# asharakeh/bayes-od-rc

Hardware: AMD Instinct MI355X
Metric: images/sec at N=10 MC samples, 512x512; per-anchor covariance latency (higher is better)
Workload: dtype bf16; 1 GPU; ResNet-50 RetinaNet + covar head, N=10 MC-dropout, 512x512, full BayesOD pipeline (forward+posterior+soft-NMS+cluster-fuse); global_batch=512, mc_samples=10, anchors=49104, parallelism=one GPU (no exchange; N > 1: image-sharded, one RCCL gather/step), visible_gpus=1, gpu_max_hw_queues=4

## Files before the change

### bayes-od-rc_amd/build.py

```python
import os
import shutil
import subprocess
import sys

HERE = os.path.dirname(os.path.abspath(__file__))
CSRC = os.path.join(HERE, "csrc")
LIB_DIR = os.path.join(HERE, "lib")
LIB_PATH = os.path.join(LIB_DIR, "libbayesod_hip.so")

SOURCES = [
    ("conv_igemm.hip", []),
    ("conv_igemm_f32.hip", []),
    ("conv_pointwise.hip", []),
    ("aux_kernels.hip", []),
    ("post_kernels.hip", ["-ffp-contract=off"]),
    ("loss_kernels.hip", ["-ffp-contract=off"]),
    ("pdq_kernels.hip", ["-ffp-contract=off"]),
    ("score_kernels.hip", ["-ffp-contract=off"]),
    ("target_kernels.hip", ["-ffp-contract=off"]),
    ("stat_kernels.hip", ["-ffp-contract=off"]),
    ("train_kernels.hip", []),
    ("jpeg_kernels.hip", []),
    ("png_kernels.hip", []),
    ("corrupt_kernels.hip", ["-ffp-contract=off"]),
    ("engine.hip", []),
]
COMMON = ["--offload-arch=gfx950", "-O3", "-std=c++17", "-fPIC", "-Wall", "-Wno-unused-function",
          "-Wno-unused-result", "-Wno-unused-value", "-fno-slp-vectorize"]


def _hipcc():
    for cand in (os.environ.get("HIPCC"), shutil.which("hipcc"), "/opt/rocm/bin/hipcc"):
        if cand and os.path.exists(cand):
            return cand
    raise RuntimeError("hipcc not found (ROCm toolchain required to build libbayesod_hip.so)")


def _stale(target, deps):
    if not os.path.exists(target):
        return True
    t = os.path.getmtime(target)
    return any(os.path.getmtime(d) > t for d in deps)


HEADER = os.path.join(os.path.dirname(HERE), "include", "bayesod.h")
CDEF = os.path.join(os.path.dirname(HERE), "include", "bayesod_cdef.h")


def cdef_text():
    import re
    text = open(HEADER).read()
    text = re.sub(r"/\*.*?\*/", "", text, flags=re.S)
    out = []
    for line in text.splitlines():
        t = line.strip()
        if not t or t.startswith("#") or t == 'extern "C" {' or t == "}":
            continue
        out.append(line.rstrip())
    return ("/* GENERATED from include/bayesod.h by bayes_od_rc_amd.build.write_cdef(): the same declarations without\n"
            " * comments / preprocessor lines, for ffi.cdef(open('include/bayesod_cdef.h').read()).  Do not edit. */\n"
            + "\n".join(out) + "\n")


def write_cdef():
    text = cdef_text()
    if not os.path.exists(CDEF) or open(CDEF).read() != text:
        with open(CDEF, "w") as fp:
            fp.write(text)
    return CDEF


def _load_guard():
    import importlib.util
    spec = importlib.util.spec_from_file_location("bayesod_kernel_guard", os.path.join(HERE, "kernel_guard.py"))
    mod = importlib.util.module_from_spec(spec)
    spec.loader.exec_module(mod)
    return mod


def build(force=False, verbose=True):
    hipcc = _hipcc()
    try:
        write_cdef()
    except OSError as e:
        if verbose:
            print("include/bayesod_cdef.h not refreshed (%s)" % e, flush=True)
    os.makedirs(LIB_DIR, exist_ok=True)
    obj_dir = os.path.join(LIB_DIR, "obj")
    os.makedirs(obj_dir, exist_ok=True)
    headers = [os.path.join(CSRC, f) for f in os.listdir(CSRC) if f.endswith((".h", ".inc"))]
    headers.append(os.path.join(os.path.dirname(HERE), "include", "bayesod.h"))
    objs = []
    for src, extra in SOURCES:
        s = os.path.join(CSRC, src)
        o = os.path.join(obj_dir, src.replace(".hip", ".o"))
        if force or _stale(o, [s] + headers):
            cmd = [hipcc] + COMMON + extra + ["-c", s, "-o", o]
            if verbose:
                print(" ".join(cmd), flush=True)
            subprocess.check_call(cmd)
        objs.append(o)
    if force or _stale(LIB_PATH, objs):
        if os.environ.get("BOD_SKIP_KERNEL_GUARD") == "1":
            print("WARNING: BOD_SKIP_KERNEL_GUARD=1 -- linking libbayesod_hip.so WITHOUT the disassembly guards (spills, inline-asm MFMA "
                  "hazard windows and hand-counted LDS waits are UNCHECKED)", file=sys.stderr, flush=True)
        else:
            kernel_guard = _load_guard()
            regs = kernel_guard.verify(os.path.join(obj_dir, "conv_igemm.o"))
            regs.update(kernel_guard.verify_aux(os.path.join(obj_dir, "aux_kernels.o")))
            regs.update(kernel_guard.verify_pointwise(os.path.join(obj_dir, "conv_pointwise.o")))
            regs.update(kernel_guard.verify_pointwise_stage3(os.path.join(obj_dir, "conv_pointwise.o")))
            n_checked = sum(kernel_guard.check_no_packed_fp32(o) for o in objs)
            if verbose:
                print("no packed fp32 instruction in %d kernels" % n_checked, flush=True)
            if verbose:
                print("kernel guards ok: %d production kernels, no spills, inline-asm MFMA windows clean" % len(regs), flush=True)
        cmd = [hipcc, "--offload-arch=gfx950", "-shared", "-fPIC"] + objs + ["-o", LIB_PATH]
        if verbose:
            print(" ".join(cmd), flush=True)
        subprocess.check_call(cmd)
    return LIB_PATH


if __name__ == "__main__":
    build(force="--force" in sys.argv)
```

### bayes-od-rc_amd/csrc/conv_pointwise.hip

```cpp
#include "kernels.h"
#include <algorithm>

typedef __attribute__((ext_vector_type(8))) short pw_bf16x8;
typedef __attribute__((ext_vector_type(16))) float pw_f32x16;
typedef __attribute__((ext_vector_type(4))) float pw_f32x4;
typedef __attribute__((ext_vector_type(2))) uint32_t pw_u32x2;
typedef __attribute__((ext_vector_type(4))) uint32_t pw_u32x4;
typedef __attribute__((ext_vector_type(4))) int pw_i32x4;

#define PW_GLOBAL_PTR(p) ((const __attribute__((address_space(1))) void*)(p))
#define PW_LDS_PTR(p) ((__attribute__((address_space(3))) void*)(p))

__device__ uint4 pw_sink[64];

__device__ __forceinline__ uint32_t pw_pack(float lo, float hi) {
    uint32_t r;
    asm("v_cvt_pk_bf16_f32 %0, %1, %2" : "=v"(r) : "v"(lo), "v"(hi));
    return r;
}
__device__ __forceinline__ uint32_t pw_relu(uint32_t w) {
    uint32_t r;
    asm("v_pk_max_i16 %0, %1, 0" : "=v"(r) : "v"(w));
    return r;
}
__device__ __forceinline__ float pw_bf2f(uint32_t v) { return __uint_as_float(v << 16); }

template <int CPR> __device__ __forceinline__ int pw_swz(int px) { return CPR >= 16 ? (px & 15) : ((px >> 1) & 7); }

template <int N> __device__ __forceinline__ void pw_wait_vm() { asm volatile("s_waitcnt vmcnt(%0)" ::"n"(N) : "memory"); }
__device__ __forceinline__ void pw_lds_barrier() {
    asm volatile("s_waitcnt lgkmcnt(0)" ::: "memory");
    __builtin_amdgcn_s_barrier();
    asm volatile("" ::: "memory");
}

template <int K, int BP, bool RES, int WGS, int BC = 128, int NEXT = 0>
__global__ __launch_bounds__(BC * 2, WGS) void pw_conv_kernel(const ConvArgs a, int ptiles, int ctiles, int pstride) {
    constexpr int THREADS = BC * 2;
    constexpr int CPX = K * 2 / 16;
    constexpr int RCH = BC / 8;
    constexpr int XB = BP * K * 2;
    constexpr int RB = BP * BC * 2;
    constexpr int NXP = BP * CPX / THREADS;
    constexpr int NRP = BP * RCH / THREADS;
    constexpr int FP = BP / 32, KS = K / 16;
    constexpr int C2 = 64, KS2 = NEXT == 2 ? K / 16 : BC / 16;
    constexpr int K2 = NEXT == 2 ? K : BC;
    constexpr int NTP = NEXT ? BP * (C2 / 8) / THREADS : 0;
    static_assert(NXP >= 1 && NRP >= 1 && BP % 32 == 0 && (CPX & 7) == 0 && (!NEXT || (BC == 256 && BP == 64 && NTP == 1)), "tile shape");
    extern __shared__ __attribute__((aligned(16))) char pw_smem[];
    char* const xbuf = pw_smem;
    constexpr int NRB = RES ? 2 : 1;
    char* const rbuf = pw_smem + 2 * XB;
    int4* const meta = reinterpret_cast<int4*>(pw_smem + 2 * XB + NRB * RB);
    char* const tbuf = pw_smem + 2 * XB + NRB * RB + 3 * BP * 16;

    const int tid = threadIdx.x, lane = tid & 63;
    const int wave = __builtin_amdgcn_readfirstlane(tid >> 6);
    const int frow = lane & 31, fhalf = lane >> 5;
    const ConvGroup& G = a.g[0];
    const int xcd = blockIdx.x & 7, jb = blockIdx.x >> 3;
    const int ct = jb % ctiles, p0 = (jb / ctiles) * 8 + xcd;
    const int c0 = ct * BC;
    const int nt = p0 < ptiles ? (ptiles - p0 + pstride - 1) / pstride : 0;
    if (nt == 0) return;

    auto load_ent = [&](int t) {
        const int tt = t < nt ? t : nt - 1;
        int m = (p0 + tt * pstride) * BP + (tid % BP);
        const int valid = m < a.M;
        m = valid ? m : a.M - 1;
        const int4 e = *reinterpret_cast<const int4*>(&a.rows[m]);
        return make_int4(e.x, e.z, e.w, valid);
    };
    auto issue = [&](int t) {
        const int4* mt = meta + (t % 3) * BP;
        char* xb = xbuf + (t & 1) * XB;
#pragma unroll
        for (int i = 0; i < NXP; ++i) {
            const int q = i * THREADS + tid, row = q / CPX, cp = q % CPX;
            const int c = cp ^ pw_swz<CPX>(row);
            const char* src = reinterpret_cast<const char*>(G.in) + ((size_t)mt[row].x * a.in_cstride + G.in_coff + c * 8) * 2;
            __builtin_amdgcn_global_load_lds(PW_GLOBAL_PTR(src), PW_LDS_PTR(xb + (i * THREADS + wave * 64) * 16), 16, 0, 0);
        }
        if (RES) {
            char* rb = rbuf + (t & 1) * RB;
#pragma unroll
            for (int i = 0; i < NRP; ++i) {
                const int q = i * THREADS + tid, row = q / RCH, cp = q % RCH;
                const int c = cp ^ (row & 7);
                const char* src = reinterpret_cast<const char*>(G.res) + ((size_t)mt[row].z * a.res_cstride + c0 + c * 8) * 2;
                __builtin_amdgcn_global_load_lds(PW_GLOBAL_PTR(src), PW_LDS_PTR(rb + (i * THREADS + wave * 64) * 16), 16, 0, 0);
            }
        }
    };

    {
        const int4 e0 = load_ent(0), e1 = load_ent(1);
        if (tid < BP) { meta[tid] = e0; meta[BP + tid] = e1; }
    }
    __syncthreads();
    issue(0);
    asm volatile("" ::: "memory");
    pw_bf16x8 wf[KS];
    {
        const char* wrow = reinterpret_cast<const char*>(G.w) + ((size_t)(c0 + wave * 32 + frow) * K + fhalf * 8) * 2;
#pragma unroll
        for (int ks = 0; ks < KS; ++ks) wf[ks] = *reinterpret_cast<const pw_bf16x8*>(wrow + ks * 32);
    }
    float4 bv[4];
#pragma unroll
    for (int g = 0; g < 4; ++g) bv[g] = *reinterpret_cast<const float4*>(G.bias + c0 + wave * 32 + g * 8 + fhalf * 4);
    const bool relu = a.flags & CONV_RELU;
    pw_bf16x8 wf2[NEXT ? KS2 : 1];
    float4 bv2[4];
    if (NEXT) {
        const char* wrow = reinterpret_cast<const char*>(G.ch_w3) + ((size_t)((wave & 1) * 32 + frow) * K2 + fhalf * 8) * 2;
#pragma unroll
        for (int ks = 0; ks < KS2; ++ks) wf2[ks] = *reinterpret_cast<const pw_bf16x8*>(wrow + ks * 32);
#pragma unroll
        for (int g = 0; g < 4; ++g) bv2[g] = *reinterpret_cast<const float4*>(G.ch_b3 + (wave & 1) * 32 + g * 8 + fhalf * 4);
    }

    for (int t = 0; t < nt; ++t) {
        __syncthreads();
        const bool more = t + 1 < nt;
        if (more) issue(t + 1);
        asm volatile("" ::: "memory");
        const int4 ent = load_ent(t + 2);
        asm volatile("" ::: "memory");
        if (more) { if (t > 0) pw_wait_vm<1 + NRP + NTP + NXP + (RES ? NRP : 0) + 1>(); else pw_wait_vm<NXP + (RES ? NRP : 0) + 1>(); }
        else pw_wait_vm<1>();
        __syncthreads();

        const char* xb = xbuf + (t & 1) * XB;
        char* rb = rbuf + (RES ? (t & 1) : 0) * RB;
        pw_f32x16 acc[FP];
#pragma unroll
        for (int j = 0; j < FP; ++j)
#pragma unroll
            for (int r = 0; r < 16; ++r) acc[j][r] = 0.f;
#pragma unroll
        for (int ks = 0; ks < KS; ++ks)
#pragma unroll
            for (int j = 0; j < FP; ++j) {
                const int px = j * 32 + frow;
                const pw_bf16x8 b = *reinterpret_cast<const pw_bf16x8*>(xb + px * (K * 2) + (((ks * 2 + fhalf) ^ pw_swz<CPX>(px)) << 4));
                acc[j] = __builtin_amdgcn_mfma_f32_32x32x16_bf16(wf[ks], b, acc[j], 0, 0, 0);
            }
#pragma unroll
        for (int j = 0; j < FP; ++j) {
            const int px = j * 32 + frow;
#pragma unroll
            for (int g = 0; g < 4; ++g) {
                char* p = rb + px * (BC * 2) + (((wave * 4 + g) ^ (px & 7)) << 4) + fhalf * 8;
                float v0 = __builtin_fmaf(acc[j][g * 4 + 0], 1.0f, bv[g].x), v1 = __builtin_fmaf(acc[j][g * 4 + 1], 1.0f, bv[g].y);
                float v2 = __builtin_fmaf(acc[j][g * 4 + 2], 1.0f, bv[g].z), v3 = __builtin_fmaf(acc[j][g * 4 + 3], 1.0f, bv[g].w);
                if (RES) {
                    const uint2 r = *reinterpret_cast<const uint2*>(p);
                    v0 += pw_bf2f(r.x & 0xFFFFu) * 1.0f; v1 += pw_bf2f(r.x >> 16) * 1.0f;
                    v2 += pw_bf2f(r.y & 0xFFFFu) * 1.0f; v3 += pw_bf2f(r.y >> 16) * 1.0f;
                }
                uint2 o;
                o.x = pw_pack(v0, v1); o.y = pw_pack(v2, v3);
                if (relu) { o.x = pw_relu(o.x); o.y = pw_relu(o.y); }
                *reinterpret_cast<uint2*>(p) = o;
            }
        }
        __syncthreads();
        {
            const int4* mt = meta + (t % 3) * BP;
#pragma unroll
            for (int i = 0; i < NRP; ++i) {
                const int q = i * THREADS + tid, row = q / RCH, cp = q % RCH;
                const int c = cp ^ (row & 7);
                const uint4 v = *reinterpret_cast<const uint4*>(rb + q * 16);
                const int4 e = mt[row];
                uint4* dst = e.w ? reinterpret_cast<uint4*>(reinterpret_cast<uint16_t*>(G.out) + (size_t)e.y * a.out_cstride + c0 + c * 8) : &pw_sink[lane];
                *dst = v;
            }
        }
        if (NEXT) {
            if (wave < 4) {
                const int px = (wave >> 1) * 32 + frow;
                pw_f32x16 acc2;
#pragma unroll
                for (int r = 0; r < 16; ++r) acc2[r] = 0.f;
#pragma unroll
                for (int ks = 0; ks < KS2; ++ks) {
                    const pw_bf16x8 b = NEXT == 2 ? *reinterpret_cast<const pw_bf16x8*>(xb + px * (K * 2) + (((ks * 2 + fhalf) ^ pw_swz<CPX>(px)) << 4))
                                                  : *reinterpret_cast<const pw_bf16x8*>(rb + px * (BC * 2) + (((ks * 2 + fhalf) ^ (px & 7)) << 4));
                    acc2 = __builtin_amdgcn_mfma_f32_32x32x16_bf16(wf2[ks], b, acc2, 0, 0, 0);
                }
#pragma unroll
                for (int g = 0; g < 4; ++g) {
                    uint2 o;
                    o.x = pw_relu(pw_pack(__builtin_fmaf(acc2[g * 4 + 0], 1.0f, bv2[g].x), __builtin_fmaf(acc2[g * 4 + 1], 1.0f, bv2[g].y)));
                    o.y = pw_relu(pw_pack(__builtin_fmaf(acc2[g * 4 + 2], 1.0f, bv2[g].z), __builtin_fmaf(acc2[g * 4 + 3], 1.0f, bv2[g].w)));
                    *reinterpret_cast<uint2*>(tbuf + px * 128 + ((((wave & 1) * 4 + g) ^ (px & 7)) << 4) + fhalf * 8) = o;
                }
            }
            __syncthreads();
            {
                const int4* mt = meta + (t % 3) * BP;
                const int q = tid, row = q >> 3, cp = q & 7;
                const int c = cp ^ (row & 7);
                const uint4 v = *reinterpret_cast<const uint4*>(tbuf + q * 16);
                const int4 e = mt[row];
                uint4* dst = e.w ? reinterpret_cast<uint4*>(reinterpret_cast<uint16_t*>(G.ch_out3) + (size_t)e.y * C2 + c * 8) : &pw_sink[lane];
                *dst = v;
            }
        }
        asm volatile("" ::: "memory");
        if (tid < BP) meta[((t + 2) % 3) * BP + tid] = ent;
    }
}

template <int K, int BP, bool RES, int WGS, int BC = 128, int NEXT = 0>
static hipError_t pw_launch_cfg(const ConvArgs& a, hipStream_t s) {
    constexpr int LDS = 2 * BP * K * 2 + (RES ? 2 : 1) * BP * BC * 2 + 3 * BP * 16 + (NEXT ? BP * 128 : 0);
    static PerDeviceOnce once;
    bool& attr_set = *once.slot();
    auto kern = pw_conv_kernel<K, BP, RES, WGS, BC, NEXT>;
    if (!attr_set) {
        hipError_t e = hipFuncSetAttribute(reinterpret_cast<const void*>(kern), hipFuncAttributeMaxDynamicSharedMemorySize, LDS);
        if (e != hipSuccess) return e;
        attr_set = true;
    }
    const int ptiles = (a.M + BP - 1) / BP, ctiles = a.cout_pad / BC;
    const int slots = launch_cus(a) * WGS;
    int pstride = std::min(slots / ctiles, ptiles) / 8 * 8;
    if (pstride < 8) pstride = 8;
    hipLaunchKernelGGL(kern, dim3(pstride * ctiles), dim3(BC * 2), LDS, s, a, ptiles, ctiles, pstride);
    return hipGetLastError();
}

__global__ __launch_bounds__(512, 1) void pw_conv512_next_kernel(const ConvArgs a, int ptiles, int pstride) {
    constexpr int K = 128, BP = 32, BC = 512, C2 = 128, THREADS = 512;
    constexpr int CPX = K / 8, RCH = BC / 8, TCH = C2 / 8;
    constexpr int XB = BP * K * 2, RB = BP * BC * 2, TB = BP * C2 * 2;
    constexpr int NXP = BP * CPX / THREADS, NRP = BP * RCH / THREADS, NTP = BP * TCH / THREADS;
    constexpr int KS = K / 16, KSH = BC / 32;
    static_assert(NXP == 1 && NRP == 4 && NTP == 1, "tile shape");
    extern __shared__ __attribute__((aligned(16))) char pw_smem[];
    char* const xbuf = pw_smem;
    char* const rbuf = pw_smem + 2 * XB;
    pw_i32x4* const meta = reinterpret_cast<pw_i32x4*>(pw_smem + 2 * XB + 2 * RB);
    char* const tbuf = pw_smem + 2 * XB + 2 * RB + 3 * BP * 16;
    pw_f32x4* const relay = reinterpret_cast<pw_f32x4*>(pw_smem + 2 * XB + 2 * RB + 3 * BP * 16 + TB);
    float* const sbias = reinterpret_cast<float*>(pw_smem + 2 * XB + 2 * RB + 3 * BP * 16 + TB + 16384);

    const int tid = threadIdx.x, lane = tid & 63;
    const int wave = __builtin_amdgcn_readfirstlane(tid >> 6);
    const int frow = lane & 31, fhalf = lane >> 5;
    const int cb = wave & 3, kh = wave >> 2;
    const ConvGroup& G = a.g[0];
    const int p0 = blockIdx.x;
    const int nt = p0 < ptiles ? (ptiles - p0 + pstride - 1) / pstride : 0;
    if (nt == 0) return;

    auto load_ent = [&](int t) {
        const int tt = t < nt ? t : nt - 1;
        int m = (p0 + tt * pstride) * BP + (tid % BP);
        const int valid = m < a.M;
        m = valid ? m : a.M - 1;
        const int4 e = *reinterpret_cast<const int4*>(&a.rows[m]);
        return pw_i32x4{e.x, e.z, e.w, valid};
    };
    auto issue = [&](int t) {
        const int* mt = reinterpret_cast<const int*>(meta + (t % 3) * BP);
        const int in_off = mt[(tid / CPX) * 4];
        int res_off[NRP];
#pragma unroll
        for (int i = 0; i < NRP; ++i) res_off[i] = mt[((i * THREADS + tid) / RCH) * 4 + 2];
        {
            const int row = tid / CPX, cp = tid % CPX;
            const int c = cp ^ pw_swz<CPX>(row);
            const char* src = reinterpret_cast<const char*>(G.in) + ((size_t)in_off * a.in_cstride + G.in_coff + c * 8) * 2;
            __builtin_amdgcn_global_load_lds(PW_GLOBAL_PTR(src), PW_LDS_PTR(xbuf + (t & 1) * XB + (wave * 64) * 16), 16, 0, 0);
        }
        char* rb = rbuf + (t & 1) * RB;
#pragma unroll
        for (int i = 0; i < NRP; ++i) {
            const int q = i * THREADS + tid, row = q / RCH, cp = q % RCH;
            const int c = cp ^ pw_swz<RCH>(row);
            const char* src = reinterpret_cast<const char*>(G.res) + ((size_t)res_off[i] * a.res_cstride + c * 8) * 2;
            __builtin_amdgcn_global_load_lds(PW_GLOBAL_PTR(src), PW_LDS_PTR(rb + (i * THREADS + wave * 64) * 16), 16, 0, 0);
        }
    };

    {
        const pw_i32x4 e0 = load_ent(0), e1 = load_ent(1);
        if (tid < BP) { meta[tid] = e0; meta[BP + tid] = e1; }
        sbias[tid] = G.bias[tid];
        if (tid < C2) sbias[BC + tid] = G.ch_b3[tid];
    }
    __syncthreads();
    issue(0);
    asm volatile("" ::: "memory");
    pw_bf16x8 wf[2][KS], wf2[KSH];
#pragma unroll
    for (int b = 0; b < 2; ++b) {
        const char* wrow = reinterpret_cast<const char*>(G.w) + ((size_t)(wave * 64 + b * 32 + frow) * K + fhalf * 8) * 2;
#pragma unroll
        for (int ks = 0; ks < KS; ++ks) wf[b][ks] = *reinterpret_cast<const pw_bf16x8*>(wrow + ks * 32);
    }
    {
        const char* wrow = reinterpret_cast<const char*>(G.ch_w3) + ((size_t)(cb * 32 + frow) * BC + kh * (BC / 2) + fhalf * 8) * 2;
#pragma unroll
        for (int ks = 0; ks < KSH; ++ks) wf2[ks] = *reinterpret_cast<const pw_bf16x8*>(wrow + ks * 32);
    }
    const bool relu = a.flags & CONV_RELU;
    const int px = frow;

    for (int t = 0; t < nt; ++t) {
        pw_lds_barrier();
        const bool more = t + 1 < nt;
        if (more) issue(t + 1);
        asm volatile("" ::: "memory");
        const pw_i32x4 ent = load_ent(t + 2);
        asm volatile("" ::: "memory");
        if (more) { if (t > 0) pw_wait_vm<1 + NRP + NTP + NXP + NRP + 1>(); else pw_wait_vm<NXP + NRP + 1>(); }
        else pw_wait_vm<1>();
        pw_lds_barrier();

        const char* xb = xbuf + (t & 1) * XB;
        char* rb = rbuf + (t & 1) * RB;
        int sw = pw_swz<RCH>(px);
        asm volatile("" : "+v"(sw));
        pw_f32x16 acc[2];
#pragma unroll
        for (int b = 0; b < 2; ++b)
#pragma unroll
            for (int r = 0; r < 16; ++r) acc[b][r] = 0.f;
#pragma unroll
        for (int ks = 0; ks < KS; ++ks) {
            const pw_bf16x8 bf = *reinterpret_cast<const pw_bf16x8*>(xb + px * (K * 2) + (((ks * 2 + fhalf) ^ sw) << 4));
            acc[0] = __builtin_amdgcn_mfma_f32_32x32x16_bf16(wf[0][ks], bf, acc[0], 0, 0, 0);
            acc[1] = __builtin_amdgcn_mfma_f32_32x32x16_bf16(wf[1][ks], bf, acc[1], 0, 0, 0);
        }
#pragma unroll
        for (int b = 0; b < 2; ++b)
#pragma unroll
            for (int g = 0; g < 4; ++g) {
                char* p = rb + px * (BC * 2) + ((((wave * 2 + b) * 4 + g) ^ sw) << 4) + fhalf * 8;
                const pw_f32x4 bv = *reinterpret_cast<const pw_f32x4*>(sbias + (wave * 2 + b) * 32 + g * 8 + fhalf * 4);
                float v0 = __builtin_fmaf(acc[b][g * 4 + 0], 1.0f, bv.x), v1 = __builtin_fmaf(acc[b][g * 4 + 1], 1.0f, bv.y);
                float v2 = __builtin_fmaf(acc[b][g * 4 + 2], 1.0f, bv.z), v3 = __builtin_fmaf(acc[b][g * 4 + 3], 1.0f, bv.w);
                const pw_u32x2 r = *reinterpret_cast<const pw_u32x2*>(p);
                v0 += pw_bf2f(r.x & 0xFFFFu) * 1.0f; v1 += pw_bf2f(r.x >> 16) * 1.0f;
                v2 += pw_bf2f(r.y & 0xFFFFu) * 1.0f; v3 += pw_bf2f(r.y >> 16) * 1.0f;
                pw_u32x2 o;
                o.x = pw_pack(v0, v1); o.y = pw_pack(v2, v3);
                if (relu) { o.x = pw_relu(o.x); o.y = pw_relu(o.y); }
                *reinterpret_cast<pw_u32x2*>(p) = o;
            }
        pw_lds_barrier();
        const pw_i32x4* mt = meta + (t % 3) * BP;
#pragma unroll
        for (int i = 0; i < NRP; ++i) {
            const int q = i * THREADS + tid, row = q / RCH, cp = q % RCH;
            const int c = cp ^ pw_swz<RCH>(row);
            const pw_u32x4 v = *reinterpret_cast<const pw_u32x4*>(rb + q * 16);
            const pw_i32x4 e = mt[row];
            pw_u32x4* dst = e.w ? reinterpret_cast<pw_u32x4*>(reinterpret_cast<uint16_t*>(G.out) + (size_t)e.y * a.out_cstride + c * 8) : reinterpret_cast<pw_u32x4*>(&pw_sink[lane]);
            *dst = v;
        }
        pw_f32x16 acc2;
        if (kh == 0) {
#pragma unroll
            for (int r = 0; r < 16; ++r) acc2[r] = 0.f;
#pragma unroll
            for (int ks = 0; ks < KSH; ++ks) {
                const pw_bf16x8 bf = *reinterpret_cast<const pw_bf16x8*>(rb + px * (BC * 2) + (((ks * 2 + fhalf) ^ sw) << 4));
                acc2 = __builtin_amdgcn_mfma_f32_32x32x16_bf16(wf2[ks], bf, acc2, 0, 0, 0);
            }
#pragma unroll
            for (int g = 0; g < 4; ++g) relay[(cb * 4 + g) * 64 + lane] = pw_f32x4{acc2[g * 4 + 0], acc2[g * 4 + 1], acc2[g * 4 + 2], acc2[g * 4 + 3]};
        }
        pw_lds_barrier();
        if (kh == 1) {
#pragma unroll
            for (int g = 0; g < 4; ++g) {
                const pw_f32x4 v = relay[(cb * 4 + g) * 64 + lane];
                acc2[g * 4 + 0] = v.x; acc2[g * 4 + 1] = v.y; acc2[g * 4 + 2] = v.z; acc2[g * 4 + 3] = v.w;
            }
#pragma unroll
            for (int ks = 0; ks < KSH; ++ks) {
                const pw_bf16x8 bf = *reinterpret_cast<const pw_bf16x8*>(rb + px * (BC * 2) + (((KSH * 2 + ks * 2 + fhalf) ^ sw) << 4));
                acc2 = __builtin_amdgcn_mfma_f32_32x32x16_bf16(wf2[ks], bf, acc2, 0, 0, 0);
            }
#pragma unroll
            for (int g = 0; g < 4; ++g) {
                const pw_f32x4 bv = *reinterpret_cast<const pw_f32x4*>(sbias + BC + cb * 32 + g * 8 + fhalf * 4);
                pw_u32x2 o;
                o.x = pw_relu(pw_pack(__builtin_fmaf(acc2[g * 4 + 0], 1.0f, bv.x), __builtin_fmaf(acc2[g * 4 + 1], 1.0f, bv.y)));
                o.y = pw_relu(pw_pack(__builtin_fmaf(acc2[g * 4 + 2], 1.0f, bv.z), __builtin_fmaf(acc2[g * 4 + 3], 1.0f, bv.w)));
                *reinterpret_cast<pw_u32x2*>(tbuf + px * (C2 * 2) + (((cb * 4 + g) ^ sw) << 4) + fhalf * 8) = o;
            }
        }
        pw_lds_barrier();
        if (tid < BP) meta[((t + 2) % 3) * BP + tid] = ent;
        {
            const int row = tid / TCH, cp = tid % TCH;
            const int c = cp ^ pw_swz<TCH>(row);
            const pw_u32x4 v = *reinterpret_cast<const pw_u32x4*>(tbuf + tid * 16);
            const pw_i32x4 e = mt[row];
            pw_u32x4* dst = e.w ? reinterpret_cast<pw_u32x4*>(reinterpret_cast<uint16_t*>(G.ch_out3) + (size_t)e.y * C2 + c * 8) : reinterpret_cast<pw_u32x4*>(&pw_sink[lane]);
            *dst = v;
        }
    }
}

static hipError_t pw_launch_next512(const ConvArgs& a, hipStream_t s) {
    constexpr int BP = 32;
    constexpr int LDS = 2 * BP * 128 * 2 + 2 * BP * 512 * 2 + 3 * BP * 16 + BP * 128 * 2 + 16384 + (512 + 128) * 4;
    static PerDeviceOnce once;
    bool& attr_set = *once.slot();
    if (!attr_set) {
        hipError_t e = hipFuncSetAttribute(reinterpret_cast<const void*>(pw_conv512_next_kernel), hipFuncAttributeMaxDynamicSharedMemorySize, LDS);
        if (e != hipSuccess) return e;
        attr_set = true;
    }
    const int ptiles = (a.M + BP - 1) / BP;
    int pstride = std::min(launch_cus(a), ptiles) / 8 * 8;
    if (pstride < 8) pstride = 8;
    hipLaunchKernelGGL(pw_conv512_next_kernel, dim3(pstride), dim3(512), LDS, s, a, ptiles, pstride);
    return hipGetLastError();
}

bool conv_pointwise_eligible(const ConvArgs& a) {
    static const bool on = [] { const char* e = getenv("BOD_POINTWISE"); return !e || atoi(e) != 0; }();
    if (!on) return false;
    const ConvGroup& g = a.g[0];
    if (a.variant != 0 || a.split || a.xreuse || a.ksplit > 1 || a.groups != 1 || a.taps != 1 || a.fan_count > 1) return false;
    if (a.flags & (CONV_DROPOUT | CONV_OUT_F32 | CONV_ACCUM)) return false;
    if (g.w2 || g.ch_w2 || g.out_relu || g.agg_kind) return false;
    if (g.ch_w3 && !(g.ch_b3 && g.ch_out3 && ((a.cin == 64 && a.cout_pad == 256 && (g.res != nullptr) != (g.ch_dual != 0)) ||
                                              (a.cin == 128 && a.cout_pad == 512 && g.res && !g.ch_dual)))) return false;
    if (a.cin != 64 && a.cin != 128 && a.cin != 256 && !(a.cin == 512 && !g.res)) return false;
    if (a.cout_pad % 128 != 0 || a.cout_valid != a.cout_pad) return false;
    if ((a.in_cstride & 7) || (a.out_cstride & 7) || (g.in_coff & 7) || (g.res && (a.res_cstride & 7))) return false;
    static const int min_m = [] { const char* e = getenv("BOD_POINTWISE_MIN_M"); return e ? atoi(e) : -1; }();
    if (a.M < (min_m >= 0 ? min_m : 128 * launch_cus(a))) return false;
    return true;
}

hipError_t launch_conv_pointwise(const ConvArgs& a, hipStream_t s) {
    const bool res = a.g[0].res != nullptr;
    if (a.g[0].ch_w3 && a.g[0].ch_dual) return pw_launch_cfg<64, 64, false, 1, 256, 2>(a, s);
    if (a.g[0].ch_w3 && a.cin == 128) return pw_launch_next512(a, s);
    if (a.g[0].ch_w3) return pw_launch_cfg<64, 64, true, 1, 256, 1>(a, s);
    if (a.cin == 64) return res ? pw_launch_cfg<64, 64, true, 3>(a, s) : pw_launch_cfg<64, 64, false, 3>(a, s);
    if (a.cin == 128) return res ? pw_launch_cfg<128, 64, true, 2>(a, s) : pw_launch_cfg<128, 64, false, 2>(a, s);
    if (a.cin == 512) return pw_launch_cfg<512, 32, false, 2>(a, s);
    return res ? pw_launch_cfg<256, 32, true, 3>(a, s) : pw_launch_cfg<256, 32, false, 3>(a, s);
}


__global__ __launch_bounds__(256, 2) void slide3x3_c64_kernel(const ConvArgs a, int nstrips, int xsegs) {
    constexpr int SLOT = 66 * 128;
    constexpr int LEAD = 1;
    constexpr int RING = 4;
    constexpr int OB = 64 * 128;
    extern __shared__ __attribute__((aligned(16))) char sl_smem[];
    char* const ring = sl_smem;
    char* const obuf = sl_smem + RING * SLOT;
    const int tid = threadIdx.x, lane = tid & 63;
    const int wave = __builtin_amdgcn_readfirstlane(tid >> 6);
    const int frow = lane & 31, fhalf = lane >> 5;
    const int wc = wave & 1, wp = wave >> 1;
    const ConvGroup& G = a.g[0];
    const int H = a.plane_h, W = a.plane_w;

    pw_bf16x8 wf[36];
    {
        const char* wrow = reinterpret_cast<const char*>(G.w) + ((size_t)(wc * 32 + frow) * 576 + fhalf * 8) * 2;
#pragma unroll
        for (int k = 0; k < 36; ++k) wf[k] = *reinterpret_cast<const pw_bf16x8*>(wrow + k * 32);
    }
    float4 bv[4];
#pragma unroll
    for (int g = 0; g < 4; ++g) bv[g] = *reinterpret_cast<const float4*>(G.bias + wc * 32 + g * 8 + fhalf * 4);
    const bool relu = a.flags & CONV_RELU;

    for (int strip = blockIdx.x; strip < nstrips; strip += gridDim.x) {
        const int b = strip / xsegs, xs = strip - b * xsegs;
        const int x0 = xs * 64, nv = min(64, W - x0);
        const int m00 = (b * H) * W + x0;
        const int4 e0 = *reinterpret_cast<const int4*>(&a.rows[m00]);
        const int out_pitch = H > 1 ? a.rows[m00 + W].out_off - e0.z : 0;
        const long in0 = (long)e0.x;
        const int in_pitch = e0.y;
        auto issue_row = [&](int ir) {
            char* slot = ring + (ir % RING) * SLOT;
            auto piece = [&](int i) {
                const int q = i * 256 + tid;
                int px = q >> 3;
                const int cp = q & 7;
                const int c = cp ^ pw_swz<8>(px);
                px = px < nv + 2 ? px : 0;
                const char* src = reinterpret_cast<const char*>(G.in) + (((size_t)(in0 + (long)ir * in_pitch + px)) * a.in_cstride + G.in_coff + c * 8) * 2;
                __builtin_amdgcn_global_load_lds(PW_GLOBAL_PTR(src), PW_LDS_PTR(slot + (i * 256 + wave * 64) * 16), 16, 0, 0);
            };
            piece(0); piece(1);
            if (wave == 0 && lane < 16) piece(2);
        };
        __syncthreads();
        issue_row(0); issue_row(1); issue_row(2);
        for (int y = 0; y < H; ++y) {
            const bool pre = y + LEAD < H;
            if (pre) issue_row(y + 2 + LEAD);
            asm volatile("" ::: "memory");
            if (!pre) pw_wait_vm<0>();
            else if (wave == 0) { if (y == 0) pw_wait_vm<3>(); else pw_wait_vm<5>(); }
            else { if (y == 0) pw_wait_vm<2>(); else pw_wait_vm<4>(); }
            __syncthreads();
            pw_f32x16 acc;
#pragma unroll
            for (int r = 0; r < 16; ++r) acc[r] = 0.f;
#pragma unroll
            for (int ky = 0; ky < 3; ++ky) {
                const char* slot = ring + ((y + ky) % RING) * SLOT;
#pragma unroll
                for (int kx = 0; kx < 3; ++kx)
#pragma unroll
                    for (int ks = 0; ks < 4; ++ks) {
                        const int px = wp * 32 + frow + kx;
                        const pw_bf16x8 bf = *reinterpret_cast<const pw_bf16x8*>(slot + px * 128 + (((ks * 2 + fhalf) ^ pw_swz<8>(px)) << 4));
                        acc = __builtin_amdgcn_mfma_f32_32x32x16_bf16(wf[(ky * 3 + kx) * 4 + ks], bf, acc, 0, 0, 0);
                    }
            }
            char* ob = obuf + (y & 1) * OB;
            {
                const int px = wp * 32 + frow;
#pragma unroll
                for (int g = 0; g < 4; ++g) {
                    uint2 o;
                    o.x = pw_pack(__builtin_fmaf(acc[g * 4 + 0], 1.0f, bv[g].x), __builtin_fmaf(acc[g * 4 + 1], 1.0f, bv[g].y));
                    o.y = pw_pack(__builtin_fmaf(acc[g * 4 + 2], 1.0f, bv[g].z), __builtin_fmaf(acc[g * 4 + 3], 1.0f, bv[g].w));
                    if (relu) { o.x = pw_relu(o.x); o.y = pw_relu(o.y); }
                    *reinterpret_cast<uint2*>(ob + px * 128 + (((wc * 4 + g) ^ (px & 7)) << 4) + fhalf * 8) = o;
                }
            }
            __syncthreads();
#pragma unroll
            for (int i = 0; i < 2; ++i) {
                const int q = i * 256 + tid, px = q >> 3, cp = q & 7;
                const int c = cp ^ (px & 7);
                const uint4 v = *reinterpret_cast<const uint4*>(ob + q * 16);
                uint4* dst = px < nv ? reinterpret_cast<uint4*>(reinterpret_cast<uint16_t*>(G.out) + ((size_t)e0.z + (size_t)y * out_pitch + px) * a.out_cstride + c * 8)
                                     : &pw_sink[lane];
                *dst = v;
            }
            asm volatile("" ::: "memory");
        }
    }
}

__global__ __launch_bounds__(512, 1) void slide3x3_c128_kernel(const ConvArgs a, int nstrips, int xsegs) {
    constexpr int SLOT = 66 * 256;
    constexpr int RING = 4;
    constexpr int OB = 64 * 256;
    extern __shared__ __attribute__((aligned(16))) char sl_smem[];
    char* const ring = sl_smem;
    char* const obuf = sl_smem + RING * SLOT;
    float4* const xch = reinterpret_cast<float4*>(sl_smem + RING * SLOT + 2 * OB);
    float* const sbias = reinterpret_cast<float*>(sl_smem + RING * SLOT + 2 * OB + 8 * 4096);
    const int tid = threadIdx.x, lane = tid & 63;
    const int wave = __builtin_amdgcn_readfirstlane(tid >> 6);
    const int frow = lane & 31, fhalf = lane >> 5;
    const int cb = wave & 3, kh = wave >> 2;
    const ConvGroup& G = a.g[0];
    const int H = a.plane_h, W = a.plane_w;

    pw_bf16x8 wf[36];
    {
        const char* wrow = reinterpret_cast<const char*>(G.w) + ((size_t)(cb * 32 + frow) * 1152 + kh * 64 + fhalf * 8) * 2;
#pragma unroll
        for (int t = 0; t < 9; ++t)
#pragma unroll
            for (int ks = 0; ks < 4; ++ks) wf[t * 4 + ks] = *reinterpret_cast<const pw_bf16x8*>(wrow + (t * 128 + ks * 16) * 2);
    }
    if (tid < 128) sbias[tid] = G.bias[tid];
    const bool relu = a.flags & CONV_RELU;

    for (int strip = blockIdx.x; strip < nstrips; strip += gridDim.x) {
        const int b = strip / xsegs, xs = strip - b * xsegs;
        const int x0 = xs * 64, nv = min(64, W - x0);
        const int m00 = (b * H) * W + x0;
        const int4 e0 = *reinterpret_cast<const int4*>(&a.rows[m00]);
        const int out_pitch = H > 1 ? a.rows[m00 + W].out_off - e0.z : 0;
        const long in0 = (long)e0.x;
        const int in_pitch = e0.y;
        auto issue_row = [&](int ir) {
            char* slot = ring + (ir % RING) * SLOT;
            auto piece = [&](int i) {
                const int q = i * 512 + tid;
                int px = q >> 4;
                const int cp = q & 15;
                const int c = cp ^ (px & 7);
                px = px < nv + 2 ? px : 0;
                const char* src = reinterpret_cast<const char*>(G.in) + (((size_t)(in0 + (long)ir * in_pitch + px)) * a.in_cstride + G.in_coff + c * 8) * 2;
                __builtin_amdgcn_global_load_lds(PW_GLOBAL_PTR(src), PW_LDS_PTR(slot + (i * 512 + wave * 64) * 16), 16, 0, 0);
            };
            piece(0); piece(1);
            if (wave == 0 && lane < 32) piece(2);
        };
        __syncthreads();
        issue_row(0); issue_row(1); issue_row(2);
        for (int y = 0; y < H; ++y) {
            const bool pre = y + 1 < H;
            if (pre) issue_row(y + 3);
            asm volatile("" ::: "memory");
            if (!pre) pw_wait_vm<0>();
            else if (wave == 0) { if (y == 0) pw_wait_vm<3>(); else pw_wait_vm<5>(); }
            else { if (y == 0) pw_wait_vm<2>(); else pw_wait_vm<4>(); }
            __syncthreads();
            pw_f32x16 acc[2];
#pragma unroll
            for (int j = 0; j < 2; ++j)
#pragma unroll
                for (int r = 0; r < 16; ++r) acc[j][r] = 0.f;
#pragma unroll
            for (int ky = 0; ky < 3; ++ky) {
                const char* slot = ring + ((y + ky) % RING) * SLOT;
#pragma unroll
                for (int kx = 0; kx < 3; ++kx)
#pragma unroll
                    for (int ks = 0; ks < 4; ++ks)
#pragma unroll
                        for (int j = 0; j < 2; ++j) {
                            const int px = j * 32 + frow + kx;
                            const pw_bf16x8 bf = *reinterpret_cast<const pw_bf16x8*>(slot + px * 256 + (((kh * 8 + ks * 2 + fhalf) ^ (px & 7)) << 4));
                            acc[j] = __builtin_amdgcn_mfma_f32_32x32x16_bf16(wf[(ky * 3 + kx) * 4 + ks], bf, acc[j], 0, 0, 0);
                        }
            }
            {
                float4* mine = xch + wave * 256;
#pragma unroll
                for (int g = 0; g < 4; ++g) {
                    const pw_f32x16& v = acc[1 - kh];
                    mine[g * 64 + lane] = make_float4(v[g * 4 + 0], v[g * 4 + 1], v[g * 4 + 2], v[g * 4 + 3]);
                }
            }
            __syncthreads();
            char* ob = obuf + (y & 1) * OB;
            {
                const float4* theirs = xch + (wave ^ 4) * 256;
                const int px = kh * 32 + frow;
#pragma unroll
                for (int g = 0; g < 4; ++g) {
                    const float4 t = theirs[g * 64 + lane];
                    const pw_f32x16& v = acc[kh];
                    const float s0 = kh ? t.x + v[g * 4 + 0] : v[g * 4 + 0] + t.x, s1 = kh ? t.y + v[g * 4 + 1] : v[g * 4 + 1] + t.y;
                    const float s2 = kh ? t.z + v[g * 4 + 2] : v[g * 4 + 2] + t.z, s3 = kh ? t.w + v[g * 4 + 3] : v[g * 4 + 3] + t.w;
                    const float4 bvg = *reinterpret_cast<const float4*>(sbias + cb * 32 + g * 8 + fhalf * 4);
                    uint2 o;
                    o.x = pw_pack(__builtin_fmaf(s0, 1.0f, bvg.x), __builtin_fmaf(s1, 1.0f, bvg.y));
                    o.y = pw_pack(__builtin_fmaf(s2, 1.0f, bvg.z), __builtin_fmaf(s3, 1.0f, bvg.w));
                    if (relu) { o.x = pw_relu(o.x); o.y = pw_relu(o.y); }
                    *reinterpret_cast<uint2*>(ob + px * 256 + (((cb * 4 + g) ^ (px & 7)) << 4) + fhalf * 8) = o;
                }
            }
            __syncthreads();
#pragma unroll
            for (int i = 0; i < 2; ++i) {
                const int q = i * 512 + tid, px = q >> 4, cp = q & 15;
                const int c = cp ^ (px & 7);
                const uint4 v = *reinterpret_cast<const uint4*>(ob + q * 16);
                uint4* dst = px < nv ? reinterpret_cast<uint4*>(reinterpret_cast<uint16_t*>(G.out) + ((size_t)e0.z + (size_t)y * out_pitch + px) * a.out_cstride + c * 8)
                                     : &pw_sink[lane];
                *dst = v;
            }
            asm volatile("" ::: "memory");
        }
    }
}

bool conv_slide3x3_eligible(const ConvArgs& a) {
    static const bool on = [] { const char* e = getenv("BOD_SLIDE3X3"); return !e || atoi(e) != 0; }();
    if (!on) return false;
    const ConvGroup& g = a.g[0];
    if (a.variant != 0 || a.split || a.xreuse || a.ksplit > 1 || a.groups != 1 || a.taps != 9 || a.KW != 3 || a.fan_count > 1) return false;
    if (a.flags & (CONV_DROPOUT | CONV_OUT_F32 | CONV_ACCUM)) return false;
    if (g.w2 || g.ch_w2 || g.out_relu || g.agg_kind || g.res) return false;
    const bool c64 = a.cin == 64 && a.cout_pad == 64 && a.cout_valid == 64;
    static const bool c128_on = [] { const char* e = getenv("BOD_SLIDE3X3_C128"); return !e || atoi(e) != 0; }();
    const bool c128 = c128_on && a.cin == 128 && a.cout_pad == 128 && a.cout_valid == 128;
    if ((!c64 && !c128) || a.plane_h < 1 || a.plane_w < 1) return false;
    if ((a.in_cstride & 7) || (a.out_cstride & 7) || (g.in_coff & 7)) return false;
    if (a.M % (a.plane_h * a.plane_w) != 0) return false;
    static const int min_m = [] { const char* e = getenv("BOD_POINTWISE_MIN_M"); return e ? atoi(e) : -1; }();
    if (min_m >= 0) return a.M >= min_m;
    const long nstrips = (long)(a.M / (a.plane_h * a.plane_w)) * ((a.plane_w + 63) / 64);
    if (c128) return nstrips >= (long)launch_cus(a);
    return 2 * nstrips >= 3 * (long)launch_cus(a);
}

hipError_t launch_conv_slide3x3(const ConvArgs& a, hipStream_t s) {
    if (a.cin == 128) {
        constexpr int LDS128 = 4 * 66 * 256 + 2 * 64 * 256 + 8 * 4096 + 512;
        static PerDeviceOnce once128;
        bool& set128 = *once128.slot();
        if (!set128) {
            hipError_t e = hipFuncSetAttribute(reinterpret_cast<const void*>(slide3x3_c128_kernel), hipFuncAttributeMaxDynamicSharedMemorySize, LDS128);
            if (e != hipSuccess) return e;
            set128 = true;
        }
        const int xsegs = (a.plane_w + 63) / 64;
        const int nstrips = a.M / (a.plane_h * a.plane_w) * xsegs;
        hipLaunchKernelGGL(slide3x3_c128_kernel, dim3(std::min(nstrips, launch_cus(a))), dim3(512), LDS128, s, a, nstrips, xsegs);
        return hipGetLastError();
    }
    constexpr int LDS = 4 * 66 * 128 + 2 * 64 * 128;
    static PerDeviceOnce once;
    bool& attr_set = *once.slot();
    if (!attr_set) {
        hipError_t e = hipFuncSetAttribute(reinterpret_cast<const void*>(slide3x3_c64_kernel), hipFuncAttributeMaxDynamicSharedMemorySize, LDS);
        if (e != hipSuccess) return e;
        attr_set = true;
    }
    const int xsegs = (a.plane_w + 63) / 64;
    const int nstrips = a.M / (a.plane_h * a.plane_w) * xsegs;
    const int wgs = std::min(nstrips, 2 * launch_cus(a));
    hipLaunchKernelGGL(slide3x3_c64_kernel, dim3(wgs), dim3(256), LDS, s, a, nstrips, xsegs);
    return hipGetLastError();
}

bool conv_pointwise_can_fuse_next(const ConvArgs& a) {
    static const bool on = [] { const char* e = getenv("BOD_PW_FUSE_NEXT"); return !e || atoi(e) != 0; }();
    static const bool forced = [] { const char* e = getenv("BOD_FORCE_CONV_TILE"); return e && atoi(e) != 0; }();
    if (!on || forced) return false;
    return a.cin == 64 && a.cout_pad == 256 && a.g[0].res && conv_pointwise_eligible(a);
}

bool conv_pointwise_can_fuse_next3(const ConvArgs& a) {
    static const bool on = [] { const char* e = getenv("BOD_PW_FUSE_NEXT3"); return !e || atoi(e) != 0; }();
    static const bool forced = [] { const char* e = getenv("BOD_FORCE_CONV_TILE"); return e && atoi(e) != 0; }();
    if (!on || forced) return false;
    return a.cin == 128 && a.cout_pad == 512 && a.g[0].res && conv_pointwise_eligible(a);
}

bool conv_pointwise_can_fuse_dual(const ConvArgs& a) {
    static const bool on = [] { const char* e = getenv("BOD_PW_FUSE_DUAL"); return !e || atoi(e) != 0; }();
    static const bool forced = [] { const char* e = getenv("BOD_FORCE_CONV_TILE"); return e && atoi(e) != 0; }();
    if (!on || forced) return false;
    return a.cin == 64 && a.cout_pad == 256 && !a.g[0].res && !(a.flags & CONV_RELU) && conv_pointwise_eligible(a);
}
```

### bayes-od-rc_amd/csrc/engine.hip

```cpp
#include "../../include/bayesod.h"
#include "kernels.h"
#include "plane_tables.h"
#include "jpeg_entropy.h"
#include "png_inflate.h"

#include <algorithm>
#include <array>
#include <atomic>
#include <chrono>
#include <cmath>
#include <condition_variable>
#include <deque>
#include <functional>
#include <mutex>
#include <thread>
#include <tuple>
#include <type_traits>
#include <cstdarg>
#include <cstdio>
#include <cstring>
#include <map>
#include <memory>
#include <string>
#include <system_error>
// ... 3744 lines not shown
    }
    return pdq_call(device, [&](hipStream_t s, char* err, size_t cap) -> int {
        CorruptSlot slot;
        uint8_t* d_rgb = nullptr;
        uint8_t* d_out = nullptr;
        int st = corrupt_prepare(slot, who, spec, src_hw, s, err, cap);
        if (st == BOD_OK && hipMalloc(reinterpret_cast<void**>(&d_rgb), slot.frame_bytes) != hipSuccess) {
            d_rgb = nullptr; snprintf(err, cap, "%s: out of device memory for the frames", who); st = BOD_ERR_OOM;
        }
        if (st == BOD_OK && hipMemcpyAsync(d_rgb, rgb_packed_in, slot.frame_bytes, hipMemcpyHostToDevice, s) != hipSuccess) {
            snprintf(err, cap, "%s: copying the frames in failed", who); st = BOD_ERR_HIP;
        }
        if (st == BOD_OK) st = corrupt_enqueue(slot, who, spec, d_rgb, s, &d_out, err, cap);
        if (st == BOD_OK && (hipMemcpyAsync(rgb_packed_out, d_out, slot.frame_bytes, hipMemcpyDeviceToHost, s) != hipSuccess ||
                             hipStreamSynchronize(s) != hipSuccess)) {
            snprintf(err, cap, "%s: copying the frames back failed: %s", who, hipGetErrorString(hipGetLastError())); st = BOD_ERR_HIP;
        }
        hipStreamSynchronize(s);
        if (d_rgb) hipFree(d_rgb);
        slot.release();
        return st;
    });
}

bod_status bod_set_upload_corruption(bod_handle h, const bod_corrupt_op* ops, int32_t ops_per_frame, const uint32_t* frame_ids,
                                     const uint16_t* taps, int32_t n_taps, const uint8_t* luts, int32_t n_luts, const uint16_t* qtables,
                                     int32_t n_qtables, uint64_t seed) {
    if (!h) return BOD_ERR_INVALID_ARG;
    if (!ops) { h->corrupt_pending = CorruptSpec{}; return BOD_OK; }
    CorruptSpec spec;
    char err[512] = {0};
    const int st = corrupt_spec_make("bod_set_upload_corruption", h->cfg.batch, ops, ops_per_frame, frame_ids, taps, n_taps, luts, n_luts, qtables,
                                     n_qtables, seed, &spec, err, sizeof err);
    if (st != BOD_OK) return h->fail((bod_status)st, "%s", err);
    h->corrupt_pending = std::move(spec);
    return BOD_OK;
}

bod_status bod_jpeg_decode_rgb(int32_t device, int32_t n, const uint8_t* const* data, const int64_t* len, int32_t threads,
                               uint8_t* rgb_packed, int64_t rgb_capacity, int32_t* src_hw) {
    static const char* who = "bod_jpeg_decode_rgb";
    if (n < 1 || !data || !len || !rgb_packed || !src_hw) { g_create_error = std::string(who) + ": NULL argument or no frame"; return BOD_ERR_INVALID_ARG; }
    return pdq_call(device, [&](hipStream_t s, char* err, size_t cap) -> int {
        JpegSlot js;
        std::string e;
        uint8_t* d_rgb = nullptr;
        bod_status st = jpeg_host_decode(js, who, n, data, len, threads, src_hw, &e);
        if (st == BOD_OK && js.rgb_bytes > rgb_capacity) {
            e = std::string(who) + ": the frames take " + std::to_string(js.rgb_bytes) + " bytes, the buffer holds " + std::to_string(rgb_capacity);
            st = BOD_ERR_INVALID_ARG;
        }
        if (st == BOD_OK && hipMalloc(reinterpret_cast<void**>(&d_rgb), (size_t)js.rgb_bytes) != hipSuccess) {
            d_rgb = nullptr; e = std::string(who) + ": out of device memory for the frames"; st = BOD_ERR_OOM;
        }
        if (st == BOD_OK) st = jpeg_enqueue(js, who, d_rgb, s, &e);
        if (st == BOD_OK && (hipMemcpyAsync(rgb_packed, d_rgb, (size_t)js.rgb_bytes, hipMemcpyDeviceToHost, s) != hipSuccess ||
                             hipStreamSynchronize(s) != hipSuccess)) {
            e = std::string(who) + ": copying the frames back failed: " + hipGetErrorString(hipGetLastError()); st = BOD_ERR_HIP;
        }
        hipStreamSynchronize(s);
        if (d_rgb) hipFree(d_rgb);
        js.release();
        if (st != BOD_OK) snprintf(err, cap, "%s", e.c_str());
        return st;
    });
}

bod_status bod_png_decode_rgb(int32_t device, int32_t n, const uint8_t* const* data, const int64_t* len, int32_t threads,
                              uint8_t* rgb_packed, int64_t rgb_capacity, int32_t* src_hw) {
    static const char* who = "bod_png_decode_rgb";
    if (n < 1 || !data || !len || !rgb_packed || !src_hw) { g_create_error = std::string(who) + ": NULL argument or no frame"; return BOD_ERR_INVALID_ARG; }
    return pdq_call(device, [&](hipStream_t s, char* err, size_t cap) -> int {
        PngSlot ps;
        std::string e;
        uint8_t* d_rgb = nullptr;
        bod_status st = png_host_decode(ps, who, n, data, len, threads, src_hw, &e);
        if (st == BOD_OK && ps.rgb_bytes > rgb_capacity) {
            e = std::string(who) + ": the frames take " + std::to_string(ps.rgb_bytes) + " bytes, the buffer holds " + std::to_string(rgb_capacity);
            st = BOD_ERR_INVALID_ARG;
        }
        if (st == BOD_OK && hipMalloc(reinterpret_cast<void**>(&d_rgb), (size_t)ps.rgb_bytes) != hipSuccess) {
            d_rgb = nullptr; e = std::string(who) + ": out of device memory for the frames"; st = BOD_ERR_OOM;
        }
        if (st == BOD_OK) st = png_enqueue(ps, who, d_rgb, s, &e);
        if (st == BOD_OK && (hipMemcpyAsync(rgb_packed, d_rgb, (size_t)ps.rgb_bytes, hipMemcpyDeviceToHost, s) != hipSuccess ||
                             hipStreamSynchronize(s) != hipSuccess)) {
            e = std::string(who) + ": copying the frames back failed: " + hipGetErrorString(hipGetLastError()); st = BOD_ERR_HIP;
        }
        hipStreamSynchronize(s);
        if (d_rgb) hipFree(d_rgb);
        ps.release();
        if (st != BOD_OK) snprintf(err, cap, "%s", e.c_str());
        return st;
    });
}

bod_status bod_bench_png_decode(int32_t device, int32_t n, const uint8_t* const* data, const int64_t* len, int32_t threads, int32_t iters,
                                double* host_ms, double* kernel_ms) {
    static const char* who = "bod_bench_png_decode";
    if (n < 1 || iters < 1 || !data || !len || !host_ms || !kernel_ms) { g_create_error = std::string(who) + ": NULL argument, no frame or no iteration"; return BOD_ERR_INVALID_ARG; }
    return pdq_call(device, [&](hipStream_t s, char* err, size_t cap) -> int {
        PngSlot ps;
        std::string e;
        uint8_t* d_rgb = nullptr;
        hipEvent_t ev[2] = {nullptr, nullptr};
        std::vector<int32_t> hw((size_t)n * 2);
        bod_status st = BOD_OK;
        for (int i = 0; i < iters && st == BOD_OK; ++i) {
            const auto t0 = std::chrono::steady_clock::now();
            st = png_host_decode(ps, who, n, data, len, threads, hw.data(), &e);
            host_ms[i] = std::chrono::duration<double, std::milli>(std::chrono::steady_clock::now() - t0).count();
        }
        if (st == BOD_OK && hipMalloc(reinterpret_cast<void**>(&d_rgb), (size_t)ps.rgb_bytes) != hipSuccess) {
            d_rgb = nullptr; e = std::string(who) + ": out of device memory for the frames"; st = BOD_ERR_OOM;
        }
        if (st == BOD_OK) st = png_enqueue(ps, who, d_rgb, s, &e);
        if (st == BOD_OK && (hipEventCreate(&ev[0]) != hipSuccess || hipEventCreate(&ev[1]) != hipSuccess)) { e = std::string(who) + ": hipEventCreate failed"; st = BOD_ERR_HIP; }
        for (int i = 0; i < iters && st == BOD_OK; ++i) {
            float ms = 0.f;
            hipError_t he = hipEventRecord(ev[0], s);
            if (he == hipSuccess) he = launch_png_unfilter(png_args(ps, d_rgb), s);
            if (he == hipSuccess) he = hipEventRecord(ev[1], s);
            if (he == hipSuccess) he = hipEventSynchronize(ev[1]);
            if (he == hipSuccess) he = hipEventElapsedTime(&ms, ev[0], ev[1]);
            if (he != hipSuccess) { e = std::string(who) + ": timing the kernel failed: " + hipGetErrorString(he); st = BOD_ERR_HIP; }
            kernel_ms[i] = ms;
        }
        hipStreamSynchronize(s);
        for (hipEvent_t v : ev) if (v) hipEventDestroy(v);
        if (d_rgb) hipFree(d_rgb);
        ps.release();
        if (st != BOD_OK) snprintf(err, cap, "%s", e.c_str());
        return st;
    });
}

bod_status bod_bench_head_conv(bod_handle h, int32_t layer, int32_t variant, int32_t iters, double* mean_ms, double* flops) {
    if (!h || !mean_ms || iters < 1 || layer < 0 || layer > 7) return BOD_ERR_INVALID_ARG;
    BODCHK(join_overlap(h));
    if (!h->weights_ready) return h->fail(BOD_ERR_NOT_READY, "weights not finalized");
    HIPCHK(h, hipSetDevice(h->cfg.device));
    int seen = 0; Op* op = nullptr;
    for (Op& o : h->ops) if (o.is_head3x3 && o.flavour != FLAVOUR_RAW && seen++ == layer) { op = &o; break; }
    if (!op) return h->fail(BOD_ERR_INVALID_ARG, "no head launch %d", layer);
    ConvArgs a = op->conv;
    a.variant = variant;
    hipEvent_t e0, e1;
    HIPCHK(h, hipEventCreate(&e0)); HIPCHK(h, hipEventCreate(&e1));
    HIPCHK(h, launch_conv_igemm(a, h->stream));
    HIPCHK(h, hipEventRecord(e0, h->stream));
    for (int i = 0; i < iters; ++i) HIPCHK(h, launch_conv_igemm(a, h->stream));
    HIPCHK(h, hipEventRecord(e1, h->stream));
    HIPCHK(h, hipStreamSynchronize(h->stream));
    float ms = 0; HIPCHK(h, hipEventElapsedTime(&ms, e0, e1));
    hipEventDestroy(e0); hipEventDestroy(e1);
    if ((variant == 90 || variant == 91) && a.mx == 1) {
        unsigned long long c[16];
        conv_igemm_phase_cycles(c, true);
        const double tiles = (double)c[15];
        fprintf(stderr, "# f16mx phase clock, wave 0, cycles per tile (%.0f tiles): whole tile %.0f = set-up %.0f + loop %.0f (of which: waiting for the next K-tile's pieces + barrier %.0f, "
                        "K-tile bodies %.0f; 72 K-tiles) + epilogue %.0f; of the wait: vmcnt / lgkmcnt %.0f, s_barrier %.0f\n", tiles, (double)c[9] / tiles, ((double)c[8] - (double)c[6] - (double)c[7]) / tiles,
                ((double)c[6] + (double)c[7]) / tiles, (double)c[6] / tiles, (double)c[7] / tiles, ((double)c[9] - (double)c[8]) / tiles,
                (double)c[13] / tiles, ((double)c[6] - (double)c[13]) / tiles);
        fprintf(stderr, "# f16mx phase clock by K-tile flavour, cycles per K-tile: wave 0: H %.0f  X %.0f | wave 4: H %.0f  X %.0f, wait + barrier per K-tile %.0f (wave 0: %.0f)"
                        " | MFMA issue of a SIMD's two waves: H 2048, X 1024\n",
                (double)c[0] / tiles / 36.0, (double)c[1] / tiles / 36.0, (double)c[2] / tiles / 36.0, (double)c[3] / tiles / 36.0, (double)c[4] / tiles / 72.0, (double)c[6] / tiles / 72.0);
    } else if (variant == 90) {
        unsigned long long c[16];
        conv_igemm_phase_cycles(c, true);
        const double tiles = (double)c[15];
        static const char* names[6] = {"set-up", "main loop", "barrier+bias/relu/pack", "philox+lds writes", "barrier", "store loop"};
        fprintf(stderr, "# phase clock, wave 0, cycles per tile (%.0f tiles):", tiles);
        for (int k = 0; k < 6; ++k) fprintf(stderr, "  %s %.0f", names[k], (double)c[k] / tiles);
        if (c[10] + c[11] + c[12] > 0)
            fprintf(stderr, "  fused 1x1 MFMAs %.0f  barriers+fp32 tile %.0f  MC reduction+stores %.0f", (double)c[10] / tiles, (double)c[11] / tiles, (double)c[12] / tiles);
        double cyc = 0; for (int k = 0; k < 6; ++k) cyc += (double)c[k];
        cyc += (double)c[10] + (double)c[11] + (double)c[12];
        fprintf(stderr, "  | shader clock during the tiles %.3f GHz (cycles / 100 MHz real-time ticks); tiles account for %.3f ms of the %.3f ms launch per CU\n",
                cyc / (double)c[14] * 0.1, (double)c[14] / tiles * 1e-5 * (tiles / (iters + 1)) / 256.0, ms / iters);
    }
    *mean_ms = ms / iters;
    if (flops) *flops = op->flops;
    return BOD_OK;
}

bod_status bod_profile_begin(bod_handle h) {
    if (!h) return BOD_ERR_INVALID_ARG;
    for (auto& e : h->ev_head) { hipEventDestroy(e.first); hipEventDestroy(e.second); }
    for (auto& e : h->ev_post) { hipEventDestroy(e.first); hipEventDestroy(e.second); }
    h->ev_head.clear(); h->ev_post.clear(); h->prof_flops = 0; h->profiling = true;
    return BOD_OK;
}

extern "C++" {
namespace {
struct Rccl {
    typedef int (*gather_fn)(const void*, void*, size_t, int, int, void*, hipStream_t);
    typedef const char* (*errstr_fn)(int);
    gather_fn gather = nullptr; errstr_fn errstr = nullptr; bool tried = false;
    bool load() {
        if (tried) return gather != nullptr;
        tried = true;
        void* lib = dlopen("librccl.so", RTLD_NOW | RTLD_GLOBAL);
        if (!lib) lib = dlopen("librccl.so.1", RTLD_NOW | RTLD_GLOBAL);
        if (!lib) return false;
        gather = reinterpret_cast<gather_fn>(dlsym(lib, "ncclGather"));
        errstr = reinterpret_cast<errstr_fn>(dlsym(lib, "ncclGetErrorString"));
        return gather != nullptr;
    }
};
Rccl& rccl() { static Rccl r; return r; }
}
}

int32_t bod_record_width(bod_handle h) { return h ? 21 + 2 * h->cfg.num_classes + (h->parts ? 48 : 0) + (h->class_parts ? 4 : 0) : 0; }

bod_status bod_gather_detections(bod_handle h, int32_t slot, void* nccl_comm, int32_t world, int32_t rank, int32_t root,
                                 float* gathered_host, float** gathered_device) {
    MarkerRange mr_api("bod:gather_detections");
    if (!h) return BOD_ERR_INVALID_ARG;
    if (world < 1 || rank < 0 || rank >= world || root < 0 || root >= world)
        return h->fail(BOD_ERR_INVALID_ARG, "bod_gather_detections: world %d, rank %d, root %d", world, rank, root);
    if (!nccl_comm && world != 1) return h->fail(BOD_ERR_INVALID_ARG, "bod_gather_detections: %d ranks need an ncclComm_t", world);
    if (rank != root && (gathered_host || gathered_device)) return h->fail(BOD_ERR_INVALID_ARG, "bod_gather_detections: only the root receives");
    HIPCHK(h, hipSetDevice(h->cfg.device));
    const int B = h->cfg.batch, K = h->cfg.nms_max_output_size, C = h->cfg.num_classes, W = bod_record_width(h);
    const size_t block = (size_t)B * K * W;
    int sidx = slot;
    static const bool side_on = [] { const char* e = getenv("BOD_SIDE_STREAM"); return e && atoi(e) != 0; }();
    hipStream_t st = (slot >= 0 && slot <= 1 && !side_on && h->done_stream[slot]) ? h->done_stream[slot] : h->side;
    if (slot < 0) {
        if (!h->cluster_done) return h->fail(BOD_ERR_NOT_READY, "bod_gather_detections: bod_cluster_fuse has not run");
        BODCHK(join_overlap(h));
        sidx = h->slot;
        st = h->stream;
    } else if (slot > 1 || !h->side_pending[slot]) {
        return h->fail(BOD_ERR_NOT_READY, "bod_gather_detections: slot %d has no pending batch", slot);
    }
    for (int img = 0; h->parts && img < B; ++img)
        if (!h->det_parts_ok[sidx][img]) return h->fail(BOD_ERR_NOT_READY, "bod_gather_detections: image %d was fused without its posterior's parts (bod_set_posterior_parts)", img);
    for (int img = 0; h->cparts && img < B; ++img)
        if (!h->det_cparts_ok[sidx][img]) return h->fail(BOD_ERR_NOT_READY, "bod_gather_detections: image %d was fused without its posterior's class parts (bod_set_posterior_class_parts)", img);
    if (!h->rec_send && hipMalloc(reinterpret_cast<void**>(&h->rec_send), block * 4) != hipSuccess)
        return h->fail(BOD_ERR_OOM, "bod_gather_detections: %zu bytes", block * 4);
    if (h->ev_gather && h->gather_stream && h->gather_stream != st) HIPCHK(h, hipStreamWaitEvent(st, h->ev_gather, 0));
    if (slot >= 0) HIPCHK(h, hipStreamWaitEvent(st, h->ev_done[slot], 0));
    if (h->cparts)
        HIPCHK(h, launch_pack_records_class(h->nms_nsel_s[sidx], h->out_scores_s[sidx], h->out_means_s[sidx], h->out_covs_s[sidx],
                                            h->out_counts_s[sidx], h->out_parts_s[sidx], h->out_cparts_s[sidx], h->rec_send, B, K, C, st));
    else if (h->parts)
        HIPCHK(h, launch_pack_records_parts(h->nms_nsel_s[sidx], h->out_scores_s[sidx], h->out_means_s[sidx], h->out_covs_s[sidx],
                                            h->out_counts_s[sidx], h->out_parts_s[sidx], h->rec_send, B, K, C, st));
    else
        HIPCHK(h, launch_pack_records(h->nms_nsel_s[sidx], h->out_scores_s[sidx], h->out_means_s[sidx], h->out_covs_s[sidx],
                                      h->out_counts_s[sidx], h->rec_send, B, K, C, st));
    float* recv = nullptr;
    if (rank == root) {
        if (world == 1 && !nccl_comm) recv = h->rec_send;
        else {
            if (h->rec_recv_elems < block * world) {
                if (h->rec_recv && h->rec_recv != h->rec_send) hipFree(h->rec_recv);
                h->rec_recv = nullptr; h->rec_recv_elems = 0;
                if (hipMalloc(reinterpret_cast<void**>(&h->rec_recv), block * world * 4) != hipSuccess)
                    return h->fail(BOD_ERR_OOM, "bod_gather_detections: %zu bytes", block * world * 4);
                h->rec_recv_elems = block * world;
            }
            recv = h->rec_recv;
        }
    }
    if (nccl_comm) {
        if (!rccl().load()) return h->fail(BOD_ERR_NOT_READY, "bod_gather_detections: librccl.so (ncclGather) could not be opened");
        const int rc = rccl().gather(h->rec_send, recv, block,  7, root, nccl_comm, st);
        if (rc != 0) return h->fail(BOD_ERR_HIP, "ncclGather: %s", rccl().errstr ? rccl().errstr(rc) : "error");
    }
    if (!h->ev_gather) HIPCHK(h, hipEventCreateWithFlags(&h->ev_gather, hipEventDisableTiming));
    if (rank == root && gathered_host) {
        HIPCHK(h, hipMemcpyAsync(gathered_host, recv, block * world * 4, hipMemcpyDeviceToHost, st));
        HIPCHK(h, hipEventRecord(h->ev_gather, st)); h->gather_stream = st;
        HIPCHK(h, hipEventSynchronize(h->ev_gather));
    } else {
        HIPCHK(h, hipEventRecord(h->ev_gather, st)); h->gather_stream = st;
    }
    if (!(rank == root && gathered_host) && slot >= 0) {
        HIPCHK(h, hipEventRecord(h->ev_done[slot], st));
    }
    if (gathered_device) *gathered_device = recv;
    return BOD_OK;
}

bod_status bod_plan_info(bod_handle h, int32_t* info8) {
    if (!h || !info8) return BOD_ERR_INVALID_ARG;
    if (!h->weights_ready) return h->fail(BOD_ERR_NOT_READY, "bod_plan_info: the plan is built by bod_finalize_weights");
    for (int i = 0; i < 8; ++i) info8[i] = 0;
    info8[0] = h->agg_plan; info8[1] = h->plan_fused_out; info8[2] = h->plan_xreuse; info8[3] = h->plan_xreuse0;
    info8[4] = (int32_t)h->ops.size();
    for (const Op& o : h->ops) if (o.kind == Op::CONV && !o.is_head3x3 && o.conv.xreuse) ++info8[5];
    info8[6] = h->plan_mx;
    info8[7] = h->plan_sparse;
    return BOD_OK;
}

bod_status bod_plan_info_n(bod_handle h, int32_t* info, int32_t n) {
    if (!h || !info || n < 0) return BOD_ERR_INVALID_ARG;
    int32_t all[11];
    BODCHK(bod_plan_info(h, all));
    all[8] = h->plan_halo;
    all[9] = h->plan_tail_rows;
    all[10] = h->plan_stage_end;
    for (int i = 0; i < n && i < 11; ++i) info[i] = all[i];
    return BOD_OK;
}

static bod_status stat_handle(bod_handle h, const char* who) {
    if (!h->cfg.mc_statistics) return h->fail(BOD_ERR_INVALID_ARG, "%s: the handle was not created with mc_statistics = 1", who);
    BODCHK(join_overlap(h));
    HIPCHK(h, hipSetDevice(h->cfg.device));
    return ensure_stat(h);
}

static bod_status stat_view_ready(bod_handle h, const char* who, int32_t view) {
    if (view != BOD_VIEW_IDENTITY && view != BOD_VIEW_HFLIP)
        return h->fail(BOD_ERR_INVALID_ARG, "%s: view must be BOD_VIEW_IDENTITY (0) or BOD_VIEW_HFLIP (1), got %d", who, view);
    if (view == BOD_VIEW_IDENTITY) return BOD_OK;
    if (!h->anchors_ready) return h->fail(BOD_ERR_NOT_READY, "%s: bod_set_anchors has not been called (a mirrored view maps every anchor to its partner)", who);
    const bod_config& c = h->cfg;
    const int K = c.anchors_per_location;
    if (h->mirror_sym < 0) {
        std::vector<float> an((size_t)h->A * 4);
        HIPCHK(h, hipMemcpyAsync(an.data(), h->d_anchors, an.size() * 4, hipMemcpyDeviceToHost, h->stream));
        HIPCHK(h, hipStreamSynchronize(h->stream));
        const float fw = (float)c.image_w;
        int bad = -1;
        for (int l = 0; l < h->nlev && bad < 0; ++l) {
            const size_t off = (size_t)h->lvl_p0[l] * K;
            const int W = h->lw[l];
            for (int y = 0; y < h->lh[l] && bad < 0; ++y)
                for (int x = 0; x < W && bad < 0; ++x)
                    for (int k = 0; k < K; ++k) {
                        const float* s = &an[(off + ((size_t)y * W + x) * K + k) * 4];
                        const float* p = &an[(off + ((size_t)y * W + (W - 1 - x)) * K + k) * 4];
                        const float want[4] = {s[0], fw - s[1], s[2], s[3]};
                        if (memcmp(p, want, 16) != 0) { bad = l; break; }
                    }
        }
        h->mirror_sym = bad < 0; h->mirror_bad_level = bad < 0 ? 0 : c.min_level + bad;
    }
    if (!h->mirror_sym)
        return h->fail(BOD_ERR_INVALID_ARG, "%s: the anchors of pyramid level %d are not mirror-symmetric about image_w / 2 for a %dx%d image "
                       "(BOD_VIEW_HFLIP needs image_w to be a multiple of 2^max_level = %d)", who, h->mirror_bad_level, c.image_h, c.image_w,
                       1 << c.max_level);
    return BOD_OK;
}

static bod_status stat_fold(bod_handle h, const char* who, const float* cls, const float* box, const float* cov, int kb, int32_t view = BOD_VIEW_IDENTITY) {
    if (kb < 1) return h->fail(BOD_ERR_INVALID_ARG, "%s: a record of %d samples", who, kb);
    if (h->stat_k > (1 << 24) - kb) return h->fail(BOD_ERR_INVALID_ARG, "%s: more than 2^24 samples in one accumulator", who);
    if (h->class_parts && h->stat_ent_k != h->stat_k)
        return h->fail(BOD_ERR_NOT_READY, "%s: ent_sum holds %d of the record's %d samples (bod_stat_merge_entropy / bod_stat_set_entropy has not followed)", who, h->stat_ent_k, h->stat_k);
    StatMergeArgs m{};
    m.BA = (int64_t)h->cfg.batch * h->A; m.C = h->cfg.num_classes; m.ka = h->stat_k; m.kb = kb;
    m.acc_cls = h->stat_acc[0]; m.acc_box = h->stat_acc[1]; m.acc_cov = h->stat_acc[2];
    m.src_cls = cls; m.src_box = box; m.src_cov = h->cfg.has_covar_head ? cov : nullptr;
    if (!cls || !box || (h->cfg.has_covar_head && !cov)) return h->fail(BOD_ERR_INVALID_ARG, "%s: NULL statistics array", who);
    if (cls == m.acc_cls || box == m.acc_box) return h->fail(BOD_ERR_INVALID_ARG, "%s: the source is the accumulator itself", who);
    if (((uintptr_t)cls | (uintptr_t)box | (uintptr_t)m.src_cov) & 15u) return h->fail(BOD_ERR_INVALID_ARG, "%s: statistics arrays must be 16-byte aligned", who);
    if (view == BOD_VIEW_HFLIP) {
        StatMirrorArgs mm{};
        mm.m = m; mm.A = h->A; mm.K = h->cfg.anchors_per_location; mm.nlev = h->nlev;
        for (int l = 0; l < h->nlev; ++l) { mm.lvl_off[l] = (int32_t)h->lvl_p0[l] * mm.K; mm.lvl_w[l] = h->lw[l]; }
        mm.lvl_off[h->nlev] = h->A;
        mm.u_flip = (float)(h->cfg.image_w - 1);
        HIPCHK(h, launch_stat_merge_mirror(mm, h->stream));
    } else {
        HIPCHK(h, launch_stat_merge(m, h->stream));
    }
    h->stat_k += kb;
    return BOD_OK;
}

static bod_status stat_fold_entropy(bod_handle h, const char* who, const float* ent, int32_t view = BOD_VIEW_IDENTITY) {
    if (!ent) return h->fail(BOD_ERR_INVALID_ARG, "%s: ent_sum is NULL", who);
    if (ent == h->stat_ent) return h->fail(BOD_ERR_INVALID_ARG, "%s: the source is the accumulator itself", who);
    if ((uintptr_t)ent & 15u) return h->fail(BOD_ERR_INVALID_ARG, "%s: ent_sum must be 16-byte aligned", who);
    if (h->stat_ent_k >= h->stat_k) return h->fail(BOD_ERR_NOT_READY, "%s: ent_sum already holds the record's %d samples (fold the three arrays first)", who, h->stat_k);
    const int64_t BA = (int64_t)h->cfg.batch * h->A;
    if (view == BOD_VIEW_HFLIP) {
        StatMirrorArgs mm{};
        mm.A = h->A; mm.K = h->cfg.anchors_per_location; mm.nlev = h->nlev;
        for (int l = 0; l < h->nlev; ++l) { mm.lvl_off[l] = (int32_t)h->lvl_p0[l] * mm.K; mm.lvl_w[l] = h->lw[l]; }
        mm.lvl_off[h->nlev] = h->A;
        HIPCHK(h, launch_stat_merge_entropy(h->stat_ent, ent, BA, h->stat_ent_k == 0, &mm, h->stream));
    } else {
        HIPCHK(h, launch_stat_merge_entropy(h->stat_ent, ent, BA, h->stat_ent_k == 0, nullptr, h->stream));
    }
    h->stat_ent_k = h->stat_k;
    return BOD_OK;
}

bod_status bod_stat_reset(bod_handle h) {
    if (!h) return BOD_ERR_INVALID_ARG;
    BODCHK(stat_handle(h, "bod_stat_reset"));
    h->stat_k = 0; h->stat_ent_k = 0;
    return BOD_OK;
}

static bod_status stat_forward_view(bod_handle h, const char* who, const float* images, int32_t on_device, uint64_t seed, uint32_t first_image_id,
                                    int32_t sample_base, int32_t view) {
    MarkerRange mr_api("bod:stat_forward");
    if (!h) return BOD_ERR_INVALID_ARG;
    BODCHK(stat_handle(h, who));
    if (!h->weights_ready) return h->fail(BOD_ERR_NOT_READY, "weights not finalized");
    if (!h->anchors_ready) return h->fail(BOD_ERR_NOT_READY, "bod_set_anchors has not been called (the box statistics are those of the decoded boxes)");
    const bod_config& c = h->cfg;
    const int n = c.mc_samples;
    if (sample_base < 0 || sample_base + n > 65535 || (c.mc_ensemble_size > 0 && sample_base + n > c.mc_ensemble_size))
        return h->fail(BOD_ERR_INVALID_ARG, "%s: sample_base=%d / mc_samples=%d / mc_ensemble_size=%d inconsistent", who, sample_base, n,
                       c.mc_ensemble_size);
    if (h->stat_k > (1 << 24) - n) return h->fail(BOD_ERR_INVALID_ARG, "%s: more than 2^24 samples in one accumulator", who);
    BODCHK(stat_view_ready(h, who, view));
    if (view == BOD_VIEW_HFLIP && !h->d_mirror) BODCHK(h->dalloc(&h->d_mirror, (size_t)c.batch * c.image_h * c.image_w * 3, false));
    const float* dev = nullptr;
    BODCHK(stage_images(h, images, on_device, &dev));
    if (view == BOD_VIEW_HFLIP) {
        HIPCHK(h, launch_mirror_images(dev, h->d_mirror, c.batch, c.image_h, c.image_w, h->stream));
        dev = h->d_mirror;
    }
    h->cur_images = dev;
    const int flavour = h->agg_plan ? FLAVOUR_AGG : FLAVOUR_RAW;
    const int32_t base = c.mc_sample_base;
    h->cfg.mc_sample_base = sample_base;
    const bod_status st = run_forward(h, dev, seed, first_image_id, flavour);
    h->cfg.mc_sample_base = base;
    BODCHK(st);
    if (flavour == FLAVOUR_RAW) {
        StatRawArgs r{};
        r.B = c.batch; r.N = n; r.A = h->A; r.C = c.num_classes;
        r.cls = h->raw[0]; r.box = h->raw[1]; r.cov = c.has_covar_head ? h->raw[2] : nullptr; r.anchors = h->d_anchors;
        r.cls_sum = h->agg[0]; r.box_moments = h->agg[1]; r.cov_sum = c.has_covar_head ? h->agg[2] : nullptr;
        r.ent_sum = h->ent;
        HIPCHK(h, launch_stat_from_raw(r, h->stream));
    }
    BODCHK(stat_fold(h, who, h->agg[0], h->agg[1], h->agg[2], n, view));
    if (h->class_parts) BODCHK(stat_fold_entropy(h, who, h->ent, view));
    return BOD_OK;
}

bod_status bod_stat_forward(bod_handle h, const float* images, int32_t on_device, uint64_t seed, uint32_t first_image_id, int32_t sample_base) {
    return stat_forward_view(h, "bod_stat_forward", images, on_device, seed, first_image_id, sample_base, BOD_VIEW_IDENTITY);
}

bod_status bod_stat_forward_view(bod_handle h, const float* images, int32_t on_device, uint64_t seed, uint32_t first_image_id, int32_t sample_base,
                                 int32_t view) {
    return stat_forward_view(h, "bod_stat_forward_view", images, on_device, seed, first_image_id, sample_base, view);
}

bod_status bod_stat_merge_from(bod_handle dst, bod_handle src) {
    if (!dst) return BOD_ERR_INVALID_ARG;
    if (!src) return dst->fail(BOD_ERR_INVALID_ARG, "bod_stat_merge_from: src is NULL");
    if (src == dst) return dst->fail(BOD_ERR_INVALID_ARG, "bod_stat_merge_from: src and dst are the same handle");
    if (!src->cfg.mc_statistics) return dst->fail(BOD_ERR_INVALID_ARG, "bod_stat_merge_from: src was not created with mc_statistics = 1");
    const bod_config& a = dst->cfg; const bod_config& b = src->cfg;
    const char* field = a.device != b.device ? "device" : a.batch != b.batch ? "batch" : dst->A != src->A ? "num_anchors" :
                        a.num_classes != b.num_classes ? "num_classes" : a.has_covar_head != b.has_covar_head ? "has_covar_head" : nullptr;
    if (field) return dst->fail(BOD_ERR_INVALID_ARG, "bod_stat_merge_from: the handles differ in %s", field);
    if (dst->class_parts && !src->class_parts)
        return dst->fail(BOD_ERR_INVALID_ARG, "bod_stat_merge_from: src carries no ent_sum (it was created without BOD_PARTS_CLASS in covariance_parts, dst with it)");
    BODCHK(stat_handle(dst, "bod_stat_merge_from"));
    if (src->stat_k == 0) return BOD_OK;
    if (stat_handle(src, "bod_stat_merge_from") != BOD_OK) return dst->fail(BOD_ERR_HIP, "bod_stat_merge_from: src: %s", src->err.c_str());
    if (dst->class_parts && (src->stat_ent_k != src->stat_k || dst->stat_ent_k != dst->stat_k))
        return dst->fail(BOD_ERR_NOT_READY, "bod_stat_merge_from: ent_sum is behind its record (src %d of %d samples, dst %d of %d)", src->stat_ent_k, src->stat_k,
                         dst->stat_ent_k, dst->stat_k);
    HIPCHK(dst, hipEventRecord(src->ev_stat, src->stream));
    HIPCHK(dst, hipStreamWaitEvent(dst->stream, src->ev_stat, 0));
    BODCHK(stat_fold(dst, "bod_stat_merge_from", src->stat_acc[0], src->stat_acc[1], src->stat_acc[2], src->stat_k));
    if (dst->class_parts) BODCHK(stat_fold_entropy(dst, "bod_stat_merge_from", src->stat_ent));
    HIPCHK(dst, hipEventRecord(dst->ev_stat, dst->stream));
    HIPCHK(dst, hipStreamWaitEvent(src->stream, dst->ev_stat, 0));
    return BOD_OK;
}

bod_status bod_stat_merge(bod_handle h, const void* const* ptrs3, int32_t samples) {
    if (!h) return BOD_ERR_INVALID_ARG;
    BODCHK(stat_handle(h, "bod_stat_merge"));
    if (!ptrs3) return h->fail(BOD_ERR_INVALID_ARG, "bod_stat_merge: ptrs3 is NULL");
    return stat_fold(h, "bod_stat_merge", static_cast<const float*>(ptrs3[0]), static_cast<const float*>(ptrs3[1]),
                     static_cast<const float*>(ptrs3[2]), samples);
}

bod_status bod_stat_merge_view(bod_handle h, const void* const* ptrs3, int32_t samples, int32_t view) {
    if (!h) return BOD_ERR_INVALID_ARG;
    BODCHK(stat_handle(h, "bod_stat_merge_view"));
    if (!ptrs3) return h->fail(BOD_ERR_INVALID_ARG, "bod_stat_merge_view: ptrs3 is NULL");
    BODCHK(stat_view_ready(h, "bod_stat_merge_view", view));
    return stat_fold(h, "bod_stat_merge_view", static_cast<const float*>(ptrs3[0]), static_cast<const float*>(ptrs3[1]),
                     static_cast<const float*>(ptrs3[2]), samples, view);
}

bod_status bod_stat_device(bod_handle h, void** ptrs3, int32_t* samples) {
    if (!h) return BOD_ERR_INVALID_ARG;
    BODCHK(stat_handle(h, "bod_stat_device"));
    if (ptrs3) { ptrs3[0] = h->stat_acc[0]; ptrs3[1] = h->stat_acc[1]; ptrs3[2] = h->cfg.has_covar_head ? h->stat_acc[2] : nullptr; }
    if (samples) *samples = h->stat_k;
    return BOD_OK;
}

bod_status bod_stat_get(bod_handle h, float* cls_sum, float* box_moments, float* cov_sum, int32_t* samples) {
    if (!h) return BOD_ERR_INVALID_ARG;
    BODCHK(stat_handle(h, "bod_stat_get"));
    if (cov_sum && !h->cfg.has_covar_head) return h->fail(BOD_ERR_INVALID_ARG, "model has no covariance head");
    const size_t BA = (size_t)h->cfg.batch * h->A;
    BODCHK(d2h(h, cls_sum, h->stat_acc[0], BA * h->cfg.num_classes));
    BODCHK(d2h(h, box_moments, h->stat_acc[1], BA * 16));
    BODCHK(d2h(h, cov_sum, h->stat_acc[2], BA * 10));
    HIPCHK(h, hipStreamSynchronize(h->stream));
    if (samples) *samples = h->stat_k;
    return BOD_OK;
}

bod_status bod_stat_set(bod_handle h, const float* cls_sum, const float* box_moments, const float* cov_sum, int32_t samples) {
    if (!h) return BOD_ERR_INVALID_ARG;
    BODCHK(stat_handle(h, "bod_stat_set"));
    if (samples < 0 || samples > (1 << 24)) return h->fail(BOD_ERR_INVALID_ARG, "bod_stat_set: samples = %d", samples);
    if (cov_sum && !h->cfg.has_covar_head) return h->fail(BOD_ERR_INVALID_ARG, "model has no covariance head");
    const size_t BA = (size_t)h->cfg.batch * h->A;
    if (cls_sum) HIPCHK(h, hipMemcpyAsync(h->stat_acc[0], cls_sum, BA * h->cfg.num_classes * 4, hipMemcpyHostToDevice, h->stream));
    if (box_moments) HIPCHK(h, hipMemcpyAsync(h->stat_acc[1], box_moments, BA * 64, hipMemcpyHostToDevice, h->stream));
    if (cov_sum) HIPCHK(h, hipMemcpyAsync(h->stat_acc[2], cov_sum, BA * 40, hipMemcpyHostToDevice, h->stream));
    HIPCHK(h, hipStreamSynchronize(h->stream));
    h->stat_k = samples;
    h->stat_ent_k = 0;
    return BOD_OK;
}

bod_status bod_stat_merge_entropy(bod_handle h, const void* ent_sum, int32_t view) {
    BODCHK(class_parts_handle(h, "bod_stat_merge_entropy"));
    BODCHK(stat_handle(h, "bod_stat_merge_entropy"));
    BODCHK(stat_view_ready(h, "bod_stat_merge_entropy", view));
    return stat_fold_entropy(h, "bod_stat_merge_entropy", static_cast<const float*>(ent_sum), view);
}

bod_status bod_stat_device_entropy(bod_handle h, void** ptr) {
    BODCHK(class_parts_handle(h, "bod_stat_device_entropy"));
    BODCHK(stat_handle(h, "bod_stat_device_entropy"));
    if (!ptr) return h->fail(BOD_ERR_INVALID_ARG, "bod_stat_device_entropy: ptr is NULL");
    *ptr = h->stat_ent;
    return BOD_OK;
}

bod_status bod_stat_get_entropy(bod_handle h, float* ent_sum) {
    BODCHK(class_parts_handle(h, "bod_stat_get_entropy"));
    BODCHK(stat_handle(h, "bod_stat_get_entropy"));
    if (h->stat_ent_k != h->stat_k)
        return h->fail(BOD_ERR_NOT_READY, "bod_stat_get_entropy: ent_sum holds %d of the record's %d samples", h->stat_ent_k, h->stat_k);
    BODCHK(d2h(h, ent_sum, h->stat_ent, (size_t)h->cfg.batch * h->A));
    HIPCHK(h, hipStreamSynchronize(h->stream));
    return BOD_OK;
}

bod_status bod_stat_set_entropy(bod_handle h, const float* ent_sum) {
    BODCHK(class_parts_handle(h, "bod_stat_set_entropy"));
    BODCHK(stat_handle(h, "bod_stat_set_entropy"));
    if (!ent_sum) return h->fail(BOD_ERR_INVALID_ARG, "bod_stat_set_entropy: ent_sum is NULL");
    HIPCHK(h, hipMemcpyAsync(h->stat_ent, ent_sum, (size_t)h->cfg.batch * h->A * 4, hipMemcpyHostToDevice, h->stream));
    HIPCHK(h, hipStreamSynchronize(h->stream));
    h->stat_ent_k = h->stat_k;
    return BOD_OK;
}

bod_status bod_stat_posterior(bod_handle h, uint64_t seed, uint32_t first_image_id) {
    if (!h) return BOD_ERR_INVALID_ARG;
    BODCHK(stat_handle(h, "bod_stat_posterior"));
    if (h->stat_k < 2) return h->fail(BOD_ERR_NOT_READY, "bod_stat_posterior: the accumulator holds %d samples; bayes_od needs >= 2 (sample covariance divides by N-1)", h->stat_k);
    if (h->class_parts && h->stat_ent_k != h->stat_k)
        return h->fail(BOD_ERR_NOT_READY, "bod_stat_posterior: ent_sum holds %d of the record's %d samples (bod_stat_merge_entropy / bod_stat_set_entropy has not followed)", h->stat_ent_k, h->stat_k);
    if (!h->anchors_ready) return h->fail(BOD_ERR_NOT_READY, "bod_set_anchors has not been called");
    for (int sidx = 0; sidx < 2; ++sidx)
        if (h->side_pending[sidx]) HIPCHK(h, hipStreamWaitEvent(h->stream, h->ev_done[sidx], 0));
    MarkerRange mr("bod:posterior");
    PostCfg pc = post_cfg(h, seed, first_image_id);
    pc.N = h->stat_k;
    pc.aggregated = 1;
    PostBuffers pb = h->pb;
    pb.cls = nullptr; pb.box = nullptr; pb.cov = nullptr; pb.anchors = h->d_anchors;
    pb.agg_cls = h->stat_acc[0]; pb.agg_box = h->stat_acc[1]; pb.agg_cov = h->stat_acc[2];
    h->keep_ready = false;
    HIPCHK(h, launch_posterior(pc, pb, h->stream));
    if (h->parts) { HIPCHK(h, launch_posterior_parts(pc, pb, h->parts, h->stream)); std::fill(h->parts_ok.begin(), h->parts_ok.end(), 1); }
    if (h->cparts) { HIPCHK(h, launch_posterior_class_parts(pc, pb, h->stat_ent, h->cparts, h->stream)); std::fill(h->cparts_ok.begin(), h->cparts_ok.end(), 1); }
    if (h->cfg.ranking_method == BOD_RANK_JOINT_ENTROPY && h->cfg.gaussian_isotropic && h->cfg.dirichlet_non_informative)
        HIPCHK(h, launch_joint_entropy_rank(pc, pb, h->stream));
    h->posterior_done = true; h->nms_done = h->cluster_done = false; h->affinity_img = -1;
    return BOD_OK;
}

bod_status bod_profile_select(bod_handle h, int32_t which) {
    if (!h) return BOD_ERR_INVALID_ARG;
    if (which < 0 || which > 2) return h->fail(BOD_ERR_INVALID_ARG, "bod_profile_select: %d", which);
    h->prof_which = which;
    return BOD_OK;
}

bod_status bod_profile_end(bod_handle h, double* head_ms, int64_t* head_launches, double* head_flops, double* post_ms, int64_t* post_launches) {
    if (!h) return BOD_ERR_INVALID_ARG;
    BODCHK(join_overlap(h));
    HIPCHK(h, hipStreamSynchronize(h->stream));
    double hm = 0, pm = 0;
    for (auto& e : h->ev_head) { float ms = 0; HIPCHK(h, hipEventElapsedTime(&ms, e.first, e.second)); hm += ms; }
    for (auto& e : h->ev_post) { float ms = 0; HIPCHK(h, hipEventElapsedTime(&ms, e.first, e.second)); pm += ms; }
    if (head_ms) *head_ms = hm;
    if (head_launches) *head_launches = (int64_t)h->ev_head.size();
    if (head_flops) *head_flops = h->prof_flops;
// ... 11 lines not shown
```

### bayes-od-rc_amd/csrc/kernels.h

```cpp
#pragma once
#include <hip/hip_runtime.h>
#include <stdint.h>
#include <vector>
#include "../../include/bayesod.h"
#include "plan_tables.h"
#include "sparse_tables.h"


struct ConvGroup {
    const void* in;
    const void* w;
    const float* bias;
    void* out;
    const void* res;
    void* out_relu;
    int32_t in_coff;
    int32_t layer_id;
    const void* w2;
    const float* bias2;
    float* out2;
    int32_t cout2;
    int32_t out2_cstride;
    int32_t agg_kind;
    int32_t agg_n;
// ... 60 lines not shown
bool conv_igemm_uses_full_cout_tile(const ConvArgs& a);
bool conv_igemm_uses_big_tile(const ConvArgs& a);
void conv_igemm_phase_cycles(unsigned long long* out16, bool reset);
hipError_t launch_conv_igemm_f32(const ConvArgs& a, hipStream_t s);
hipError_t launch_pairs_to_hx(const void* in, void* out, long npix, int C, hipStream_t s, int fmt = 1);

hipError_t launch_stem_conv(const float* img, const float* w, const float* bias, void* out, int out_f32,
                            int B, int H, int W, int oh, int ow, hipStream_t s);
enum StemConvForm { STEM_CONV_F32 = 0, STEM_CONV_SEG64 = 1, STEM_CONV_ROW = 2 };
bool stem_conv_row_fits(const float* img, int W);
StemConvForm stem_conv_form(const float* img, int out_f32, int W);
hipError_t launch_stem_conv_form(StemConvForm form, const float* img, const float* w, const float* bias, void* out,
                                 int B, int H, int W, int oh, int ow, hipStream_t s);
bool stem_pool_fused_applies(const float* img, int B, int W, int ow, int n_cu);
hipError_t launch_stem_pool_fused(const float* img, const float* w, const float* bias, void* pooled, int split, int B, int H, int W, int oh,
                                  int ow, int ph, int pw, int pool_pitch, int pool_plane, hipStream_t s);
enum StemFusedForm { STEM_FUSED_8 = 0, STEM_FUSED_4 = 1, STEM_FUSED_SPLIT = 2 };
bool stem_pool_fused_fits(const float* img, int W, int ow);
StemFusedForm stem_pool_fused_form(int split);
hipError_t launch_stem_pool_fused_form(StemFusedForm form, const float* img, const float* w, const float* bias, void* pooled, int B, int H,
                                       int W, int oh, int ow, int ph, int pw, int pool_pitch, int pool_plane, hipStream_t s);
hipError_t launch_stem_pool(const void* in, void* out, int mode, int B, int ih, int iw, int oh, int ow,
                            int out_pitch, int out_plane, hipStream_t s);

struct PostCfg {
    int32_t B, N, A, C, draws;
    int32_t use_full_covar, has_covar, dirichlet, gaussian_iso, ranking_method;
    float iso_var;
    float kitti_sh, kitti_sw;
    const float* kitti_frame;
    uint32_t seed_lo, seed_hi, image_base;
    int32_t aggregated;
};

struct PostBuffers {
    const float* cls;
    const float* box;
    const float* cov;
    const float* anchors;
    const float* agg_cls;
    const float* agg_box;
    const float* agg_cov;
    uint8_t* keep;
    float* d_counts;
    int32_t* block_counts;
    int32_t* num_kept;
    float* counts;
    float* score;
    float* means;
    float* covs;
    float* ranking;
    float* corners;
    int32_t* anchor_index;
};

hipError_t launch_posterior(const PostCfg& c, const PostBuffers& b, hipStream_t s);
hipError_t launch_posterior_keep(const PostCfg& c, const PostBuffers& b, hipStream_t s);
hipError_t launch_posterior_fuse(const PostCfg& c, const PostBuffers& b, hipStream_t s);

struct SparseTailArgs {
    const uint8_t* keep;
    const RowEnt* pix;
    RowEnt* rows;
    int2* ext;
    RowEnt* halo_rows;
    int2* halo_ext;
    int32_t* tile_count;
    int2* runs;
    StQuad* chunks;
    StQuad* tiles;
    int32_t B, N, P, apl, cap_tiles;
    int32_t tail_rows;
    int64_t Ppad;
    SparseLevels lv;
};
hipError_t launch_sparse_tail_rows(const SparseTailArgs& a, hipStream_t s);
hipError_t launch_joint_entropy_rank(const PostCfg& c, const PostBuffers& b, hipStream_t s);
hipError_t launch_validation_post(const PostCfg& c, const PostBuffers& b, hipStream_t s);

struct NmsArgs {
    int32_t B, A;
    const int32_t* num_kept;
    const float* corners;
    const float* ranking;
    float* work_scores;
    int32_t* work_begin;
    int32_t* selected;
    int32_t* num_selected;
    int32_t max_out;
    float iou_thr, sigma;
    int32_t variant;
};
hipError_t launch_nms(const NmsArgs& a, hipStream_t s);

struct ValGatherArgs {
    int32_t B, A, C, max_out;
    const int32_t* num_kept;
    const int32_t* selected;
    const int32_t* num_selected;
    const float* score;
    const float* corners;
    float* out_scores;
    float* out_corners;
    int32_t* out_num;
};
hipError_t launch_validation_gather(const ValGatherArgs& a, hipStream_t s);

struct ClusterArgs {
    int32_t B, A, C, max_out;
    const int32_t* num_kept;
    const int32_t* selected;
    const int32_t* num_selected;
    const float* corners;
    const float* counts;
    const float* means;
    const float* covs;
    float thr;
    const float* affinity; int32_t affinity_img;
    float* out_scores; float* out_means; float* out_covs; float* out_counts;
};
hipError_t launch_cluster_fuse(const ClusterArgs& a, hipStream_t s);
hipError_t launch_iou_matrix(const float* corners, int M, float* out, hipStream_t s);
#define BOD_PARTS_TRI 30
hipError_t launch_posterior_parts(const PostCfg& c, const PostBuffers& b, float* parts, hipStream_t s);
hipError_t launch_cluster_parts(const ClusterArgs& a, const float* parts, float* out_parts, hipStream_t s);
#define BOD_LOG_SDEN(x) (__builtin_amdgcn_logf(x) * 0.693147180559945f)
hipError_t launch_posterior_class_parts(const PostCfg& c, const PostBuffers& b, const float* ent_sum, float* cparts, hipStream_t s);
hipError_t launch_cluster_class_parts(const ClusterArgs& a, const float* cparts, float* out_cparts, hipStream_t s);
hipError_t launch_pack_records(const int32_t* num, const float* scores, const float* means, const float* covs, const float* counts,
                               float* rec, int B, int K, int C, hipStream_t s);
hipError_t launch_pack_records_parts(const int32_t* num, const float* scores, const float* means, const float* covs, const float* counts,
                                     const float* parts, float* rec, int B, int K, int C, hipStream_t s);
hipError_t launch_pack_records_class(const int32_t* num, const float* scores, const float* means, const float* covs, const float* counts,
                                     const float* parts, const float* cparts, float* rec, int B, int K, int C, hipStream_t s);

struct PreprocArgs {
    const uint8_t* src;
    float* dst;
    int32_t B, sh, sw;
    int32_t rh, rw;
    int32_t H, W;
    int32_t crop_y, crop_x, pad_y, pad_x, vis_h, vis_w;
    int32_t resize;
    float scale_y, scale_x;
    float mean[3];
};
hipError_t launch_preprocess(const PreprocArgs& a, hipStream_t s);

struct PreprocFrame {
    int64_t offset;
    int32_t sh, sw, rh, rw;
    float scale_y, scale_x;
    int32_t crop_y, crop_x, pad_y, pad_x, vis_h, vis_w;
};
struct PreprocRaggedArgs {
    const uint8_t* src;
    float* dst;
    const PreprocFrame* frames;
    int32_t B, H, W;
    int32_t resize;
    float mean[3];
};
hipError_t launch_preprocess_ragged(const PreprocRaggedArgs& a, hipStream_t s);

struct PreprocAugFrame {
    PreprocFrame g;
    int32_t flip;
    int32_t resize;
    float gain, bias;
};
struct PreprocAugArgs {
    const uint8_t* src;
    float* dst;
    const PreprocAugFrame* frames;
    int32_t B, H, W;
    float mean[3];
};
hipError_t launch_preprocess_augment(const PreprocAugArgs& a, hipStream_t s);

struct JpegFrame {
    int64_t coef_off[3];
    int64_t plane_off[3];
    int64_t rgb_off;
    int32_t bw[3], bh[3];
    int32_t components;
    int32_t h_samp, v_samp;
    int32_t width, height;
    int32_t pad[7];
    uint16_t quant[3][64];
};
static_assert(sizeof(JpegFrame) == 512 && offsetof(JpegFrame, quant) == 128, "JpegFrame layout (16-byte loads of the quantisation rows)");
struct JpegArgs {
    const JpegFrame* frames;
    const int16_t* coefs;
    uint8_t* planes;
    uint8_t* rgb;
    int32_t n;
    int32_t idct_wgs_per_frame;
    int32_t color_wgs_per_frame;
};
hipError_t launch_jpeg_idct(const JpegArgs& a, hipStream_t s);
hipError_t launch_jpeg_color(const JpegArgs& a, hipStream_t s);

struct PngFrame {
    int64_t raw_off;
    int64_t rgb_off;
    int32_t height, width;
    int32_t channels;
    int32_t pad;
};
static_assert(sizeof(PngFrame) == 32, "PngFrame layout");
struct PngArgs {
    const PngFrame* frames;
    const uint8_t* raw;
    uint8_t* rgb;
    int32_t n;
    int32_t rows_per_band;
};
constexpr int PNG_MAX_BAND_ROWS = 1024;
hipError_t launch_png_unfilter(const PngArgs& a, hipStream_t s);

struct LossArgs {
    int32_t B, A, C;
    int32_t do_cls;
    int32_t reg_kind;
    float label_smoothing;
    const float* cls; const float* cls_t;
    const float* box; const float* box_t;
    const float* cov;
    const float* anchors;
    const uint8_t* pos; const uint8_t* neg;
    const float* row_term;
};
hipError_t launch_loss(const LossArgs& a, float* partial, int nblocks, hipStream_t s);
hipError_t launch_loss_reduce(const float* partial, int nblocks, float* sums4, hipStream_t s);
hipError_t launch_loss_frames(const LossArgs& a, float* partial, hipStream_t s);
hipError_t launch_loss_frames_reduce(const float* partial, int frames, int nblocks, double* sums, hipStream_t s);
hipError_t launch_loss_backward(const LossArgs& a, const float* sums4, float w_cls, float w_reg, float* dcls, float* dbox, float* dcov,
                                hipStream_t s);
#define BOD_ENERGY_MIN_SAMPLES 2
#define BOD_ENERGY_MAX_SAMPLES 1024
#define BOD_ENERGY_DEFAULT_SAMPLES 64
struct EnergyArgs {
    int32_t B, A, M;
    const float* box; const float* box_t;
    const float* cov;
    const float* anchors;
    const uint32_t* dyn;
    uint32_t seed_lo, seed_hi, first_image_id;
    int32_t id_stride;
    const int32_t* list;
    float* row_term;
};
hipError_t launch_loss_compact(const uint8_t* pos, long long n, int32_t* list, hipStream_t s);
hipError_t launch_energy_forward(const EnergyArgs& a, hipStream_t s);
hipError_t launch_energy_backward(const EnergyArgs& a, const float* sums4, float w_reg, float* dbox, float* dcov, hipStream_t s);
hipError_t launch_head_bias_grad(const float* g, long long rows, int nch, float* out, hipStream_t s);

struct TargetArgs {
    int32_t A, B, C;
    float min_positive_iou, max_negative_iou;
    const float* anchors;
    const int32_t* gt_off;
    const float* gt_boxes;
    const float* gt_classes;
    float* cls_t; float* box_t;
    uint8_t* pos; uint8_t* neg;
    int32_t* best_gt; float* best_iou;
};
hipError_t launch_anchor_targets(const TargetArgs& a, hipStream_t s);

struct StatRawArgs {
    int32_t B, N, A, C;
    const float* cls; const float* box; const float* cov;
    const float* anchors;
    float* cls_sum; float* box_moments; float* cov_sum;
    float* ent_sum;
};
hipError_t launch_stat_from_raw(const StatRawArgs& a, hipStream_t s);
struct StatMergeArgs {
    int64_t BA;
    int32_t C;
    int32_t ka, kb;
    float* acc_cls; float* acc_box; float* acc_cov;
    const float* src_cls; const float* src_box; const float* src_cov;
};
hipError_t launch_stat_merge(const StatMergeArgs& a, hipStream_t s);
struct StatMirrorArgs {
    StatMergeArgs m;
    int32_t A, K, nlev;
    int32_t lvl_off[9];
    int32_t lvl_w[8];
    float u_flip;
};
hipError_t launch_stat_merge_mirror(const StatMirrorArgs& a, hipStream_t s);
hipError_t launch_stat_merge_entropy(float* acc, const float* src, int64_t BA, int copy, const StatMirrorArgs* mirror, hipStream_t s);
hipError_t launch_mirror_images(const float* in, float* out, int B, int H, int W, hipStream_t s);

bool conv_pointwise_eligible(const ConvArgs& a);
bool conv_pointwise_can_fuse_next(const ConvArgs& a);
bool conv_pointwise_can_fuse_next3(const ConvArgs& a);
bool conv_pointwise_can_fuse_dual(const ConvArgs& a);
hipError_t launch_conv_pointwise(const ConvArgs& a, hipStream_t s);
bool conv_slide3x3_eligible(const ConvArgs& a);
hipError_t launch_conv_slide3x3(const ConvArgs& a, hipStream_t s);

hipError_t launch_gather_transpose(const void* in, const RowEnt* rows, void* out, int M, int Kpad, int C, int cstride,
                                   int taps, int KW, bool append_ones_row, hipStream_t s, bool f32 = false);
hipError_t launch_fill_row_bf16(void* row, int n_set, int n_total, float value, hipStream_t s);

struct FoldArgs {
    const float* kernel;
    const float* bias;
    const float *gamma, *beta, *mean, *var;
    float eps;
    int32_t taps, cin, cout, cout_pad;
    uint16_t* w_fwd;
    float* w_fwd32;
    uint16_t* w_bwd;
    uint16_t* w_flip;
    float* b_fwd;
    int32_t f32;
};
struct ActBwdArgs {
    const float* dout;
    const uint16_t* out_bf16;
    const RowEnt* rows;
    float* dres;
    uint16_t* dz;
    uint16_t* dzp;
    uint16_t* dzt;
    int32_t M, cout, cout_pad, out_cstride, res_cstride, Kpad;
    float scale;
    int32_t f32;
};
struct UnfoldArgs {
    const float* dwp;
    const float* kernel; const float* bias;
    const float *gamma, *mean, *var;
    float eps;
    int32_t taps, cin, cout;
    float *d_kernel, *d_bias, *d_gamma, *d_beta;
    float* dot;
    float l2;
    float* l2_loss;
};
hipError_t launch_fold_pack(const FoldArgs& a, hipStream_t s);
hipError_t launch_fold_pack_all(const FoldArgs* device_array, int count, long max_elems, hipStream_t s);
hipError_t launch_act_backward_gather(const ActBwdArgs& a, hipStream_t s, bool* wrote_transpose = nullptr);
hipError_t launch_relu_merge(const float* dout_relu, const void* out, float* dout, long n, hipStream_t s, bool f32 = false);
hipError_t launch_col2im(const float* dxcol, const RowEnt* rows, float* din, int M, int taps, int KW, int cin, int in_cstride, hipStream_t s);
hipError_t launch_stem_pool_backward(const void* stem_out, const float* dpool, void* dz, int B, int ih, int iw, int oh, int ow, int pool_pitch,
                                     int pool_plane, hipStream_t s, bool f32 = false);
hipError_t launch_unfold_grad(const UnfoldArgs& a, hipStream_t s);
hipError_t launch_l2_grad(const float* w, float* g, long n, float rate, float* loss_acc, hipStream_t s);
hipError_t launch_sumsq(const float* g, long n, float* acc, float* partial1024, hipStream_t s);
hipError_t launch_adam(float* w, const float* g, float* m, float* v, long n, const float* sumsq, float clip, const float* lr_t, float beta1, float beta2,
                       float eps, hipStream_t s);
hipError_t launch_f32_to_bf16(const float* in, void* out, long n, hipStream_t s);
hipError_t launch_make_dgrad_rows(const RowEnt* fwd, RowEnt* out, int M, hipStream_t s);

int pdq_corner_heatmaps_run(int H, int W, int n, const double* means_yx, const double* covs_yx, int32_t* rois, float* heatmaps,
                            hipStream_t s, char* errbuf, size_t errcap);
int pdq_frames_run(int H, int W, int F, const int32_t* num_gt, const int32_t* gt_boxes, const int32_t* num_det, const int32_t* det_boxes,
                   const double* det_corner_covs, double* fg_loss, double* bg_loss, double* det_bg_loss, float* heatmaps, hipStream_t s,
                   char* errbuf, size_t errcap);
int score_pairs_run(long long n, const double* means, const double* covs, const double* targets, int num_samples, unsigned long long seed,
                    unsigned long long first_row_id, double* out, int32_t* status, hipStream_t s, char* errbuf, size_t errcap);

struct CorruptSpec {
    int32_t n = 0, ops_per_frame = 0;
    std::vector<bod_corrupt_op> ops;
    std::vector<uint32_t> frame_ids;
    std::vector<uint16_t> taps;
    std::vector<uint8_t> luts;
    std::vector<uint16_t> qtables;
    uint64_t seed = 0;
};
int corrupt_spec_make(const char* who, int32_t n, const bod_corrupt_op* ops, int32_t ops_per_frame, const uint32_t* frame_ids,
                      const uint16_t* taps, int32_t n_taps, const uint8_t* luts, int32_t n_luts, const uint16_t* qtables,
                      int32_t n_qtables, uint64_t seed, CorruptSpec* out, char* errbuf, size_t errcap);
struct CorruptSlot {
    std::vector<char> host;
    char* dev = nullptr; size_t dev_cap = 0;
    uint8_t* scratch = nullptr; size_t scratch_cap = 0;
    hipEvent_t copied = nullptr;
    size_t sums_off = 0, sums_bytes = 0, taps_off = 0, luts_off = 0, q_off = 0, frame_bytes = 0;
    int32_t wgs[4][4] = {};
    uint32_t kinds[4] = {};
    void release();
};
int corrupt_prepare(CorruptSlot& slot, const char* who, const CorruptSpec& spec, const int32_t* src_hw, hipStream_t stream,
                    char* errbuf, size_t errcap);
int corrupt_enqueue(CorruptSlot& slot, const char* who, const CorruptSpec& spec, uint8_t* buf, hipStream_t stream, uint8_t** result,
                    char* errbuf, size_t errcap);
```

### bayes-od-rc_amd/engine.py

```python
import ctypes as C

import numpy as np

from . import _lib
from ._lib import BodConfig, BodSizes, as_f32, fptr, iptr

_KINDS = {"kernel": 0, "bias": 1, "gamma": 2, "beta": 3, "mean": 4, "var": 5}
PRECISIONS = {"bf16": 0, "fp32": 1, "bf16x3": 2, "f16mx": 3, "f16mx4": 4}
VIEWS = {"identity": _lib.BOD_VIEW_IDENTITY, "hflip": _lib.BOD_VIEW_HFLIP}


def make_config(image_hw, batch=1, mc_samples=10, num_classes=8, anchors_per_location=9, device=0,
                dropout_rate=0.3, use_full_covar=True, bayes_od_config=None, nms_config=None,
                has_covar_head=True, dataset_name='bdd', orig_size=None, nms_variant='A',
                num_categorical_draws=30, layers=(3, 4, 5, 6, 7), precision='bf16', mc_sample_base=0,
                mc_ensemble_size=0, training=False, backbone_depth=50, pipeline_overlap=False, mc_statistics=False,
                covariance_parts=False, class_parts=False):
    bo = bayes_od_config or {'ranking_method': 'score', 'dirichlet_prior': {'type': 'non_informative'},
                             'gaussian_prior': {'type': 'isotropic', 'isotropic_variance': 100000.0}}
    nms = nms_config or {'max_output_size': 100, 'iou_threshold': 0.5, 'soft_nms_sigma': 0.5}
    cfg = BodConfig()
    cfg.device = int(device)
    cfg.image_h, cfg.image_w = int(image_hw[0]), int(image_hw[1])
    cfg.batch, cfg.mc_samples = int(batch), int(mc_samples)
# ... 396 lines not shown
        if loss_options is not None:
            self.set_loss_options(**loss_options)
        ng, boxes, classes = _pack_gt(gt_boxes, gt_classes, self.B, self.Ccls)
        sums = np.empty((self.B, 4), np.float64)
        self._chk_val(self.lib.bod_validation_losses_boxes(self.h, iptr(ng), fptr(boxes), fptr(classes), float(min_positive_iou),
                                                           float(max_negative_iou), int(bool(do_classification)), int(reg_kind),
                                                           float(label_smoothing), _lib.dptr(sums)))
        return sums

    def _val_records(self, num, scores, corners):
        return [(scores[b, :num[b]].copy(), corners[b, :num[b]].copy()) for b in range(self.B)]

    def validation_detections_batch(self):
        num = np.empty(self.B, np.int32)
        scores, corners = np.empty((self.B, self.K, self.Ccls), np.float32), np.empty((self.B, self.K, 4), np.float32)
        self._chk_val(self.lib.bod_get_validation_detections_batch(self.h, iptr(num), fptr(scores), fptr(corners)))
        return self._val_records(num, scores, corners)

    def validate_boxes(self, images, gt_boxes, gt_classes, min_positive_iou=0.5, max_negative_iou=0.4, do_classification=True,
                       reg_kind=3, label_smoothing=0.001, loss_options=None):
        if loss_options is not None:
            self.set_loss_options(**loss_options)
        ng, boxes, classes = _pack_gt(gt_boxes, gt_classes, self.B, self.Ccls)
        if images is None:
            ptr, on_dev = self.lib.bod_device_images(self.h), 1
        else:
            img = self._img(images)
            ptr, on_dev = img.ctypes.data, 0
        sums, num = np.empty((self.B, 4), np.float64), np.empty(self.B, np.int32)
        scores, corners = np.empty((self.B, self.K, self.Ccls), np.float32), np.empty((self.B, self.K, 4), np.float32)
        self._chk_val(self.lib.bod_validate_boxes(self.h, ptr, on_dev, iptr(ng), fptr(boxes), fptr(classes), float(min_positive_iou),
                                                  float(max_negative_iou), int(bool(do_classification)), int(reg_kind),
                                                  float(label_smoothing), _lib.dptr(sums), iptr(num), fptr(scores), fptr(corners)))
        return sums, self._val_records(num, scores, corners)

    def num_kept(self):
        out = np.zeros(self.B, np.int32)
        self._chk(self.lib.bod_get_num_kept(self.h, iptr(out)))
        return out

    def get_posterior(self, image_index=0):
        m = int(self.num_kept()[image_index])
        counts = np.empty((m, self.Ccls), np.float32)
        score = np.empty((m, self.Ccls), np.float32)
        means = np.empty((m, 4), np.float32)
        covs = np.empty((m, 4, 4), np.float32)
        ranking = np.empty((m,), np.float32)
        aidx = np.empty((m,), np.int32)
        self._chk(self.lib.bod_get_posterior(self.h, image_index, fptr(counts), fptr(score), fptr(means),
                                             fptr(covs), fptr(ranking), iptr(aidx)))
        return {"counts": counts, "score": score, "means": means, "covs": covs, "ranking": ranking,
                "anchor_index": aidx}

    def set_posterior(self, image_index, counts, means, covs, ranking):
        counts, means, covs, ranking = as_f32(counts), as_f32(means).reshape(-1, 4), as_f32(covs), as_f32(ranking)
        m = means.shape[0]
        self._chk(self.lib.bod_set_posterior(self.h, image_index, m, fptr(counts), fptr(means), fptr(covs),
                                             fptr(ranking)))

    def get_posterior_parts(self, image_index=0):
        m = int(self.num_kept()[image_index])
        parts = np.empty((m, 3, 4, 4), np.float32)
        self._chk(self.lib.bod_get_posterior_parts(self.h, image_index, fptr(parts)))
        return parts

    def set_posterior_parts(self, image_index, parts):
        parts = as_f32(parts).reshape(-1, 3, 4, 4)
        self._chk(self.lib.bod_set_posterior_parts(self.h, image_index, parts.shape[0], fptr(parts)))

    def get_detection_parts(self, image_index=0):
        parts = np.empty((self.K, 3, 4, 4), np.float32)
        n = C.c_int32(0)
        self._chk(self.lib.bod_get_detection_parts(self.h, image_index, fptr(parts)))
        self._chk(self.lib.bod_get_detections(self.h, image_index, C.byref(n), None, None, None, None))
        return parts[:n.value].copy()

    def get_detection_parts_batch(self):
        parts = np.empty((self.B, self.K, 3, 4, 4), np.float32)
        self._chk(self.lib.bod_get_detection_parts_batch(self.h, fptr(parts)))
        return parts

    def device_detection_parts_pointer(self, slot=0):
        p = C.c_void_p(0)
        self._chk(self.lib.bod_device_detection_parts(self.h, slot, C.byref(p)))
        return int(p.value or 0), (self.B, self.K, 3, 16)

    @property
    def has_cov_parts(self):
        return bool(self.cfg.covariance_parts & _lib.BOD_PARTS_COVARIANCE)

    @property
    def has_class_parts(self):
        return bool(self.cfg.covariance_parts & _lib.BOD_PARTS_CLASS)

    def get_posterior_class_parts(self, image_index=0):
        m = int(self.num_kept()[image_index])
        rows = np.empty((m, 3), np.float32)
        self._chk(self.lib.bod_get_posterior_class_parts(self.h, image_index, fptr(rows)))
        return rows

    def get_posterior_mean_probs(self, image_index=0):
        m = int(self.num_kept()[image_index])
        p = np.empty((m, self.Ccls), np.float32)
        self._chk(self.lib.bod_get_posterior_mean_probs(self.h, image_index, fptr(p)))
        return p

    def set_posterior_class_parts(self, image_index, mean_probs, rows):
        mean_probs = as_f32(mean_probs).reshape(-1, self.Ccls)
        rows = as_f32(rows).reshape(-1, 3)
        if rows.shape[0] != mean_probs.shape[0]:
            raise ValueError("mean_probs has %d rows, rows has %d" % (mean_probs.shape[0], rows.shape[0]))
        self._chk(self.lib.bod_set_posterior_class_parts(self.h, image_index, rows.shape[0], fptr(mean_probs), fptr(rows)))

    def get_detection_class_parts(self, image_index=0):
        rows = np.empty((self.K, 4), np.float32)
        n = C.c_int32(0)
        self._chk(self.lib.bod_get_detection_class_parts(self.h, image_index, fptr(rows)))
        self._chk(self.lib.bod_get_detections(self.h, image_index, C.byref(n), None, None, None, None))
        return rows[:n.value].copy()

    def get_detection_class_parts_batch(self):
        rows = np.empty((self.B, self.K, 4), np.float32)
        self._chk(self.lib.bod_get_detection_class_parts_batch(self.h, fptr(rows)))
        return rows

    def device_detection_class_parts_pointer(self, slot=0):
        p = C.c_void_p(0)
        self._chk(self.lib.bod_device_detection_class_parts(self.h, slot, C.byref(p)))
        return int(p.value or 0), (self.B, self.K, 4)

    def nms(self):
        self._chk(self.lib.bod_nms(self.h))

    def get_nms(self, image_index=0):
        idx = np.zeros(self.K, np.int32)
        n = C.c_int32(0)
        self._chk(self.lib.bod_get_nms(self.h, image_index, iptr(idx), C.byref(n)))
        return idx[:n.value].copy()

    def _set_centres(self, image_index, centres):
        c = np.ascontiguousarray(centres, dtype=np.int32)
        self._chk(self.lib.bod_set_nms(self.h, image_index, iptr(c), c.shape[0]))

    def set_affinity(self, image_index, centre_columns):
        c = as_f32(centre_columns)
        self._chk(self.lib.bod_set_affinity(self.h, image_index, fptr(c), c.shape[0], c.shape[1]))

    def get_iou_matrix(self, image_index=0):
        m = int(self.num_kept()[image_index])
        out = np.empty((m, m), np.float32)
        if m:
            self._chk(self.lib.bod_get_iou_matrix(self.h, image_index, fptr(out)))
        return out

    def cluster_fuse(self):
        self._chk(self.lib.bod_cluster_fuse(self.h))

    def get_detections(self, image_index=0):
        k = self.K
        scores = np.empty((k, self.Ccls), np.float32)
        means = np.empty((k, 4), np.float32)
        covs = np.empty((k, 4, 4), np.float32)
        counts = np.empty((k, self.Ccls), np.float32)
        n = C.c_int32(0)
        self._chk(self.lib.bod_get_detections(self.h, image_index, C.byref(n), fptr(scores), fptr(means),
                                              fptr(covs), fptr(counts)))
        n = n.value
        return scores[:n].copy(), means[:n].copy(), covs[:n].copy(), counts[:n].copy()

    def get_detections_batch(self, out=None):
        b, k, c = self.B, self.K, self.Ccls
        if out is None:
            out = {"num": np.empty(b, np.int32), "scores": np.empty((b, k, c), np.float32),
                   "means": np.empty((b, k, 4), np.float32), "covs": np.empty((b, k, 4, 4), np.float32),
                   "counts": np.empty((b, k, c), np.float32)}
        self._chk(self.lib.bod_get_detections_batch(self.h, iptr(out["num"]), fptr(out["scores"]),
                                                    fptr(out["means"]), fptr(out["covs"]), fptr(out["counts"])))
        return out

    def wait_slot(self, slot):
        self._chk(self.lib.bod_collect(self.h, slot, None, None, None, None, None))

    def device_raw_pointers(self, mark_ready=False):
        ptrs = (C.c_void_p * 3)()
        self._chk(self.lib.bod_device_raw(self.h, ptrs, int(mark_ready)))
        return [ptrs[i] for i in range(3)]

    def device_detection_pointers(self, slot=0):
        ptrs = (C.c_void_p * 5)()
        self._chk(self.lib.bod_device_detections(self.h, slot, ptrs))
        b, k, c = self.B, self.K, self.Ccls
        shapes = [(b,), (b, k, c), (b, k, 4), (b, k, 16), (b, k, c)]
        names = ["num", "scores", "means", "covs", "counts"]
        return {n: (int(p), s) for n, p, s in zip(names, ptrs, shapes)}

    def stat_reset(self):
        self._chk(self.lib.bod_stat_reset(self.h))

    @staticmethod
    def _view(view):
        if isinstance(view, str):
            if view not in VIEWS:
                raise ValueError("view must be one of %s or 0 / 1, got %r" % (sorted(VIEWS), view))
            return VIEWS[view]
        return int(view)

    def stat_forward(self, images=None, seed=0, first_image_id=0, sample_base=0, image_buffer=None, device_images=None, view=0):
        v = self._view(view)
        if images is None:
            ptr, on_device = (self._device_images(image_buffer) if device_images is None else int(device_images)), 1
        else:
            a = self._img(images)
            ptr, on_device = a.ctypes.data, 0
        if v == _lib.BOD_VIEW_IDENTITY:
            self._chk(self.lib.bod_stat_forward(self.h, ptr, on_device, seed, first_image_id, int(sample_base)))
        else:
            self._chk(self.lib.bod_stat_forward_view(self.h, ptr, on_device, seed, first_image_id, int(sample_base), v))

    def stat_merge_from(self, other):
        self._chk(self.lib.bod_stat_merge_from(self.h, other.h))

    def stat_merge(self, ptrs, samples, view=0):
        ptrs = list(ptrs)
        p = (C.c_void_p * 3)(*[int(x) if x else None for x in (ptrs + [None])[:3]])
        v = self._view(view)
        if v == _lib.BOD_VIEW_IDENTITY:
            self._chk(self.lib.bod_stat_merge(self.h, p, int(samples)))
        else:
            self._chk(self.lib.bod_stat_merge_view(self.h, p, int(samples), v))
        if len(ptrs) > 3 and ptrs[3]:
            self.stat_merge_entropy(ptrs[3], view=v)

    def stat_merge_entropy(self, ptr, view=0):
        self._chk(self.lib.bod_stat_merge_entropy(self.h, C.c_void_p(int(ptr)), self._view(view)))

    def stat_device_entropy_pointer(self):
        p = C.c_void_p(0)
        self._chk(self.lib.bod_stat_device_entropy(self.h, C.byref(p)))
        return int(p.value or 0)

    def get_entropy(self):
        ent = np.empty((self.B, self.A), np.float32)
        self._chk(self.lib.bod_stat_get_entropy(self.h, fptr(ent)))
        return ent

    def set_entropy(self, ent_sum):
        ent = as_f32(ent_sum)
        if ent.shape != (self.B, self.A):
            raise ValueError("ent_sum of shape %s, expected %s" % (ent.shape, (self.B, self.A)))
        self._chk(self.lib.bod_stat_set_entropy(self.h, fptr(ent)))

    def stat_device_pointers(self):
        ptrs = (C.c_void_p * 3)()
        self._chk(self.lib.bod_stat_device(self.h, ptrs, None))
        return [ptrs[i] for i in range(3)]

    @property
    def stat_samples(self):
        k = C.c_int32(0)
        self._chk(self.lib.bod_stat_device(self.h, None, C.byref(k)))
        return int(k.value)

    def get_statistics(self):
        n = (self.B, self.A)
        cls = np.empty(n + (self.Ccls,), np.float32)
        box = np.empty(n + (16,), np.float32)
        cov = np.empty(n + (10,), np.float32) if self.cfg.has_covar_head else None
        k = C.c_int32(0)
        self._chk(self.lib.bod_stat_get(self.h, fptr(cls), fptr(box), fptr(cov), C.byref(k)))
        return cls, box, cov, int(k.value)

    def set_statistics(self, cls_sum, box_moments, cov_sum=None, samples=0):
        n = (self.B, self.A)
        arrs = []
        for a, w in ((cls_sum, self.Ccls), (box_moments, 16), (cov_sum, 10)):
            a = as_f32(a) if a is not None else None
            if a is not None and a.shape != n + (w,):
                raise ValueError("statistics array of shape %s, expected %s" % (a.shape, n + (w,)))
            arrs.append(a)
        self._chk(self.lib.bod_stat_set(self.h, fptr(arrs[0]), fptr(arrs[1]), fptr(arrs[2]), int(samples)))

    def stat_posterior(self, seed=0, first_image_id=0):
        self._chk(self.lib.bod_stat_posterior(self.h, seed, first_image_id))

    def bench_head_conv(self, layer=1, variant=0, iters=10):
        ms, fl = C.c_double(0), C.c_double(0)
        self._chk(self.lib.bod_bench_head_conv(self.h, layer, variant, iters, C.byref(ms), C.byref(fl)))
        return ms.value, fl.value

    def gather_detections(self, slot=-1, comm=None, world=1, rank=0, root=0, want_host=True):
        w = int(self.lib.bod_record_width(self.h))
        out = None
        dev = C.c_void_p(0)
        if rank == root and want_host:
            out = np.empty((world, self.B, self.K, w), np.float32)
        self._chk(self.lib.bod_gather_detections(self.h, int(slot), C.c_void_p(int(comm) if comm else 0), int(world), int(rank), int(root),
                                                 out.ctypes.data if out is not None else None,
                                                 C.byref(dev) if rank == root else None))
        if rank == root and not want_host:
            return int(dev.value or 0), (world, self.B, self.K, w)
        return out

    def plan_info(self):
        info = (C.c_int32 * 11)()
        self._chk(self.lib.bod_plan_info_n(self.h, info, 11))
        return {"aggregating": bool(info[0]), "fused_head_outputs": bool(info[1]), "row_reuse": bool(info[2]),
                "fan_out_row_reuse": bool(info[3]), "ops": int(info[4]), "plane_row_reuse_layers": int(info[5]), "tower_mx": bool(info[6]), "tower_mx_format": int(info[6]),
                "sparse_tail": bool(info[7]), "sparse_halo": bool(info[8]), "sparse_tail_rows": int(info[9]),
                "stage_end_pixels": int(info[10])}

    @property
    def aggregating(self):
        return self.plan_info()["aggregating"]

    def profile_begin(self, which=None):
        if which is not None:
            self._chk(self.lib.bod_profile_select(self.h, int(which)))
        self._chk(self.lib.bod_profile_begin(self.h))

    def profile_end(self):
        hm, pm, fl = C.c_double(0), C.c_double(0), C.c_double(0)
        hl, pl = C.c_int64(0), C.c_int64(0)
        self._chk(self.lib.bod_profile_end(self.h, C.byref(hm), C.byref(hl), C.byref(fl), C.byref(pm), C.byref(pl)))
        return {"head_conv_ms": hm.value, "head_conv_launches": hl.value, "head_conv_flops": fl.value,
                "posterior_ms": pm.value, "posterior_launches": pl.value}


def pack_ragged(frames, batch=None):
    frames = list(frames)
    if batch is not None and len(frames) != int(batch):
        raise ValueError("expected %d frames, got %d" % (int(batch), len(frames)))
    if not frames:
        raise ValueError("no frames to pack")
    for i, f in enumerate(frames):
        if not isinstance(f, np.ndarray) or f.dtype != np.uint8 or f.ndim != 3 or f.shape[2] != 3 or f.shape[0] < 1 or f.shape[1] < 1:
            raise ValueError("frame %d: expected a uint8 array of shape (h, w, 3), got %s %s" %
                             (i, getattr(f, "dtype", type(f).__name__), getattr(f, "shape", "")))
    sizes = np.asarray([f.shape[:2] for f in frames], np.int32)
    buf = np.empty(3 * int(np.sum(sizes[:, 0].astype(np.int64) * sizes[:, 1])), np.uint8)
    off = 0
    for f in frames:
        buf[off:off + f.size] = f.reshape(-1)
        off += f.size
    return buf, sizes


AUGMENT_DTYPE = np.dtype([("flip", "<i4"), ("scale", "<f4"), ("off_y", "<f4"), ("off_x", "<f4"), ("gain", "<f4"), ("bias", "<f4")])
AUGMENT_IDENTITY = {"flip": 0, "scale": 1.0, "off_y": 0.5, "off_x": 0.5, "gain": 1.0, "bias": 0.0}
AUGMENT_DEFAULTS = {"flip_probability": 0.5, "scale_range": [0.8, 1.25], "random_placement": True, "gain_range": [0.8, 1.2],
                    "bias_range": [-20.0, 20.0], "min_visible": 0.25}


def augment_records(aug, batch=None):
    if isinstance(aug, np.ndarray):
        if aug.dtype != AUGMENT_DTYPE:
            raise ValueError("augmentation records must have dtype AUGMENT_DTYPE, got %s" % (aug.dtype,))
        rec = np.ascontiguousarray(aug).reshape(-1)
    else:
        rec = np.empty(len(aug), AUGMENT_DTYPE)
        for i, d in enumerate(aug):
            unknown = set(d) - set(AUGMENT_IDENTITY)
            if unknown:
                raise ValueError("frame %d: unknown augmentation field(s) %s" % (i, sorted(unknown)))
            rec[i] = tuple(d.get(k, v) for k, v in AUGMENT_IDENTITY.items())
    if batch is not None and rec.shape[0] != int(batch):
        raise ValueError("expected %d augmentation records, got %d" % (int(batch), rec.shape[0]))
    return rec


def augment_config(cfg=None):
    out = dict(AUGMENT_DEFAULTS)
    unknown = set(cfg or {}) - set(out)
    if unknown:
        raise ValueError("unknown augmentation setting(s) %s (known: %s)" % (sorted(unknown), sorted(out)))
    out.update(cfg or {})
    return out


def _f32_in(x, lo, hi):
    v = np.float32(x)
    if float(v) > hi:
        v = np.nextafter(v, np.float32(-np.inf))
    elif float(v) < lo:
        v = np.nextafter(v, np.float32(np.inf))
    return v


def draw_augmentation(cfg, seed, image_ids):
    cfg = augment_config(cfg)
    ids = [int(i) for i in np.asarray(image_ids).reshape(-1)]
    rec = np.empty(len(ids), AUGMENT_DTYPE)
    (s_lo, s_hi), (g_lo, g_hi), (b_lo, b_hi) = cfg["scale_range"], cfg["gain_range"], cfg["bias_range"]
    if not (0.0 < s_lo <= s_hi) or g_lo > g_hi or b_lo > b_hi or not (0.0 <= cfg["flip_probability"] <= 1.0):
        raise ValueError("bad augmentation ranges: %r" % (cfg,))
    for k, image_id in enumerate(ids):
        u = np.random.Generator(np.random.Philox(key=[int(seed), image_id])).random(6)
        placed = bool(cfg["random_placement"])
        rec[k] = (int(u[0] < cfg["flip_probability"]),
                  _f32_in(np.exp(np.log(s_lo) + u[1] * (np.log(s_hi) - np.log(s_lo))), s_lo, s_hi),
                  np.float32(u[2]) if placed else 0.5, np.float32(u[3]) if placed else 0.5,
                  _f32_in(g_lo + u[4] * (g_hi - g_lo), g_lo, g_hi), _f32_in(b_lo + u[5] * (b_hi - b_lo), b_lo, b_hi))
    return rec


def augment_boxes(src_hw, net_hw, aug, gt_boxes, gt_classes, aspect_resize=True, min_visible=0.25):
    lib = _lib.load()
    sizes = np.ascontiguousarray(src_hw, dtype=np.int32).reshape(-1, 2)
    b = sizes.shape[0]
    rec = augment_records(aug, b)
    if len(gt_boxes) != b or len(gt_classes) != b:
        raise ValueError("expected ground truth for %d frames, got %d box and %d class arrays" % (b, len(gt_boxes), len(gt_classes)))
    boxes = [as_f32(x).reshape(-1, 4) for x in gt_boxes]
    classes = [as_f32(c) for c in gt_classes]
    width = max([c.shape[-1] for c in classes if c.ndim == 2] + [c.size // x.shape[0] for x, c in zip(boxes, classes) if x.shape[0]])
    for i, (x, c) in enumerate(zip(boxes, classes)):
        if c.size != x.shape[0] * width:
            raise ValueError("frame %d: class rows of shape %s do not match %d boxes x %d classes" % (i, c.shape, x.shape[0], width))
    ng = np.asarray([x.shape[0] for x in boxes], np.int32)
    allb = as_f32(np.concatenate(boxes + [np.zeros((1, 4), np.float32)], axis=0))
    allc = as_f32(np.concatenate([c.reshape(-1, width) for c in classes] + [np.zeros((1, width), np.float32)], axis=0))
    rows = int(np.maximum(ng, 1).sum())
    num_out, bo, co = np.empty(b, np.int32), np.empty((rows, 4), np.float32), np.empty((rows, width), np.float32)
    st = lib.bod_augment_boxes(b, iptr(sizes), int(net_hw[0]), int(net_hw[1]), int(bool(aspect_resize)),
                               rec.ctypes.data_as(C.POINTER(_lib.BodAugment)), iptr(ng), fptr(allb), fptr(allc), width,
                               float(min_visible), iptr(num_out), fptr(bo), fptr(co))
    _lib.check(lib, None, st)
    ends = np.cumsum(num_out)
    return ([bo[e - n:e].copy() for n, e in zip(num_out, ends)], [co[e - n:e].copy() for n, e in zip(num_out, ends)])


def _pack_gt(gt_boxes, gt_classes, batch, num_classes=None):
    if len(gt_boxes) != batch or len(gt_classes) != batch:
        raise ValueError("expected ground truth for %d frames, got %d box and %d class arrays" % (batch, len(gt_boxes), len(gt_classes)))
    boxes = [as_f32(b).reshape(-1, 4) for b in gt_boxes]
    classes = [as_f32(c) for c in gt_classes]
    classes = [c.reshape(b.shape[0], -1) if c.ndim != 2 else c for b, c in zip(boxes, classes)]
    width = classes[0].shape[1] if num_classes is None else num_classes
    for b, c in zip(boxes, classes):
        if c.shape != (b.shape[0], width):
            raise ValueError("class rows of shape %s do not match %d boxes x %d classes" % (c.shape, b.shape[0], width))
    ng = np.asarray([b.shape[0] for b in boxes], np.int32)
    return ng, as_f32(np.concatenate(boxes, axis=0)), as_f32(np.concatenate(classes, axis=0))


def anchor_targets(anchors, gt_boxes, gt_classes, min_positive_iou=0.5, max_negative_iou=0.4, device=0, return_best=False):
    lib = _lib.load()
    anchors = as_f32(anchors).reshape(-1, 4)
    b, a = len(gt_boxes), anchors.shape[0]
    ng, boxes, classes = _pack_gt(gt_boxes, gt_classes, b)
    c = classes.shape[1]
    ct, bt = np.empty((b, a, c), np.float32), np.empty((b, a, 4), np.float32)
    pm, nm = np.empty((b, a), np.uint8), np.empty((b, a), np.uint8)
    bg = np.empty((b, a), np.int32) if return_best else None
    bi = np.empty((b, a), np.float32) if return_best else None
    u8 = C.POINTER(C.c_uint8)
    st = lib.bod_anchor_targets(device, a, fptr(anchors), b, iptr(ng), fptr(boxes), fptr(classes), c, float(min_positive_iou),
                                float(max_negative_iou), fptr(ct), fptr(bt), pm.ctypes.data_as(u8), nm.ctypes.data_as(u8),
                                iptr(bg), fptr(bi))
    _lib.check(lib, None, st)
    out = (ct, bt, pm.astype(bool), nm.astype(bool))
    return out + (bg, bi) if return_best else out


def stage_conv(x, w, bias=None, stride=1, padding="same", relu=False, residual=None, dropout_rate=0.0,
               seed=0, layer_id=0, image_id=0, round_output_bf16=False, device=0, precision='bf16'):
    lib = _lib.load()
    x, w = as_f32(x), as_f32(w)
    b, h, wd, cin = x.shape
    kh, kw, cin2, cout = w.shape
    if cin2 != cin:
        raise ValueError("kernel Cin %d != input Cin %d" % (cin2, cin))
    if padding == "same":
        oh, ow = -(-h // stride), -(-wd // stride)
    else:
        oh, ow = (h - kh) // stride + 1, (wd - kw) // stride + 1
    out = np.empty((b, oh, ow, cout), np.float32)
    bias = as_f32(bias) if bias is not None else None
    residual = as_f32(residual) if residual is not None else None
    st = lib.bod_stage_conv(device, fptr(x), b, h, wd, cin, fptr(w), fptr(bias), kh, kw, cout, stride,
                            int(padding == "same"), int(relu), fptr(residual), float(dropout_rate), seed,
                            layer_id, image_id, int(round_output_bf16), PRECISIONS[precision], fptr(out))
    _lib.check(lib, None, st)
    return out


def stage_conv_wgrad(x, dy, kernel_hw, stride=1, padding="same", ksplit=0, device=0):
    lib = _lib.load()
    x, dy = as_f32(x), as_f32(dy)
    b, h, wd, cin = x.shape
    kh, kw = int(kernel_hw[0]), int(kernel_hw[1])
    cout = dy.shape[-1]
    dw = np.empty((kh, kw, cin, cout), np.float32)
    db = np.empty((cout,), np.float32)
    st = lib.bod_stage_conv_wgrad(device, fptr(x), b, h, wd, cin, fptr(dy), kh, kw, cout, stride,
                                  int(padding == "same"), int(ksplit), fptr(dw), fptr(db))
    _lib.check(lib, None, st)
    return dw, db


def stage_conv_dgrad(dy, w, padding="same", device=0):
    w = as_f32(w)
    if padding != "same" or w.shape[0] % 2 == 0 or w.shape[1] % 2 == 0:
        raise ValueError("stage_conv_dgrad covers stride-1 SAME convolutions with odd kernels")
    wt = np.ascontiguousarray(np.transpose(w[::-1, ::-1], (0, 1, 3, 2)))
    return stage_conv(dy, wt, None, stride=1, padding="same", device=device)


def stage_act_backward(dout, out_off, cout, cout_pad, out_cstride, kpad, out_act=None, dout_relu=None, scale=1.0, res_off=None,
                       res_cstride=0, dres=None, dzp=None, dzt=None, precision="bf16", device=0):
    lib = _lib.load()
    dout = as_f32(dout).reshape(-1)
    out_off = np.ascontiguousarray(out_off, dtype=np.int32).reshape(-1)
    m = int(out_off.size)
    flat = lambda a: None if a is None else as_f32(a).reshape(-1).copy()
    out_act, dout_relu, dres, dzp, dzt = flat(out_act), flat(dout_relu), flat(dres), flat(dzp), flat(dzt)
    for name, a in (("out_act", out_act), ("dout_relu", dout_relu), ("dzp", dzp)):
        if a is not None and a.size != dout.size:
            raise ValueError("%s must have dout's %d elements" % (name, dout.size))
    if dzt is not None and dzt.size != int(cout_pad) * int(kpad):
        raise ValueError("dzt must have cout_pad * kpad elements")
    if res_off is not None:
        res_off = np.ascontiguousarray(res_off, dtype=np.int32).reshape(-1)
        if res_off.size != m:
            raise ValueError("res_off must have one entry per row")
    dz = np.empty((m, int(cout_pad)), np.float32)
    wrote = C.c_int32(-1)
    st = lib.bod_stage_act_backward(device, PRECISIONS[precision], fptr(dout), fptr(out_act), fptr(dout_relu), dout.size, iptr(out_off),
                                    iptr(res_off), m, int(cout), int(cout_pad), int(out_cstride), int(res_cstride), float(scale),
                                    int(kpad), fptr(dres), 0 if dres is None else dres.size, fptr(dz), fptr(dzp), fptr(dzt),
                                    C.byref(wrote))
    _lib.check(lib, None, st)
    return {"dz": dz, "dzp": dzp, "dzt": None if dzt is None else dzt.reshape(int(cout_pad), int(kpad)), "dres": dres,
            "wrote_transpose": bool(wrote.value)}


DGRAD_ROUTES = {"flip": _lib.BOD_DGRAD_FLIP, "rows": _lib.BOD_DGRAD_ROWS, "col2im": _lib.BOD_DGRAD_COL2IM}


def stage_conv_dgrad_route(dz, w, in_hw, din, route, stride=1, padding="same", ksplit=0, device=0):
    lib = _lib.load()
    dz, w, din = as_f32(dz), as_f32(w), as_f32(din).copy()
    grouped = w.ndim == 5
    g = w.shape[0] if grouped else 1
    kh, kw, cin, cout = w.shape[-4:]
    h, wd = int(in_hw[0]), int(in_hw[1])
    b = dz.shape[-4]
    if padding == "same":
        oh, ow = -(-h // stride), -(-wd // stride)
    else:
        oh, ow = (h - kh) // stride + 1, (wd - kw) // stride + 1
    lead = (g,) if grouped else ()
    if dz.shape != lead + (b, oh, ow, cout) or din.shape != lead + (b, h + 2, wd + 2, cin):
        raise ValueError("dz %s / din %s do not fit %d group(s) of a %dx%d input" % (dz.shape, din.shape, g, h, wd))
    info = np.zeros(2, np.int32)
    st = lib.bod_stage_conv_dgrad(device, DGRAD_ROUTES[route], fptr(dz), fptr(w), b, h, wd, cin, cout, kh, kw, int(stride),
                                  int(padding == "same"), int(ksplit), g, fptr(din), iptr(info))
    _lib.check(lib, None, st)
    return din, int(info[0]), bool(info[1])


def stage_stem_pool_backward(stem_out, dpool, precision="bf16", device=0):
    lib = _lib.load()
    stem_out, dpool = as_f32(stem_out), as_f32(dpool)
    b, ih, iw, c = stem_out.shape
    if c != 64:
        raise ValueError("the stem has 64 channels")
    dz = np.empty_like(stem_out)
    st = lib.bod_stage_stem_pool_backward(device, PRECISIONS[precision], fptr(stem_out), fptr(dpool), dpool.size, b, ih, iw, fptr(dz))
    _lib.check(lib, None, st)
    return dz


STEM_FORMS = {"auto": _lib.BOD_STEM_AUTO, "f32+pool_f32": _lib.BOD_STEM_F32_POOL_F32, "f32+pool_split": _lib.BOD_STEM_F32_POOL_SPLIT,
              "seg64+pool": _lib.BOD_STEM_SEG64_POOL, "row+pool": _lib.BOD_STEM_ROW_POOL, "fused8": _lib.BOD_STEM_FUSED_8,
              "fused4": _lib.BOD_STEM_FUSED_4, "fused_split": _lib.BOD_STEM_FUSED_SPLIT}
STEM_FORM_PRECISION = {"f32+pool_f32": "fp32", "f32+pool_split": "bf16x3", "seg64+pool": "bf16", "row+pool": "bf16", "fused8": "bf16",
                       "fused4": "bf16", "fused_split": "bf16x3"}
STEM_SENTINEL = -65536.0


def stem_geometry(h, w):
    oh, ow = (h - 7) // 2 + 1, (w - 7) // 2 + 1
    return oh, ow, (oh - 1) // 2 + 1, (ow + 1) // 2 + 1


def stage_stem(images, w, bias, form="auto", precision=None, misalign=False, n_cu=0, sentinel=STEM_SENTINEL, device=0):
    lib = _lib.load()
    images, w, bias = as_f32(images), as_f32(w), as_f32(bias)
    if images.ndim != 4 or images.shape[3] != 3 or w.shape != (7, 7, 3, 64) or bias.shape != (64,):
        raise ValueError("stage_stem: images [B,H,W,3], w [7,7,3,64], bias [64]")
    if precision is None:
        precision = STEM_FORM_PRECISION[form]
    b, h, wd, _ = images.shape
    oh, ow, ph, pw = stem_geometry(h, wd)
    if min(oh, ow) < 1:
        raise ValueError("stage_stem: H and W must be at least 7")
    stem = np.full((b, oh, ow, 64), np.nan, np.float32)
    pooled = np.full((b, ph + 2, pw + 2, 128 if precision == "bf16x3" else 64), np.nan, np.float32)
    ran = C.c_int32(-1)
    st = lib.bod_stage_stem(device, STEM_FORMS[form], PRECISIONS[precision], fptr(images), b, h, wd, fptr(w), fptr(bias), int(bool(misalign)),
                            int(n_cu), float(sentinel), fptr(stem), fptr(pooled), C.byref(ran))
    _lib.check(lib, None, st)
    name = {v: k for k, v in STEM_FORMS.items()}[ran.value]
    return {"form": name, "stem": None if name.startswith("fused") else stem, "pooled": pooled}


def stage_stem_pool(stem, mode, sentinel=STEM_SENTINEL, device=0):
    lib = _lib.load()
    stem = as_f32(stem)
    if stem.ndim != 4 or stem.shape[3] != 64:
        raise ValueError("stage_stem_pool: stem [B,ih,iw,64]")
    b, ih, iw, _ = stem.shape
# ... 253 lines not shown
```

### bayes-od-rc_amd/kernel_guard.py

```python
import os
import re
import subprocess
import tempfile

import shutil


def _llvm_bin_candidates():
    import glob
    roots = []
    for hipcc in (os.environ.get("HIPCC"), shutil.which("hipcc")):
        if hipcc:
            roots.append(os.path.dirname(os.path.dirname(os.path.realpath(hipcc))))
    roots += [os.environ.get("ROCM_PATH"), os.environ.get("ROCM_HOME"), "/opt/rocm"] + sorted(glob.glob("/opt/rocm-*"), reverse=True)
    out = []
    for r in roots:
        if r:
            for sub in ("lib/llvm/bin", "llvm/bin", "bin"):
                d = os.path.join(r, sub)
                if d not in out:
                    out.append(d)
    return out

PRODUCTION = [
    "conv_igemm_kernelILi256ELi256ELi2ELi4ELi0ELb1ELb0EE",
    "conv_igemm_kernelILi256ELi256ELi2ELi4ELi5ELb1ELb0EE",
    "conv_igemm_kernelILi256ELi256ELi2ELi4ELi6ELb1ELb0EE",
    "conv_igemm_kernelILi256ELi256ELi2ELi4ELi0ELb0ELb0EE",
    "conv_igemm_kernelILi128ELi128ELi2ELi2ELi0ELb0ELb0EE",
    "conv_igemm_kernelILi64ELi128ELi1ELi4ELi0ELb0ELb0EE",
    "conv_igemm_kernelILi64ELi128ELi1ELi4ELi10ELb0ELb0EE",
    "conv_igemm_kernelILi128ELi128ELi2ELi2ELi10ELb0ELb0EE",
    "conv_igemm_kernelILi256ELi256ELi2ELi4ELi0ELb0ELb1EE",
    "conv_igemm_kernelILi128ELi128ELi2ELi2ELi0ELb0ELb1EE",
    "conv_igemm_kernelILi64ELi128ELi1ELi4ELi0ELb0ELb1EE",
    "conv_igemm_kernelILi256ELi256ELi2ELi4ELi0ELb1ELb1EE",
    "conv_igemm_kernelILi256ELi256ELi2ELi4ELi9ELb1ELb0EE",
    "conv_igemm_mx_kernelILi1EE",
    "conv_igemm_mx_kernelILi2EE",
    "conv_igemm_mx_kernelILi3EE",
    "conv_igemm_kernelILi256ELi192ELi2ELi4ELi0ELb1ELb0EE",
]
MX_ASM_MFMA = ["conv_igemm_mx_kernelILi1EE", "conv_igemm_mx_kernelILi3EE"]
MX_MFMA_RE = r"(?:v_mfma_scale_f32_32x32x64_f8f6f4|v_mfma_f32_32x32x16_f16)"
def _select(*markers):
    out = [k for k in PRODUCTION if any(m in k for m in markers)]
    assert len(out) == len(markers), (markers, out)
    return out


INLINE_ASM_MFMA = _select("ELi256ELi2ELi4ELi0ELb1ELb0E", "ELi5ELb1ELb0E", "ELi6ELb1ELb0E", "ELi9ELb1ELb0E", "ELi192ELi2ELi4ELi0ELb1ELb0E")
INLINE_ASM_LDS = _select("ELi256ELi2ELi4ELi0ELb1ELb0E", "ELi5ELb1ELb0E", "ELi6ELb1ELb0E", "ELi192ELi2ELi4ELi0ELb1ELb0E")
MIN_LOOP_MFMA = {k: (144 if "ILi256ELi192E" in k else 192) for k in INLINE_ASM_MFMA}
TOLERATED_SCRATCH = {}


class GuardError(RuntimeError):
    pass


def _tool(name):
    for d in _llvm_bin_candidates():
        p = os.path.join(d, name)
        if os.path.exists(p):
            return p
    p = shutil.which(name)
    if p:
        return p
    raise GuardError("%s not found (looked in %s and PATH): the ROCm llvm tools are needed for the kernel guards; "
                     "BOD_SKIP_KERNEL_GUARD=1 builds without them, unchecked" % (name, ", ".join(_llvm_bin_candidates())))


def extract_device_object(host_obj, workdir):
    fat = os.path.join(workdir, "fat.bin")
    co = os.path.join(workdir, "dev.co")
    subprocess.check_call([_tool("llvm-objcopy"), "--dump-section=.hip_fatbin=" + fat, host_obj, os.path.join(workdir, "stripped.o")])
    subprocess.check_call([_tool("clang-offload-bundler"), "--unbundle", "--type=o", "--input=" + fat,
                           "--targets=hipv4-amdgcn-amd-amdhsa--gfx950", "--output=" + co])
    return co


def kernel_metadata(code_object):
    text = subprocess.run([_tool("llvm-readelf"), "--notes", code_object], capture_output=True, text=True, check=True).stdout
    out = {}
    for block in re.split(r"\n  - ", text)[1:]:
        name = re.search(r"\.name:\s+(\S+)", block)
        if not name or ".symbol:" not in block:
            continue
        fields = {}
        for key in ("vgpr_count", "agpr_count", "sgpr_count", "vgpr_spill_count", "sgpr_spill_count", "private_segment_fixed_size",
                    "group_segment_fixed_size"):
            m = re.search(r"\.%s:\s+(\d+)" % key, block)
            if m:
                fields[key] = int(m.group(1))
        out[name.group(1)] = fields
    return out


def check_no_spills(meta, wanted=PRODUCTION, tolerated=()):
    for want in wanted:
        hits = [(n, f) for n, f in meta.items() if want in n]
        if not hits:
            raise GuardError("kernel %s not found in the code object" % want)
        for n, f in hits:
            if want in tolerated and f.get("private_segment_fixed_size", 0) <= TOLERATED_SCRATCH.get(want, 0):
                continue
            if f.get("vgpr_spill_count", 0) or f.get("private_segment_fixed_size", 0):
                raise GuardError("%s spills %d VGPRs (%d B scratch/lane)" % (n, f.get("vgpr_spill_count", 0), f.get("private_segment_fixed_size", 0)))


def check_no_scratch_in_loop(body, want, mfma_re):
    mf = [i for i, l in enumerate(body) if re.match(mfma_re, l)]
    if not mf:
        raise GuardError("%s: no MFMA of the main loop found" % want)
    bad = [l for l in body[mf[0]:mf[-1] + 1] if l.startswith("scratch_")]
    if bad:
        raise GuardError("%s: %d scratch access(es) inside the main loop, e.g. `%s`" % (want, len(bad), bad[0]))
    return len([l for l in body if l.startswith("scratch_")])


def disassemble(code_object, with_addr=False):
    text = subprocess.run([_tool("llvm-objdump"), "-d", "--no-show-raw-insn", code_object], capture_output=True, text=True, check=True).stdout
    funcs, cur = {}, None
    for line in text.split("\n"):
        m = re.match(r"^[0-9a-f]+ <([^>]+)>:$", line)
        if m:
            cur = funcs.setdefault(m.group(1), [])
            continue
        if cur is None:
            continue
        parts = line.split("//")
        ins = parts[0].strip()
        if ins:
            if with_addr:
                am = re.match(r"\s*([0-9A-Fa-f]+):", parts[1]) if len(parts) > 1 else None
                cur.append((int(am.group(1), 16) if am else -1, ins))
            else:
                cur.append(ins)
    return funcs


def _regs(tok):
    m = re.match(r"v\[(\d+):(\d+)\]$", tok)
    if m:
        return set(range(int(m.group(1)), int(m.group(2)) + 1))
    m = re.match(r"v(\d+)$", tok)
    return {int(m.group(1))} if m else set()


MFMA = "v_mfma_f32_16x16x32_bf16"


def check_inline_asm_mfma(body, want, window=16, min_mfma=None, mfma_re=None):
    if min_mfma is None:
        min_mfma = MIN_LOOP_MFMA.get(want, 192)
    MFMA = mfma_re or globals()["MFMA"]
    is_mfma = (lambda l: re.match(MFMA, l) is not None) if mfma_re else (lambda l: l.startswith(MFMA))
    mf = [i for i, l in enumerate(body) if is_mfma(l)]
    if len(mf) < min_mfma:
        raise GuardError("%s: only %d %s found (the loop changed shape: re-derive the guard)" % (want, len(mf), MFMA))
    for i in mf:
        srcs = set()
        for tok in re.findall(r"v\[\d+:\d+\]", body[i]):
            srcs |= _regs(tok)
        slots, k = 0, i - 1
        while k >= 0 and slots < 2:
            l = body[k]
            mm = re.match(r"s_nop (\d+)", l)
            if mm:
                slots += int(mm.group(1)) + 1
            else:
                if l.startswith("v_") and not l.startswith("v_mfma") and not l.startswith("v_cmp"):
                    toks = re.findall(r"v\[\d+:\d+\]|\bv\d+\b", l)
                    if toks and (_regs(toks[0]) & srcs):
                        raise GuardError("%s: `%s` writes a source of `%s` %d slot(s) before it" % (want, l, body[i], slots))
                slots += 1
            k -= 1
        dst = _regs(re.match((MFMA if mfma_re else re.escape(MFMA)) + r" (v\[\d+:\d+\])", body[i]).group(1))
        slots, k = 0, i + 1
        while k < len(body) and slots < window:
            l = body[k]
            mm = re.match(r"s_nop (\d+)", l)
            slots += int(mm.group(1)) + 1 if mm else 1
            if not is_mfma(l) and re.match(r"(v_|ds_|buffer_|global_|flat_)", l):
                toks = re.findall(r"v\[\d+:\d+\]|\bv\d+\b", l)
                touched = set().union(*[_regs(t) for t in toks]) if toks else set()
                if touched & dst:
                    raise GuardError("%s: `%s` touches the destination of `%s` %d slots behind it" % (want, l, body[i], slots))
            if l.startswith("s_cbranch") or l.startswith("s_branch") or l.startswith("s_endpgm"):
                break
            k += 1
    return len(mf)


def check_asm_lds_reads(body, want, min_reads=60):
    addr_index = {a: i for i, (a, _) in enumerate(body)}
    mf = [i for i, (_, l) in enumerate(body) if l.startswith(MFMA)]
    if not mf:
        raise GuardError("%s: no %s" % (want, MFMA))
    start = mf[0]
    while start > 0 and not body[start - 1][1].startswith("s_barrier"):
        start -= 1
    queue, checked, i, steps = [], 0, start, 0
    end = mf[-1] + 1
    seen_back_edge = False
    while i < len(body) and steps < 200000:
        steps += 1
        a, l = body[i]
        op = l.split()[0]
        if op == "ds_read_b128":
            dst = _regs(re.match(r"ds_read_b128 (v\[\d+:\d+\])", l).group(1))
            addr_regs = set().union(*[_regs(t) for t in re.findall(r"\bv\d+\b", l)]) if re.findall(r"\bv\d+\b", l) else set()
            busy = set().union(*[q for q in queue if q]) if queue else set()
            if (dst | addr_regs) & busy:
                raise GuardError("%s: `%s` touches a fragment register still in flight" % (want, l))
            queue.append(dst)
            checked += 1
        elif op.startswith("ds_"):
            queue.append(set())
        elif op.startswith("s_load") or op.startswith("s_buffer_load"):
            pass
        elif op == "s_waitcnt":
            m = re.search(r"lgkmcnt\((\d+)\)", l)
            if m:
                n = int(m.group(1))
                while len(queue) > n:
                    queue.pop(0)
        elif op.startswith("s_cbranch") or op == "s_branch":
            off = int(l.split()[1])
            if off >= 32768:
                off -= 65536
            target = a + 4 + 4 * off
            if off < 0:
                if seen_back_edge:
                    i += 1
                    continue
                seen_back_edge = True
                if target not in addr_index:
                    raise GuardError("%s: branch target %x not found" % (want, target))
                i = addr_index[target]
                continue
            if target not in addr_index:
                raise GuardError("%s: branch target %x not found" % (want, target))
            skipped = [sk for _, sk in body[i + 1:addr_index[target]]]

            def backward(sk):
                return (sk.startswith("s_cbranch") or sk.startswith("s_branch ")) and int(sk.split()[1]) >= 32768
            if not seen_back_edge and any(backward(sk) for sk in skipped):
                i += 1
                continue
            if any(sk.startswith(MFMA) or sk.startswith("ds_read_b128") for sk in skipped):
                i += 1
                continue
            i = addr_index[target]
            continue
        else:
            busy = set().union(*[q for q in queue if q]) if queue else set()
            if busy:
                toks = re.findall(r"v\[\d+:\d+\]|\bv\d+\b", l)
                touched = set().union(*[_regs(t) for t in toks]) if toks else set()
                if touched & busy:
                    raise GuardError("%s: `%s` touches a fragment register whose ds_read may still be in flight (%d reads outstanding)"
                                     % (want, l, len([q for q in queue if q])))
        if i >= end and seen_back_edge and not queue:
            break
        i += 1
    if checked < min_reads:
        raise GuardError("%s: only %d fragment reads walked" % (want, checked))
    return checked


AUX_PRODUCTION = ["stem_conv_bf16_row_kernel", "stem_pool_fused_kernel", "stem_pool_fused_split_kernel"]


def verify_aux(host_obj, wanted=AUX_PRODUCTION):
    with tempfile.TemporaryDirectory() as wd:
        co = extract_device_object(host_obj, wd)
        meta = kernel_metadata(co)
        check_no_spills(meta, wanted)
        return {n: f.get("vgpr_count", -1) for n, f in meta.items() if any(w in n for w in wanted)}


POINTWISE_PRODUCTION = ["pw_conv_kernelILi64ELi64E", "pw_conv_kernelILi128ELi64E", "pw_conv_kernelILi256ELi32E", "pw_conv_kernelILi512ELi32E",
                        "slide3x3_c64_kernel", "slide3x3_c128_kernel"]
POINTWISE_STAGE3 = ["pw_conv512_next_kernel"]


def verify_pointwise(host_obj):
    regs = verify_aux(host_obj, POINTWISE_PRODUCTION)
    for n, v in regs.items():
        m = re.search(r"pw_conv_kernelILi\d+ELi\d+ELb[01]ELi(\d+)ELi(\d+)ELi[012]E", n)
        if m:
            waves_per_simd = int(m.group(1)) * (int(m.group(2)) // 32) / 4.0
            cap = min(512, int(512 / waves_per_simd) // 8 * 8)
        else:
            cap = 256
        if v > cap:
            raise GuardError("%s uses %d registers: more than the %d that keep its workgroups co-resident" % (n, v, cap))
    return regs


def verify_pointwise_stage3(host_obj):
    regs = verify_aux(host_obj, POINTWISE_STAGE3)
    for n, v in regs.items():
        if v > 256:
            raise GuardError("%s uses %d registers: more than the 256 of two waves per SIMD" % (n, v))
    return regs


PACKED_FP32_RE =r"v_pk_(?:mul|add|fma)_f32\b"


def check_no_packed_fp32(host_obj):
    sections = subprocess.run([_tool("llvm-readelf"), "-S", host_obj], capture_output=True, text=True, check=True).stdout
    if ".hip_fatbin" not in sections:
        return 0
    with tempfile.TemporaryDirectory() as d:
        funcs = disassemble(extract_device_object(host_obj, d))
    for name, body in funcs.items():
        hits = [l for l in body if re.match(PACKED_FP32_RE, l)]
        if hits:
            raise GuardError("%s: %d packed fp32 instruction(s) in %s, e.g. `%s` (build with -fno-slp-vectorize: DESIGN.md 8.4)"
                             % (os.path.basename(host_obj), len(hits), name, hits[0]))
    return len(funcs)


def verify(host_obj, wanted=PRODUCTION, asm_kernels=INLINE_ASM_MFMA):
    with tempfile.TemporaryDirectory() as wd:
        co = extract_device_object(host_obj, wd)
        meta = kernel_metadata(co)
        check_no_spills(meta, wanted, tolerated=[w for w in MX_ASM_MFMA if w in wanted])
        funcs = disassemble(co)
        for want in asm_kernels:
            names = [n for n in funcs if want in n]
            if not names:
                raise GuardError("kernel %s not found in the disassembly" % want)
            for n in names:
                check_inline_asm_mfma(funcs[n], want)
        for want in MX_ASM_MFMA:
            if want in wanted:
                for n in [n for n in funcs if want in n]:
                    check_inline_asm_mfma(funcs[n], want, min_mfma=144, mfma_re=MX_MFMA_RE)
                    check_no_scratch_in_loop(funcs[n], want, MX_MFMA_RE)
        if any(w in INLINE_ASM_LDS for w in asm_kernels):
            funcs_a = disassemble(co, with_addr=True)
            for want in INLINE_ASM_LDS:
                for n in [n for n in funcs_a if want in n]:
                    check_asm_lds_reads(funcs_a[n], want)
        return {n: f.get("vgpr_count", -1) + f.get("agpr_count", 0) for n, f in meta.items() if any(w in n for w in wanted)}
```

Before: 2421 images/sec.

## Use LDS-only barriers in pointwise/slide convs and route stage-5 residual 512 to pointwise

Adds an LB template variant of the pointwise and 3x3 slide conv kernels. It replaces __syncthreads with a barrier that waits only on lgkmcnt, so in-flight global DMA loads and stores are not drained at each barrier. It uses LDS-typed vector types, and it preloads the row offsets before issuing the loads so the compiler does not insert vmcnt(0) waits. It also enables the pointwise path for cin=512 with a residual (stage-5 conv) using a new 256-channel config. A disassembly guard checks where vmcnt(0) appears, because correctness now depends on hand-counted waits.

After: 2442 images/sec, median of 6. No clear change (+0.9%).

```diff
diff --git a/bayes-od-rc_amd/build.py b/bayes-od-rc_amd/build.py
--- a/bayes-od-rc_amd/build.py
+++ b/bayes-od-rc_amd/build.py
@@ -110,6 +110,7 @@
             regs.update(kernel_guard.verify_aux(os.path.join(obj_dir, "aux_kernels.o")))
             regs.update(kernel_guard.verify_pointwise(os.path.join(obj_dir, "conv_pointwise.o")))
             regs.update(kernel_guard.verify_pointwise_stage3(os.path.join(obj_dir, "conv_pointwise.o")))
+            regs.update(kernel_guard.verify_pointwise_stream_barrier(os.path.join(obj_dir, "conv_pointwise.o")))
             n_checked = sum(kernel_guard.check_no_packed_fp32(o) for o in objs)
             if verbose:
                 print("no packed fp32 instruction in %d kernels" % n_checked, flush=True)
diff --git a/bayes-od-rc_amd/csrc/conv_pointwise.hip b/bayes-od-rc_amd/csrc/conv_pointwise.hip
--- a/bayes-od-rc_amd/csrc/conv_pointwise.hip
+++ b/bayes-od-rc_amd/csrc/conv_pointwise.hip
@@ -33,8 +33,28 @@
     __builtin_amdgcn_s_barrier();
     asm volatile("" ::: "memory");
 }
-
-template <int K, int BP, bool RES, int WGS, int BC = 128, int NEXT = 0>
+template <bool LB> struct pw_lds_t { typedef float4 f4; typedef uint2 u2; typedef uint4 u4; typedef int4 i4; };
+template <> struct pw_lds_t<true> { typedef pw_f32x4 f4; typedef pw_u32x2 u2; typedef pw_u32x4 u4; typedef pw_i32x4 i4; };
+template <bool LB> __device__ __forceinline__ void pw_barrier() { if (LB) pw_lds_barrier(); else __syncthreads(); }
+
+enum : int { PW_LB_SLIDE128 = 1,
+             PW_LB_SLIDE64 = 2,
+             PW_LB_DUAL = 4,
+             PW_LB_K512 = 8,
+             PW_LB_NEXT = 16 };
+constexpr bool PW_STAGE5_2C_DEFAULT = true;
+constexpr int PW_LB_DEFAULT = PW_LB_SLIDE128 | PW_LB_DUAL | PW_LB_NEXT;
+int conv_stream_barrier_mask() {
+    static const int mask = [] {
+        const char* e = getenv("BOD_STREAM_BARRIER");
+        if (e && atoi(e) == 0) return 0;
+        const char* k = getenv("BOD_STREAM_BARRIER_KERNELS");
+        return k ? (atoi(k) & 31) : PW_LB_DEFAULT;
+    }();
+    return mask;
+}
+
+template <int K, int BP, bool RES, int WGS, int BC = 128, int NEXT = 0, bool LB = false>
 __global__ __launch_bounds__(BC * 2, WGS) void pw_conv_kernel(const ConvArgs a, int ptiles, int ctiles, int pstride) {
     constexpr int THREADS = BC * 2;
     constexpr int CPX = K * 2 / 16;
@@ -48,11 +68,12 @@
     constexpr int K2 = NEXT == 2 ? K : BC;
     constexpr int NTP = NEXT ? BP * (C2 / 8) / THREADS : 0;
     static_assert(NXP >= 1 && NRP >= 1 && BP % 32 == 0 && (CPX & 7) == 0 && (!NEXT || (BC == 256 && BP == 64 && NTP == 1)), "tile shape");
+    typedef typename pw_lds_t<LB>::f4 F4; typedef typename pw_lds_t<LB>::u2 U2; typedef typename pw_lds_t<LB>::u4 U4; typedef typename pw_lds_t<LB>::i4 I4;
     extern __shared__ __attribute__((aligned(16))) char pw_smem[];
     char* const xbuf = pw_smem;
     constexpr int NRB = RES ? 2 : 1;
     char* const rbuf = pw_smem + 2 * XB;
-    int4* const meta = reinterpret_cast<int4*>(pw_smem + 2 * XB + NRB * RB);
+    I4* const meta = reinterpret_cast<I4*>(pw_smem + 2 * XB + NRB * RB);
     char* const tbuf = pw_smem + 2 * XB + NRB * RB + 3 * BP * 16;
 
     const int tid = threadIdx.x, lane = tid & 63;
@@ -71,16 +92,27 @@
         const int valid = m < a.M;
         m = valid ? m : a.M - 1;
         const int4 e = *reinterpret_cast<const int4*>(&a.rows[m]);
-        return make_int4(e.x, e.z, e.w, valid);
+        return I4{e.x, e.z, e.w, valid};
     };
     auto issue = [&](int t) {
-        const int4* mt = meta + (t % 3) * BP;
+        const I4* mt = meta + (t % 3) * BP;
         char* xb = xbuf + (t & 1) * XB;
+        const int* mi = reinterpret_cast<const int*>(mt);
+        int in_off[NXP], res_off[NRP];
+        if (LB) {
+#pragma unroll
+            for (int i = 0; i < NXP; ++i) in_off[i] = mi[((i * THREADS + tid) / CPX) * 4];
+            if (RES) {
+#pragma unroll
+                for (int i = 0; i < NRP; ++i) res_off[i] = mi[((i * THREADS + tid) / RCH) * 4 + 2];
+            }
+            asm volatile("" ::: "memory");
+        }
 #pragma unroll
         for (int i = 0; i < NXP; ++i) {
             const int q = i * THREADS + tid, row = q / CPX, cp = q % CPX;
             const int c = cp ^ pw_swz<CPX>(row);
-            const char* src = reinterpret_cast<const char*>(G.in) + ((size_t)mt[row].x * a.in_cstride + G.in_coff + c * 8) * 2;
+            const char* src = reinterpret_cast<const char*>(G.in) + ((size_t)(LB ? in_off[i] : mt[row].x) * a.in_cstride + G.in_coff + c * 8) * 2;
             __builtin_amdgcn_global_load_lds(PW_GLOBAL_PTR(src), PW_LDS_PTR(xb + (i * THREADS + wave * 64) * 16), 16, 0, 0);
         }
         if (RES) {
@@ -89,14 +121,14 @@
             for (int i = 0; i < NRP; ++i) {
                 const int q = i * THREADS + tid, row = q / RCH, cp = q % RCH;
                 const int c = cp ^ (row & 7);
-                const char* src = reinterpret_cast<const char*>(G.res) + ((size_t)mt[row].z * a.res_cstride + c0 + c * 8) * 2;
+                const char* src = reinterpret_cast<const char*>(G.res) + ((size_t)(LB ? res_off[i] : mt[row].z) * a.res_cstride + c0 + c * 8) * 2;
                 __builtin_amdgcn_global_load_lds(PW_GLOBAL_PTR(src), PW_LDS_PTR(rb + (i * THREADS + wave * 64) * 16), 16, 0, 0);
             }
         }
     };
 
     {
-        const int4 e0 = load_ent(0), e1 = load_ent(1);
+        const I4 e0 = load_ent(0), e1 = load_ent(1);
         if (tid < BP) { meta[tid] = e0; meta[BP + tid] = e1; }
     }
     __syncthreads();
@@ -123,15 +155,15 @@
     }
 
     for (int t = 0; t < nt; ++t) {
-        __syncthreads();
+        pw_barrier<LB>();
         const bool more = t + 1 < nt;
         if (more) issue(t + 1);
         asm volatile("" ::: "memory");
-        const int4 ent = load_ent(t + 2);
+        const I4 ent = load_ent(t + 2);
         asm volatile("" ::: "memory");
         if (more) { if (t > 0) pw_wait_vm<1 + NRP + NTP + NXP + (RES ? NRP : 0) + 1>(); else pw_wait_vm<NXP + (RES ? NRP : 0) + 1>(); }
         else pw_wait_vm<1>();
-        __syncthreads();
+        pw_barrier<LB>();
 
         const char* xb = xbuf + (t & 1) * XB;
         char* rb = rbuf + (RES ? (t & 1) : 0) * RB;
@@ -157,26 +189,26 @@
                 float v0 = __builtin_fmaf(acc[j][g * 4 + 0], 1.0f, bv[g].x), v1 = __builtin_fmaf(acc[j][g * 4 + 1], 1.0f, bv[g].y);
                 float v2 = __builtin_fmaf(acc[j][g * 4 + 2], 1.0f, bv[g].z), v3 = __builtin_fmaf(acc[j][g * 4 + 3], 1.0f, bv[g].w);
                 if (RES) {
-                    const uint2 r = *reinterpret_cast<const uint2*>(p);
+                    const U2 r = *reinterpret_cast<const U2*>(p);
                     v0 += pw_bf2f(r.x & 0xFFFFu) * 1.0f; v1 += pw_bf2f(r.x >> 16) * 1.0f;
                     v2 += pw_bf2f(r.y & 0xFFFFu) * 1.0f; v3 += pw_bf2f(r.y >> 16) * 1.0f;
                 }
-                uint2 o;
+                U2 o;
                 o.x = pw_pack(v0, v1); o.y = pw_pack(v2, v3);
                 if (relu) { o.x = pw_relu(o.x); o.y = pw_relu(o.y); }
-                *reinterpret_cast<uint2*>(p) = o;
-            }
-        }
-        __syncthreads();
+                *reinterpret_cast<U2*>(p) = o;
+            }
+        }
+        pw_barrier<LB>();
         {
-            const int4* mt = meta + (t % 3) * BP;
+            const I4* mt = meta + (t % 3) * BP;
 #pragma unroll
             for (int i = 0; i < NRP; ++i) {
                 const int q = i * THREADS + tid, row = q / RCH, cp = q % RCH;
                 const int c = cp ^ (row & 7);
-                const uint4 v = *reinterpret_cast<const uint4*>(rb + q * 16);
-                const int4 e = mt[row];
-                uint4* dst = e.w ? reinterpret_cast<uint4*>(reinterpret_cast<uint16_t*>(G.out) + (size_t)e.y * a.out_cstride + c0 + c * 8) : &pw_sink[lane];
+                const U4 v = *reinterpret_cast<const U4*>(rb + q * 16);
+                const I4 e = mt[row];
+                U4* dst = e.w ? reinterpret_cast<U4*>(reinterpret_cast<uint16_t*>(G.out) + (size_t)e.y * a.out_cstride + c0 + c * 8) : reinterpret_cast<U4*>(&pw_sink[lane]);
                 *dst = v;
             }
         }
@@ -194,20 +226,20 @@
                 }
 #pragma unroll
                 for (int g = 0; g < 4; ++g) {
-                    uint2 o;
+                    U2 o;
                     o.x = pw_relu(pw_pack(__builtin_fmaf(acc2[g * 4 + 0], 1.0f, bv2[g].x), __builtin_fmaf(acc2[g * 4 + 1], 1.0f, bv2[g].y)));
                     o.y = pw_relu(pw_pack(__builtin_fmaf(acc2[g * 4 + 2], 1.0f, bv2[g].z), __builtin_fmaf(acc2[g * 4 + 3], 1.0f, bv2[g].w)));
-                    *reinterpret_cast<uint2*>(tbuf + px * 128 + ((((wave & 1) * 4 + g) ^ (px & 7)) << 4) + fhalf * 8) = o;
+                    *reinterpret_cast<U2*>(tbuf + px * 128 + ((((wave & 1) * 4 + g) ^ (px & 7)) << 4) + fhalf * 8) = o;
                 }
             }
-            __syncthreads();
+            pw_barrier<LB>();
             {
-                const int4* mt = meta + (t % 3) * BP;
+                const I4* mt = meta + (t % 3) * BP;
                 const int q = tid, row = q >> 3, cp = q & 7;
                 const int c = cp ^ (row & 7);
-                const uint4 v = *reinterpret_cast<const uint4*>(tbuf + q * 16);
-                const int4 e = mt[row];
-                uint4* dst = e.w ? reinterpret_cast<uint4*>(reinterpret_cast<uint16_t*>(G.ch_out3) + (size_t)e.y * C2 + c * 8) : &pw_sink[lane];
+                const U4 v = *reinterpret_cast<const U4*>(tbuf + q * 16);
+                const I4 e = mt[row];
+                U4* dst = e.w ? reinterpret_cast<U4*>(reinterpret_cast<uint16_t*>(G.ch_out3) + (size_t)e.y * C2 + c * 8) : reinterpret_cast<U4*>(&pw_sink[lane]);
                 *dst = v;
             }
         }
@@ -216,12 +248,12 @@
     }
 }
 
-template <int K, int BP, bool RES, int WGS, int BC = 128, int NEXT = 0>
+template <int K, int BP, bool RES, int WGS, int BC = 128, int NEXT = 0, bool LB = false>
 static hipError_t pw_launch_cfg(const ConvArgs& a, hipStream_t s) {
     constexpr int LDS = 2 * BP * K * 2 + (RES ? 2 : 1) * BP * BC * 2 + 3 * BP * 16 + (NEXT ? BP * 128 : 0);
     static PerDeviceOnce once;
     bool& attr_set = *once.slot();
-    auto kern = pw_conv_kernel<K, BP, RES, WGS, BC, NEXT>;
+    auto kern = pw_conv_kernel<K, BP, RES, WGS, BC, NEXT, LB>;
     if (!attr_set) {
         hipError_t e = hipFuncSetAttribute(reinterpret_cast<const void*>(kern), hipFuncAttributeMaxDynamicSharedMemorySize, LDS);
         if (e != hipSuccess) return e;
@@ -438,7 +470,9 @@
     if (g.w2 || g.ch_w2 || g.out_relu || g.agg_kind) return false;
     if (g.ch_w3 && !(g.ch_b3 && g.ch_out3 && ((a.cin == 64 && a.cout_pad == 256 && (g.res != nullptr) != (g.ch_dual != 0)) ||
                                               (a.cin == 128 && a.cout_pad == 512 && g.res && !g.ch_dual)))) return false;
-    if (a.cin != 64 && a.cin != 128 && a.cin != 256 && !(a.cin == 512 && !g.res)) return false;
+    static const bool stage5_2c = [] { const char* e = getenv("BOD_PW_STAGE5_2C"); return e ? atoi(e) != 0 : PW_STAGE5_2C_DEFAULT; }();
+    if (a.cin == 512 && g.res && !(stage5_2c && !g.ch_w3 && a.cout_pad % 256 == 0)) return false;
+    if (a.cin != 64 && a.cin != 128 && a.cin != 256 && a.cin != 512) return false;
     if (a.cout_pad % 128 != 0 || a.cout_valid != a.cout_pad) return false;
     if ((a.in_cstride & 7) || (a.out_cstride & 7) || (g.in_coff & 7) || (g.res && (a.res_cstride & 7))) return false;
     static const int min_m = [] { const char* e = getenv("BOD_POINTWISE_MIN_M"); return e ? atoi(e) : -1; }();
@@ -448,21 +482,25 @@
 
 hipError_t launch_conv_pointwise(const ConvArgs& a, hipStream_t s) {
     const bool res = a.g[0].res != nullptr;
-    if (a.g[0].ch_w3 && a.g[0].ch_dual) return pw_launch_cfg<64, 64, false, 1, 256, 2>(a, s);
+    const int lb = conv_stream_barrier_mask();
+    if (a.g[0].ch_w3 && a.g[0].ch_dual) return (lb & PW_LB_DUAL) ? pw_launch_cfg<64, 64, false, 1, 256, 2, true>(a, s) : pw_launch_cfg<64, 64, false, 1, 256, 2>(a, s);
     if (a.g[0].ch_w3 && a.cin == 128) return pw_launch_next512(a, s);
-    if (a.g[0].ch_w3) return pw_launch_cfg<64, 64, true, 1, 256, 1>(a, s);
+    if (a.g[0].ch_w3) return (lb & PW_LB_NEXT) ? pw_launch_cfg<64, 64, true, 1, 256, 1, true>(a, s) : pw_launch_cfg<64, 64, true, 1, 256, 1>(a, s);
     if (a.cin == 64) return res ? pw_launch_cfg<64, 64, true, 3>(a, s) : pw_launch_cfg<64, 64, false, 3>(a, s);
     if (a.cin == 128) return res ? pw_launch_cfg<128, 64, true, 2>(a, s) : pw_launch_cfg<128, 64, false, 2>(a, s);
-    if (a.cin == 512) return pw_launch_cfg<512, 32, false, 2>(a, s);
+    if (a.cin == 512 && res) return pw_launch_cfg<512, 32, true, 1, 256, 0, true>(a, s);
+    if (a.cin == 512) return (lb & PW_LB_K512) ? pw_launch_cfg<512, 32, false, 2, 128, 0, true>(a, s) : pw_launch_cfg<512, 32, false, 2>(a, s);
     return res ? pw_launch_cfg<256, 32, true, 3>(a, s) : pw_launch_cfg<256, 32, false, 3>(a, s);
 }
 
 
+template <bool LB>
 __global__ __launch_bounds__(256, 2) void slide3x3_c64_kernel(const ConvArgs a, int nstrips, int xsegs) {
     constexpr int SLOT = 66 * 128;
     constexpr int LEAD = 1;
     constexpr int RING = 4;
     constexpr int OB = 64 * 128;
+    typedef typename pw_lds_t<LB>::f4 F4; typedef typename pw_lds_t<LB>::u2 U2; typedef typename pw_lds_t<LB>::u4 U4;
     extern __shared__ __attribute__((aligned(16))) char sl_smem[];
     char* const ring = sl_smem;
     char* const obuf = sl_smem + RING * SLOT;
@@ -506,7 +544,7 @@
             piece(0); piece(1);
             if (wave == 0 && lane < 16) piece(2);
         };
-        __syncthreads();
+        pw_barrier<LB>();
         issue_row(0); issue_row(1); issue_row(2);
         for (int y = 0; y < H; ++y) {
             const bool pre = y + LEAD < H;
@@ -515,7 +553,7 @@
             if (!pre) pw_wait_vm<0>();
             else if (wave == 0) { if (y == 0) pw_wait_vm<3>(); else pw_wait_vm<5>(); }
             else { if (y == 0) pw_wait_vm<2>(); else pw_wait_vm<4>(); }
-            __syncthreads();
+            pw_barrier<LB>();
             pw_f32x16 acc;
 #pragma unroll
             for (int r = 0; r < 16; ++r) acc[r] = 0.f;
@@ -536,21 +574,21 @@
                 const int px = wp * 32 + frow;
 #pragma unroll
                 for (int g = 0; g < 4; ++g) {
-                    uint2 o;
+                    U2 o;
                     o.x = pw_pack(__builtin_fmaf(acc[g * 4 + 0], 1.0f, bv[g].x), __builtin_fmaf(acc[g * 4 + 1], 1.0f, bv[g].y));
                     o.y = pw_pack(__builtin_fmaf(acc[g * 4 + 2], 1.0f, bv[g].z), __builtin_fmaf(acc[g * 4 + 3], 1.0f, bv[g].w));
                     if (relu) { o.x = pw_relu(o.x); o.y = pw_relu(o.y); }
-                    *reinterpret_cast<uint2*>(ob + px * 128 + (((wc * 4 + g) ^ (px & 7)) << 4) + fhalf * 8) = o;
+                    *reinterpret_cast<U2*>(ob + px * 128 + (((wc * 4 + g) ^ (px & 7)) << 4) + fhalf * 8) = o;
                 }
             }
-            __syncthreads();
+            pw_barrier<LB>();
 #pragma unroll
             for (int i = 0; i < 2; ++i) {
                 const int q = i * 256 + tid, px = q >> 3, cp = q & 7;
                 const int c = cp ^ (px & 7);
-                const uint4 v = *reinterpret_cast<const uint4*>(ob + q * 16);
-                uint4* dst = px < nv ? reinterpret_cast<uint4*>(reinterpret_cast<uint16_t*>(G.out) + ((size_t)e0.z + (size_t)y * out_pitch + px) * a.out_cstride + c * 8)
-                                     : &pw_sink[lane];
+                const U4 v = *reinterpret_cast<const U4*>(ob + q * 16);
+                U4* dst = px < nv ? reinterpret_cast<U4*>(reinterpret_cast<uint16_t*>(G.out) + ((size_t)e0.z + (size_t)y * out_pitch + px) * a.out_cstride + c * 8)
+                                     : reinterpret_cast<U4*>(&pw_sink[lane]);
                 *dst = v;
             }
             asm volatile("" ::: "memory");
@@ -558,14 +596,16 @@
     }
 }
 
+template <bool LB>
 __global__ __launch_bounds__(512, 1) void slide3x3_c128_kernel(const ConvArgs a, int nstrips, int xsegs) {
     constexpr int SLOT = 66 * 256;
     constexpr int RING = 4;
     constexpr int OB = 64 * 256;
+    typedef typename pw_lds_t<LB>::f4 F4; typedef typename pw_lds_t<LB>::u2 U2; typedef typename pw_lds_t<LB>::u4 U4;
     extern __shared__ __attribute__((aligned(16))) char sl_smem[];
     char* const ring = sl_smem;
     char* const obuf = sl_smem + RING * SLOT;
-    float4* const xch = reinterpret_cast<float4*>(sl_smem + RING * SLOT + 2 * OB);
+    F4* const xch = reinterpret_cast<F4*>(sl_smem + RING * SLOT + 2 * OB);
     float* const sbias = reinterpret_cast<float*>(sl_smem + RING * SLOT + 2 * OB + 8 * 4096);
     const int tid = threadIdx.x, lane = tid & 63;
     const int wave = __builtin_amdgcn_readfirstlane(tid >> 6);
@@ -607,7 +647,7 @@
             piece(0); piece(1);
             if (wave == 0 && lane < 32) piece(2);
         };
-        __syncthreads();
+        pw_barrier<LB>();
         issue_row(0); issue_row(1); issue_row(2);
         for (int y = 0; y < H; ++y) {
             const bool pre = y + 1 < H;
@@ -616,7 +656,7 @@
             if (!pre) pw_wait_vm<0>();
             else if (wave == 0) { if (y == 0) pw_wait_vm<3>(); else pw_wait_vm<5>(); }
             else { if (y == 0) pw_wait_vm<2>(); else pw_wait_vm<4>(); }
-            __syncthreads();
+            pw_barrier<LB>();
             pw_f32x16 acc[2];
 #pragma unroll
             for (int j = 0; j < 2; ++j)
@@ -637,40 +677,40 @@
                         }
             }
             {
-                float4* mine = xch + wave * 256;
+                F4* mine = xch + wave * 256;
 #pragma unroll
                 for (int g = 0; g < 4; ++g) {
                     const pw_f32x16& v = acc[1 - kh];
-                    mine[g * 64 + lane] = make_float4(v[g * 4 + 0], v[g * 4 + 1], v[g * 4 + 2], v[g * 4 + 3]);
+                    mine[g * 64 + lane] = F4{v[g * 4 + 0], v[g * 4 + 1], v[g * 4 + 2], v[g * 4 + 3]};
                 }
             }
-            __syncthreads();
+            pw_barrier<LB>();
             char* ob = obuf + (y & 1) * OB;
             {
-                const float4* theirs = xch + (wave ^ 4) * 256;
+                const F4* theirs = xch + (wave ^ 4) * 256;
                 const int px = kh * 32 + frow;
 #pragma unroll
                 for (int g = 0; g < 4; ++g) {
-                    const float4 t = theirs[g * 64 + lane];
+                    const F4 t = theirs[g * 64 + lane];
                     const pw_f32x16& v = acc[kh];
                     const float s0 = kh ? t.x + v[g * 4 + 0] : v[g * 4 + 0] + t.x, s1 = kh ? t.y + v[g * 4 + 1] : v[g * 4 + 1] + t.y;
                     const float s2 = kh ? t.z + v[g * 4 + 2] : v[g * 4 + 2] + t.z, s3 = kh ? t.w + v[g * 4 + 3] : v[g * 4 + 3] + t.w;
-                    const float4 bvg = *reinterpret_cast<const float4*>(sbias + cb * 32 + g * 8 + fhalf * 4);
-                    uint2 o;
+                    const F4 bvg = *reinterpret_cast<const F4*>(sbias + cb * 32 + g * 8 + fhalf * 4);
+                    U2 o;
                     o.x = pw_pack(__builtin_fmaf(s0, 1.0f, bvg.x), __builtin_fmaf(s1, 1.0f, bvg.y));
                     o.y = pw_pack(__builtin_fmaf(s2, 1.0f, bvg.z), __builtin_fmaf(s3, 1.0f, bvg.w));
                     if (relu) { o.x = pw_relu(o.x); o.y = pw_relu(o.y); }
-                    *reinterpret_cast<uint2*>(ob + px * 256 + (((cb * 4 + g) ^ (px & 7)) << 4) + fhalf * 8) = o;
+                    *reinterpret_cast<U2*>(ob + px * 256 + (((cb * 4 + g) ^ (px & 7)) << 4) + fhalf * 8) = o;
                 }
             }
-            __syncthreads();
+            pw_barrier<LB>();
 #pragma unroll
             for (int i = 0; i < 2; ++i) {
                 const int q = i * 512 + tid, px = q >> 4, cp = q & 15;
                 const int c = cp ^ (px & 7);
-                const uint4 v = *reinterpret_cast<const uint4*>(ob + q * 16);
-                uint4* dst = px < nv ? reinterpret_cast<uint4*>(reinterpret_cast<uint16_t*>(G.out) + ((size_t)e0.z + (size_t)y * out_pitch + px) * a.out_cstride + c * 8)
-                                     : &pw_sink[lane];
+                const U4 v = *reinterpret_cast<const U4*>(ob + q * 16);
+                U4* dst = px < nv ? reinterpret_cast<U4*>(reinterpret_cast<uint16_t*>(G.out) + ((size_t)e0.z + (size_t)y * out_pitch + px) * a.out_cstride + c * 8)
+                                     : reinterpret_cast<U4*>(&pw_sink[lane]);
                 *dst = v;
             }
             asm volatile("" ::: "memory");
@@ -704,27 +744,31 @@
         static PerDeviceOnce once128;
         bool& set128 = *once128.slot();
         if (!set128) {
-            hipError_t e = hipFuncSetAttribute(reinterpret_cast<const void*>(slide3x3_c128_kernel), hipFuncAttributeMaxDynamicSharedMemorySize, LDS128);
+            hipError_t e = hipFuncSetAttribute(reinterpret_cast<const void*>(slide3x3_c128_kernel<true>), hipFuncAttributeMaxDynamicSharedMemorySize, LDS128);
+            if (e == hipSuccess) e = hipFuncSetAttribute(reinterpret_cast<const void*>(slide3x3_c128_kernel<false>), hipFuncAttributeMaxDynamicSharedMemorySize, LDS128);
             if (e != hipSuccess) return e;
             set128 = true;
         }
         const int xsegs = (a.plane_w + 63) / 64;
         const int nstrips = a.M / (a.plane_h * a.plane_w) * xsegs;
-        hipLaunchKernelGGL(slide3x3_c128_kernel, dim3(std::min(nstrips, launch_cus(a))), dim3(512), LDS128, s, a, nstrips, xsegs);
+        auto kern = (conv_stream_barrier_mask() & PW_LB_SLIDE128) ? slide3x3_c128_kernel<true> : slide3x3_c128_kernel<false>;
+        hipLaunchKernelGGL(kern, dim3(std::min(nstrips, launch_cus(a))), dim3(512), LDS128, s, a, nstrips, xsegs);
         return hipGetLastError();
     }
     constexpr int LDS = 4 * 66 * 128 + 2 * 64 * 128;
     static PerDeviceOnce once;
     bool& attr_set = *once.slot();
     if (!attr_set) {
-        hipError_t e = hipFuncSetAttribute(reinterpret_cast<const void*>(slide3x3_c64_kernel), hipFuncAttributeMaxDynamicSharedMemorySize, LDS);
+        hipError_t e = hipFuncSetAttribute(reinterpret_cast<const void*>(slide3x3_c64_kernel<true>), hipFuncAttributeMaxDynamicSharedMemorySize, LDS);
+        if (e == hipSuccess) e = hipFuncSetAttribute(reinterpret_cast<const void*>(slide3x3_c64_kernel<false>), hipFuncAttributeMaxDynamicSharedMemorySize, LDS);
         if (e != hipSuccess) return e;
         attr_set = true;
     }
     const int xsegs = (a.plane_w + 63) / 64;
     const int nstrips = a.M / (a.plane_h * a.plane_w) * xsegs;
     const int wgs = std::min(nstrips, 2 * launch_cus(a));
-    hipLaunchKernelGGL(slide3x3_c64_kernel, dim3(wgs), dim3(256), LDS, s, a, nstrips, xsegs);
+    auto kern = (conv_stream_barrier_mask() & PW_LB_SLIDE64) ? slide3x3_c64_kernel<true> : slide3x3_c64_kernel<false>;
+    hipLaunchKernelGGL(kern, dim3(wgs), dim3(256), LDS, s, a, nstrips, xsegs);
     return hipGetLastError();
 }
 
diff --git a/bayes-od-rc_amd/csrc/engine.hip b/bayes-od-rc_amd/csrc/engine.hip
--- a/bayes-od-rc_amd/csrc/engine.hip
+++ b/bayes-od-rc_amd/csrc/engine.hip
@@ -4070,12 +4070,13 @@
 
 bod_status bod_plan_info_n(bod_handle h, int32_t* info, int32_t n) {
     if (!h || !info || n < 0) return BOD_ERR_INVALID_ARG;
-    int32_t all[11];
+    int32_t all[12];
     BODCHK(bod_plan_info(h, all));
     all[8] = h->plan_halo;
     all[9] = h->plan_tail_rows;
     all[10] = h->plan_stage_end;
-    for (int i = 0; i < n && i < 11; ++i) info[i] = all[i];
+    all[11] = conv_stream_barrier_mask();
+    for (int i = 0; i < n && i < 12; ++i) info[i] = all[i];
     return BOD_OK;
 }
 
diff --git a/bayes-od-rc_amd/csrc/kernels.h b/bayes-od-rc_amd/csrc/kernels.h
--- a/bayes-od-rc_amd/csrc/kernels.h
+++ b/bayes-od-rc_amd/csrc/kernels.h
@@ -386,6 +386,7 @@
 bool conv_pointwise_can_fuse_next3(const ConvArgs& a);
 bool conv_pointwise_can_fuse_dual(const ConvArgs& a);
 hipError_t launch_conv_pointwise(const ConvArgs& a, hipStream_t s);
+int conv_stream_barrier_mask();
 bool conv_slide3x3_eligible(const ConvArgs& a);
 hipError_t launch_conv_slide3x3(const ConvArgs& a, hipStream_t s);
 
diff --git a/bayes-od-rc_amd/engine.py b/bayes-od-rc_amd/engine.py
--- a/bayes-od-rc_amd/engine.py
+++ b/bayes-od-rc_amd/engine.py
@@ -722,12 +722,12 @@
         return out
 
     def plan_info(self):
-        info = (C.c_int32 * 11)()
-        self._chk(self.lib.bod_plan_info_n(self.h, info, 11))
+        info = (C.c_int32 * 12)()
+        self._chk(self.lib.bod_plan_info_n(self.h, info, 12))
         return {"aggregating": bool(info[0]), "fused_head_outputs": bool(info[1]), "row_reuse": bool(info[2]),
                 "fan_out_row_reuse": bool(info[3]), "ops": int(info[4]), "plane_row_reuse_layers": int(info[5]), "tower_mx": bool(info[6]), "tower_mx_format": int(info[6]),
                 "sparse_tail": bool(info[7]), "sparse_halo": bool(info[8]), "sparse_tail_rows": int(info[9]),
-                "stage_end_pixels": int(info[10])}
+                "stage_end_pixels": int(info[10]), "stream_barrier": int(info[11])}
 
     @property
     def aggregating(self):
diff --git a/bayes-od-rc_amd/kernel_guard.py b/bayes-od-rc_amd/kernel_guard.py
--- a/bayes-od-rc_amd/kernel_guard.py
+++ b/bayes-od-rc_amd/kernel_guard.py
@@ -286,8 +286,12 @@
 POINTWISE_STAGE3 = ["pw_conv512_next_kernel"]
 
 
-def verify_pointwise(host_obj):
-    regs = verify_aux(host_obj, POINTWISE_PRODUCTION)
+def is_stream_barrier_form(name):
+    return re.search(r"(?:pw_conv_kernelILi\d+ELi\d+ELb[01]ELi\d+ELi\d+ELi[012]ELb1EE|slide3x3_c(?:64|128)_kernelILb1EE)", name) is not None
+
+
+def verify_pointwise(host_obj, stream_barrier=False):
+    regs = {n: v for n, v in verify_aux(host_obj, POINTWISE_PRODUCTION).items() if is_stream_barrier_form(n) == stream_barrier}
     for n, v in regs.items():
         m = re.search(r"pw_conv_kernelILi\d+ELi\d+ELb[01]ELi(\d+)ELi(\d+)ELi[012]E", n)
         if m:
@@ -297,6 +301,64 @@
             cap = 256
         if v > cap:
             raise GuardError("%s uses %d registers: more than the %d that keep its workgroups co-resident" % (n, v, cap))
+    return regs
+
+
+def barrier_regions(body):
+    regions = [{"vm0": 0, "mfma": 0, "dma": 0, "last_vm": None}]
+    for l in body:
+        r = regions[-1]
+        if l.startswith("s_barrier"):
+            regions.append({"vm0": 0, "mfma": 0, "dma": 0, "last_vm": None})
+        elif l.startswith("s_waitcnt"):
+            m = re.search(r"vmcnt\((\d+)\)", l)
+            if m:
+                r["last_vm"] = int(m.group(1))
+                r["vm0"] += int(m.group(1)) == 0
+        elif l.startswith("v_mfma"):
+            r["mfma"] += 1
+        elif l.startswith("global_load_lds"):
+            r["dma"] += 1
+    return regions
+
+
+def drained_barriers(body):
+    return [i for i, r in enumerate(barrier_regions(body)[:-1]) if r["last_vm"] == 0]
+
+
+_SLIDE_VM0 = "the last row of a strip (pw_wait_vm<0>: no further row is in flight), once in the peeled first row and once in the row loop"
+_PW_VM0 = ("the peeled first tile waits for the weights, loaded behind tile 0's pieces, once per workgroup; the row-table entry of tile "
+           "t + 2 is written to LDS behind the tile's last barrier, a whole tile's work behind the pieces it drains")
+STREAM_BARRIER_VM0 = {
+    "slide3x3_c128_kernelILb1EE": ({1: 1, 4: 1}, _SLIDE_VM0),
+    "slide3x3_c64_kernelILb1EE": ({1: 1, 3: 1}, _SLIDE_VM0),
+    "pw_conv_kernelILi64ELi64ELb0ELi1ELi256ELi2ELb1EE": ({3: 1, 9: 1}, _PW_VM0),
+    "pw_conv_kernelILi64ELi64ELb1ELi1ELi256ELi1ELb1EE": ({3: 1, 9: 1}, _PW_VM0),
+    "pw_conv_kernelILi512ELi32ELb0ELi2ELi128ELi0ELb1EE": ({3: 1, 7: 1}, _PW_VM0),
+    "pw_conv_kernelILi512ELi32ELb1ELi1ELi256ELi0ELb1EE": ({3: 1, 7: 1}, _PW_VM0),
+}
+
+
+def check_stream_barrier_form(body, want, allowed):
+    regions = barrier_regions(body)
+    for i, r in enumerate(regions):
+        if i and r["vm0"] != allowed.get(i, 0):
+            raise GuardError("%s: %d s_waitcnt vmcnt(0) between barriers %d and %d of the listing, %d expected (the DMA pieces and stores in "
+                             "flight are drained there: conv_pointwise.hip, LB)" % (want, r["vm0"], i - 1, i, allowed.get(i, 0)))
+    return regions
+
+
+def verify_pointwise_stream_barrier(host_obj):
+    regs = verify_pointwise(host_obj, stream_barrier=True)
+    with tempfile.TemporaryDirectory() as wd:
+        funcs = disassemble(extract_device_object(host_obj, wd))
+    for want, (allowed, _) in STREAM_BARRIER_VM0.items():
+        names = [n for n in funcs if want in n]
+        if len(names) != 1 or names[0] not in regs:
+            raise GuardError("kernel %s not found in the code object" % want)
+        check_stream_barrier_form(funcs[names[0]], want, allowed)
+    if len(regs) != len(STREAM_BARRIER_VM0):
+        raise GuardError("LB = true kernels without an entry in STREAM_BARRIER_VM0: %s" % sorted(regs))
     return regs
 
 
```
